# steveschwarcz/Cuda-Path-Tracer-SS

Measured on AMD Instinct MI355X. Metric: Mrays/sec at 1920x1080, 8 bounces, 2072 spp run (BASELINE configs[2] asks 2000 spp; a rate metric); ray = one live ray processed in one bounce, higher is better.
Workload: dtype f32; 1 GPU; configs[2]: 1920x1080 'mixed' preset (22 spheres, 16 triangles, Lambert/Phong/Cook-Torrance/glass/mirror), 8 bounces, 2072 spp = 74 steps x 1 pass(es) x 28 sample lanes per pixel; samples_per_pass=28, frame_lanes=1, lanes_free_run=True, seed=24301

## Files before the change

### cuda-path-tracer-ss_amd/csrc/pthit.h

```cpp
#pragma once
#include "ptaccel.h"

namespace ptss {
namespace {

template <bool kPrimary, bool kAccel, bool kBounded, bool kMesh = false>
__device__ __forceinline__ Hit closestHit(const float4* sc, const float4* cold, const SceneLayout& L, vec3 o, vec3 d, bool live, uint32_t* ws) {
    Hit h;
    h.distance = ptm::inf();
    h.kind = 0;
    h.idx = 0;
    h.w0 = h.w1 = h.w2 = 0;
    if constexpr (kAccel) closestSpheresRegrouped<kPrimary>(sc, cold, L, o, d, live, h, ws);
    for (int base = 0; base < (kAccel ? 0 : L.numSpheres); base += 32) {
        const int cnt = (L.numSpheres - base < 32) ? (L.numSpheres - base) : 32;
        uint32_t mask = sphereCandidates<kPrimary, kBounded>(sc, (kPrimary ? L.offPrimSphere : L.offSphere) + base, cnt, o, d);
        mask &= live ? lowBits(cnt) : 0u;
        PTSS_DIAG_CANDIDATES(mask, live, 0);
        while (mask != 0) {
            const int j = __builtin_ctz(mask);
            mask &= mask - 1;
            float t;
            const bool acc = kPrimary ? sphereTestPrimary(sc[L.offPrimSphere + base + j], d, h.distance, t)
                                      : sphereTest(sc[L.offSphere + base + j], o, d, h.distance, t);
            if (acc) {
                h.distance = t;
                h.kind = 1;
                h.idx = base + j;
            }
        }
    }
    const unsigned long long liveMask = maskOf(live);
    if constexpr (kMesh) {
        if (meshQueryOk(o, d, live)) {
            TriBest best{h.distance, kNoTriangle, 0.0f, 0.0f};
            closestTrianglesMesh<kPrimary>(sc, cold, L, o, d, live, best);
            if (best.key != kNoTriangle) {
                h.distance = best.dist;
                h.kind = 2;
                h.idx = reinterpret_cast<const int*>(cold + L.offTriPos)[0xfffffffeu - best.key];
                h.w1 = best.w1;
                h.w2 = best.w2;
                h.w0 = 1.0f - (best.w1 + best.w2);
            }
            return h;
        }
    } else if (L.triClassed) {
        if (classedQueryOk(o, d)) {
            TriBest best{h.distance, kNoTriangle, 0.0f, 0.0f};
            uint32_t triAt = vectorRow(sc, L.offTri), primAt = vectorRow(sc, L.offPrimTri);
#define PTSS_CLOSEST_BODY(c1, c2, t) \
    triangleClassed<kPrimary, c1, c2, true>(rowAt(sc, triAt), rowAt(sc, primAt), 0u, o, d, liveMask, best);
            PTSS_FOR_TRIANGLES_BY_CLASS(L, PTSS_CLOSEST_BODY, (triAt += 3 * kRowBytes, primAt += 2 * kRowBytes));
#undef PTSS_CLOSEST_BODY
            if (waveAny(best.key != kNoTriangle)) {
                const int* posOf = reinterpret_cast<const int*>(sc + L.offTriPos);
                int pos = 0;
                if (best.key != kNoTriangle) pos = posOf[0xfffffffeu - best.key];
                const bool zeroWeight = best.key != kNoTriangle && (best.w1 == 0.0f || best.w2 == 0.0f);
                if (waveAny(zeroWeight)) {
                    if (zeroWeight) {
                        const float4* rows = sc + L.offTri + 3 * pos;
                        const float4* prim = sc + L.offPrimTri + 2 * pos;
                        const pttri::Head g = pttri::head<0, 0, kPrimary>(xyz(rows[0]), xyz(rows[1]), xyz(rows[2]), xyz(prim[0]), xyz(prim[1]), prim[0].w, o, d);
                        float b0;
                        pttri::weights<0, 0>(g, d, b0, best.w1, best.w2);
                    }
                }
                if (best.key != kNoTriangle) {
                    h.distance = best.dist;
                    h.kind = 2;
                    h.idx = pos;
                    h.w1 = best.w1;
                    h.w2 = best.w2;
                    h.w0 = 1.0f - (best.w1 + best.w2);
                }
            }
            return h;
        }
    } else if (L.triDetBounded && waveAll(dot(d, d) < 0x1p30f)) {
        TriBest best{h.distance, kNoTriangle, 0.0f, 0.0f};
        uint32_t triAt = vectorRow(sc, L.offTri), primAt = vectorRow(sc, L.offPrimTri);
        for (int i = 0; i < L.numTriangles; ++i, triAt += 3 * kRowBytes, primAt += 2 * kRowBytes)
            triangleClassed<kPrimary, 0, 0, false>(rowAt(sc, triAt), rowAt(sc, primAt), (uint32_t)i, o, d, liveMask, best);
        if (best.key != kNoTriangle) {
            h.distance = best.dist;
            h.kind = 2;
            h.idx = (int)best.key;
            h.w1 = best.w1;
            h.w2 = best.w2;
            h.w0 = 1.0f - (best.w1 + best.w2);
        }
        return h;
    }
    const float4* td = kMesh ? cold : sc;
    const int* posOfOriginal = reinterpret_cast<const int*>(td + L.offTriPos);
    for (int k = 0; k < L.numTriangles; ++k) {
        const int i = (kMesh || L.triClassed) ? posOfOriginal[k] : k;
        const TriRows tcur = kPrimary ? loadTriEdges(td + L.offTri + 3 * i) : loadTri(td + L.offTri + 3 * i);
        const TriHit th = kPrimary ? triangleTestPrimary(tcur, td[L.offPrimTri + 2 * i], loadRow16(td + L.offPrimTri + 2 * i + 1), d,
                                                         h.distance, liveMask)
                                   : triangleTest(tcur, o, d, h.distance, liveMask);
        if (th.hit) {
            h.distance = th.dist;
            h.kind = 2;
            h.idx = i;
            h.w0 = th.w0;
            h.w1 = th.w1;
            h.w2 = th.w2;
        }
    }
    return h;
}

__device__ __forceinline__ void anyTriangleLoop(const float4* sc, const SceneLayout& L, vec3 lo, vec3 w_i, float distance, unsigned long long& need,
                                                unsigned long long& blocked) {
    if (L.triClassed && classedQueryOk(lo, w_i)) {
        uint32_t triAt = vectorRow(sc, L.offTri);
#define PTSS_ANY_BODY(c1, c2, t)   \
    if (need == 0ull) break;      \
    triangleClassedAny<c1, c2>(rowAt(sc, triAt), lo, w_i, distance, need, blocked);
        PTSS_FOR_TRIANGLES_BY_CLASS(L, PTSS_ANY_BODY, triAt += 3 * kRowBytes);
#undef PTSS_ANY_BODY
        return;
    }
    for (int i = 0; i < L.numTriangles; ++i) {
        if (need == 0ull) break;
        const TriRows tcur = loadTri(sc + L.offTri + 3 * i);
        const TriHit th = triangleTest(tcur, lo, w_i, distance, need);
        blocked |= th.hitMask;
        need &= ~th.hitMask;
    }
}

__device__ __forceinline__ bool anyTriangles(const float4* sc, const SceneLayout& L, vec3 lo, vec3 w_i, float distance, bool live) {
    unsigned long long need = maskOf(live), blocked = 0ull;
    anyTriangleLoop(sc, L, lo, w_i, distance, need, blocked);
    return __builtin_amdgcn_inverse_ballot_w64(blocked);
}

template <bool kAccel, bool kBounded, bool kMesh = false>
__device__ __forceinline__ bool anyHit(const float4* sc, const SceneLayout& L, vec3 lo, vec3 w_i, float distance,
                                       bool live, const float4* cold = nullptr) {
    bool occluded = false;
    if constexpr (kAccel) occluded = anySphereChunked(sc, L, lo, w_i, distance, live);
    for (int base = 0; base < (kAccel ? 0 : L.numSpheres); base += 32) {
        const int cnt = (L.numSpheres - base < 32) ? (L.numSpheres - base) : 32;
        uint32_t mask = sphereCandidatesPairs<kBounded>(sc, L.offSphere + base, cnt, lo, w_i);
        mask &= (live && !occluded) ? lowBits(cnt) : 0u;
        PTSS_DIAG_CANDIDATES(mask, live, 4);
        while (mask != 0) {
            const int j = __builtin_ctz(mask);
            mask &= mask - 1;
            float t;
            if (sphereTest(sc[L.offSphere + base + j], lo, w_i, distance, t)) {
                occluded = true;
                mask = 0;
            }
        }
    }
    if constexpr (kMesh) return anyTrianglesMesh(sc, cold, L, lo, w_i, distance, live && !occluded) || occluded;
    unsigned long long need = maskOf(live) & ~maskOf(occluded);
    unsigned long long blocked = 0ull;
    anyTriangleLoop(sc, L, lo, w_i, distance, need, blocked);
    return occluded || __builtin_amdgcn_inverse_ballot_w64(blocked);
}

template <bool kBounded>
__device__ __forceinline__ bool anyHitSplit(const float4* sc, const SceneLayout& L, vec3 lo, vec3 w_i, float distance,
                                            bool live, int shift, int sub) {
    bool occluded = false;
    const int g = 1 << shift;
    const int sphereSteps = (L.numSpheres + g - 1) >> shift;
    for (int base = 0; base < sphereSteps; base += 32) {
        const int cnt = (sphereSteps - base < 32) ? (sphereSteps - base) : 32;
        uint32_t mask = sphereCandidatesStridedPairs<kBounded>(sc + L.offSphere + (base << shift) + sub, g, cnt, lo, w_i);
        mask &= (live && !occluded) ? lowBitsClamped(((L.numSpheres - sub + g - 1) >> shift) - base) : 0u;
        while (mask != 0) {
            const int j = __builtin_ctz(mask);
            mask &= mask - 1;
            float t;
            if (sphereTest(sc[L.offSphere + ((base + j) << shift) + sub], lo, w_i, distance, t)) {
                occluded = true;
                mask = 0;
            }
        }
    }
    const int triSteps = (L.numTriangles + g - 1) >> shift;
    unsigned long long need = maskOf(live) & ~maskOf(occluded);
    unsigned long long blocked = 0ull;
    for (int k = 0; k < triSteps; ++k) {
        if (need == 0ull) break;
        const int idx = (k << shift) + sub;
        const bool in = idx < L.numTriangles;
        const TriRows tcur = loadTri(sc + L.offTri + 3 * (in ? idx : 0));
        const TriHit th = triangleTest(tcur, lo, w_i, distance, need & maskOf(in));
        blocked |= th.hitMask;
        need &= ~th.hitMask;
    }
    return occluded || __builtin_amdgcn_inverse_ballot_w64(blocked);
}

template <bool kBounded, bool kSplit>
__device__ __forceinline__ void pairAnyHit(const float4* sc, const SceneLayout& L, vec3 lo, vec3 wA, float dA, bool liveA, vec3 wB, float dB,
                                           bool liveB, int shift, int sub, bool& occA, bool& occB) {
// ... 196 lines not shown
```

### cuda-path-tracer-ss_amd/csrc/ptprim.h

```cpp
#pragma once
#include "ptscene.h"
#include "pttri.h"
#include "ptwave.h"

namespace ptss {
namespace {

__device__ __forceinline__ bool sphereTest(float4 sp, vec3 o, vec3 d, float limit, float& t) {
    const vec3 v = o - xyz(sp);
    const float b = dot(d, v) * 2;
    const float c = dot(v, v) - sp.w;
    float disc = (b * b) - 4 * c;
    if (disc < 0) return false;
    disc = ptm::sqrt(disc);
    float t0 = (-b + disc) * 0.5f;
    float t1 = (-b - disc) * 0.5f;
    if (t0 < 0 && t1 < 0) return false;
    if (t0 > t1) {
        const float tmp = t0;
        t0 = t1;
        t1 = tmp;
    }
    const float cand = (t0 < 0) ? t1 : t0;
    if (cand > limit) return false;
// ... 80 lines not shown
        const bool hit = __builtin_amdgcn_inverse_ballot_w64(hitMask);
        best.dist = hit ? h.dist : best.dist;
        best.key = hit ? key : best.key;
        best.w1 = hit ? b1 : best.w1;
        best.w2 = hit ? b2 : best.w2;
    }
}
struct ClassBounds {
    uint32_t w[5];
};
__device__ __forceinline__ ClassBounds classBounds(const SceneLayout& L) {
    return ClassBounds{{L.triClassPack[0], L.triClassPack[1], L.triClassPack[2], L.triClassPack[3], L.triClassPack[4]}};
}
template <int kCode>
__device__ __forceinline__ int classBegin(ClassBounds& b) {
    asm volatile("" : "+s"(b.w[kCode / 4]));
    return (int)((b.w[kCode / 4] >> (8 * (kCode % 4))) & 255u);
}
#define PTSS_FOR_TRIANGLES_BY_CLASS(L, BODY, STEP)                                                                  \
    do {                                                                                                            \
        ClassBounds _cb = classBounds(L);                                                                           \
        PTSS_TRI_CLASS_LOOP(_cb, 0, 0, BODY, STEP) PTSS_TRI_CLASS_LOOP(_cb, 0, 1, BODY, STEP) PTSS_TRI_CLASS_LOOP(_cb, 0, 2, BODY, STEP) PTSS_TRI_CLASS_LOOP(_cb, 0, 3, BODY, STEP) \
        PTSS_TRI_CLASS_LOOP(_cb, 1, 0, BODY, STEP) PTSS_TRI_CLASS_LOOP(_cb, 1, 2, BODY, STEP) PTSS_TRI_CLASS_LOOP(_cb, 1, 3, BODY, STEP)      \
        PTSS_TRI_CLASS_LOOP(_cb, 2, 0, BODY, STEP) PTSS_TRI_CLASS_LOOP(_cb, 2, 1, BODY, STEP) PTSS_TRI_CLASS_LOOP(_cb, 2, 3, BODY, STEP)      \
        PTSS_TRI_CLASS_LOOP(_cb, 3, 0, BODY, STEP) PTSS_TRI_CLASS_LOOP(_cb, 3, 1, BODY, STEP) PTSS_TRI_CLASS_LOOP(_cb, 3, 2, BODY, STEP)      \
    } while (0)
#define PTSS_TRI_CLASS_LOOP(cb, c1, c2, BODY, STEP) \
    for (int t = classBegin<(c1) * 4 + (c2)>(cb), tEnd = classBegin<(c1) * 4 + (c2) + 1>(cb); t < tEnd; ++t, STEP) { BODY(c1, c2, t) }

template <int kC1, int kC2>
__device__ __forceinline__ void triangleClassedAny(const float4* rows, vec3 o, vec3 d, float limit, unsigned long long& need, unsigned long long& blocked) {
    const pttri::Head h = pttri::head<kC1, kC2, false>(xyz(loadRow16(rows)), xyz(loadRow16(rows + 1)), xyz(loadRow16(rows + 2)), v3(0, 0, 0), v3(0, 0, 0), 0.0f, o, d);
    const unsigned long long passMask = need & maskOf(!(ptm::abs(h.det) <= 1e-7f)) & maskOf(!(h.dist <= 0.0f)) & maskOf(!(h.dist > limit));
    if (passMask != 0ull) {
        float b0, b1, b2;
        pttri::weights<kC1, kC2>(h, d, b0, b1, b2);
        const unsigned long long hitMask = passMask & maskOf(!(__builtin_fminf(__builtin_fminf(b0, b1), b2) < 0));
        blocked |= hitMask;
        need &= ~hitMask;
    }
}
template <int kC1, int kC2>
__device__ __forceinline__ void triangleClassedPair(const float4* rows, vec3 o, vec3 dA, float limitA, vec3 dB, float limitB, unsigned long long& needA,
                                                    unsigned long long& needB, unsigned long long& blockedA, unsigned long long& blockedB) {
    const vec3 e1 = xyz(loadRow16(rows + 1)), e2 = xyz(loadRow16(rows + 2));
    const pttri::OriginPart p = pttri::originPart<kC1, kC2>(xyz(loadRow16(rows)), e1, e2, o);
    if (needA != 0ull) {
        const pttri::Head h = pttri::headFrom<kC1, kC2>(p, e1, e2, dA);
        const unsigned long long pass = needA & maskOf(!(ptm::abs(h.det) <= 1e-7f)) & maskOf(!(h.dist <= 0.0f)) & maskOf(!(h.dist > limitA));
        if (pass != 0ull) {
            float b0, b1, b2;
            pttri::weights<kC1, kC2>(h, dA, b0, b1, b2);
            const unsigned long long hit = pass & maskOf(!(__builtin_fminf(__builtin_fminf(b0, b1), b2) < 0));
            blockedA |= hit;
            needA &= ~hit;
        }
    }
    if (needB != 0ull) {
        const pttri::Head h = pttri::headFrom<kC1, kC2>(p, e1, e2, dB);
        const unsigned long long pass = needB & maskOf(!(ptm::abs(h.det) <= 1e-7f)) & maskOf(!(h.dist <= 0.0f)) & maskOf(!(h.dist > limitB));
        if (pass != 0ull) {
            float b0, b1, b2;
            pttri::weights<kC1, kC2>(h, dB, b0, b1, b2);
            const unsigned long long hit = pass & maskOf(!(__builtin_fminf(__builtin_fminf(b0, b1), b2) < 0));
            blockedB |= hit;
            needB &= ~hit;
        }
    }
}
__device__ __forceinline__ bool classedQueryOk(vec3 o, vec3 d) { return waveAll(dot(d, d) < 0x1p30f) && waveAll(dot(o, o) < 0x1p100f); }

__device__ __forceinline__ bool sphereTestPrimary(float4 pv, vec3 d, float limit, float& t) {
    const float b = dot(d, xyz(pv)) * 2;
    float disc = (b * b) - 4 * pv.w;
    if (disc < 0) return false;
    disc = ptm::sqrt(disc);
    float t0 = (-b + disc) * 0.5f;
    float t1 = (-b - disc) * 0.5f;
    if (t0 < 0 && t1 < 0) return false;
    if (t0 > t1) {
        const float tmp = t0;
        t0 = t1;
        t1 = tmp;
    }
    const float cand = (t0 < 0) ? t1 : t0;
    if (cand > limit) return false;
    t = cand;
    return true;
}

__device__ __forceinline__ TriHit triangleTestPrimary(const TriRows& tr, float4 ps , float4 pr ,
                                                      vec3 d, float limit, unsigned long long liveMask) {
    const vec3 e1 = xyz(tr.b), e2 = xyz(tr.c);
    const vec3 q = cross(d, e2);
    const float det = dot(e1, q);
    const float inverseDet = triRcp(det);
    const float dist = ps.w * inverseDet;
    const unsigned long long passMask = liveMask & maskOf(!(ptm::abs(det) <= 1e-7f)) & maskOf(!(dist <= 0.0f)) & maskOf(!(dist > limit));
    TriHit h;
    h.hit = false;
    h.hitMask = 0ull;
    h.dist = dist;
    h.w0 = h.w1 = h.w2 = 0;
    if (passMask != 0ull) {
        const float b1 = dot(xyz(ps), q) * inverseDet;
        const float b2 = dot(d, xyz(pr)) * inverseDet;
        const float b0 = 1.0f - (b1 + b2);
        h.hitMask = passMask & maskOf(!(b0 < 0)) & maskOf(!(b1 < 0)) & maskOf(!(b2 < 0));
        h.hit = __builtin_amdgcn_inverse_ballot_w64(h.hitMask);
        h.w0 = b0;
        h.w1 = b1;
        h.w2 = b2;
    }
    return h;
}

__device__ __forceinline__ void shiftInMayHit(uint32_t& rev, float bb, float c4) {
    asm("v_cmp_nlt_f32 vcc, %1, %2\n\tv_addc_co_u32 %0, vcc, %0, %0, vcc" : "+v"(rev) : "v"(bb), "v"(c4) : "vcc");
}
template <bool kCull>
__device__ __forceinline__ float aheadFactor(float h) {
    if constexpr (kCull) {
        const float hk = h * 0x1p-18f;
        float m;
        asm("v_min_f32 %0, %1, %2" : "=v"(m) : "v"(hk), "v"(h));
        return m;
    } else {
        return h;
    }
}
template <bool kBounded, bool kCull = false>
__device__ __forceinline__ void shiftInSphere(uint32_t& rev, float4 sp, vec3 o, vec3 d) {
    const vec3 v = o - xyz(sp);
    if constexpr (kBounded) {
        const float h = dot(d, v);
        const float c = dot(v, v) - sp.w;
        shiftInMayHit(rev, h * aheadFactor<kCull>(h), c);
    } else {
        const float b = dot(d, v) * 2;
        const float c = dot(v, v) - sp.w;
        shiftInMayHit(rev, b * b, 4 * c);
    }
}
template <bool kBounded>
__device__ __forceinline__ void shiftInSpherePrimary(uint32_t& rev, float4 pv, vec3 d) {
    if constexpr (kBounded) {
        const float h = dot(d, xyz(pv));
        shiftInMayHit(rev, h * h, pv.w);
    } else {
        const float b = dot(d, xyz(pv)) * 2;
        shiftInMayHit(rev, b * b, 4 * pv.w);
    }
}
template <bool kPrimary, bool kBounded>
__device__ __forceinline__ uint32_t sphereCandidates(const float4* image, int firstRow, int cnt, vec3 o, vec3 d) {
    const int trips = (cnt + 3) >> 2;
    uint32_t rev = 0;
    uint32_t at = vectorRow(image, firstRow);
    for (int g = 0; g < trips; ++g, at += 4 * kRowBytes) {
        const float4* p = rowAt(image, at);
        const float4 r0 = p[0], r1 = p[1], r2 = p[2], r3 = p[3];
        if constexpr (kPrimary) {
            shiftInSpherePrimary<kBounded>(rev, r0, d);
            shiftInSpherePrimary<kBounded>(rev, r1, d);
            shiftInSpherePrimary<kBounded>(rev, r2, d);
            shiftInSpherePrimary<kBounded>(rev, r3, d);
        } else {
            shiftInSphere<kBounded, true>(rev, r0, o, d);
            shiftInSphere<kBounded, true>(rev, r1, o, d);
            shiftInSphere<kBounded, true>(rev, r2, o, d);
            shiftInSphere<kBounded, true>(rev, r3, o, d);
        }
    }
    return __builtin_bitreverse32(rev) >> (32 - 4 * trips);
}
template <bool kBounded>
__device__ __forceinline__ uint32_t sphereCandidatesPairs(const float4* image, int firstRow, int cnt, vec3 o, vec3 d) {
    const int trips = (cnt + 1) >> 1;
    uint32_t rev = 0;
    uint32_t at = vectorRow(image, firstRow);
    for (int g = 0; g < trips; ++g, at += 2 * kRowBytes) {
        const float4* p = rowAt(image, at);
        const float4 r0 = p[0], r1 = p[1];
        shiftInSphere<kBounded>(rev, r0, o, d);
        shiftInSphere<kBounded>(rev, r1, o, d);
    }
    return __builtin_bitreverse32(rev) >> (32 - 2 * trips);
}
template <bool kBounded>
__device__ __forceinline__ uint32_t sphereCandidatesStridedPairs(const float4* first, int stride, int cnt, vec3 o, vec3 d) {
    const int trips = (cnt + 1) >> 1;
    uint32_t rev = 0;
    for (int g = 0; g < trips; ++g) {
        const float4* p = first + 2 * g * stride;
        const float4 r0 = p[0], r1 = p[stride];
        shiftInSphere<kBounded>(rev, r0, o, d);
        shiftInSphere<kBounded>(rev, r1, o, d);
    }
    return __builtin_bitreverse32(rev) >> (32 - 2 * trips);
}

}
}
```

### cuda-path-tracer-ss_amd/csrc/ptss_api.hip

```cpp
#include <stdio.h>
#include <stdlib.h>
#include <string.h>

#include <new>
#include <string>
#include <vector>

#include "ptss.h"
#include "ptss_device.h"
#include <algorithm>
#include "ptdenoise.h"
#include "ptupsample.h"
#include "ptreproject.h"
#include "ptspecular.h"
#include "ptpack.h"

using namespace ptv;
using ptpack::cameraInRange;
static_assert(sizeof(ptpack::Row) == sizeof(float4) && alignof(ptpack::Row) == alignof(float4), "a packed row is uploaded as a float4");

#if PTSS_DIAG
namespace ptss { hipError_t readDiagCounters(unsigned long long* out8); }
#endif
namespace {

thread_local std::string g_detail;

int fail(int code, const char* what, hipError_t e = hipSuccess) {
    char buf[512];
    if (e != hipSuccess)
        snprintf(buf, sizeof(buf), "%s: %s (%s)", what, hipGetErrorString(e), hipGetErrorName(e));
    else
        snprintf(buf, sizeof(buf), "%s", what);
    g_detail = buf;
    return code;
}

#define HIP_TRY(expr)                                        \
    do {                                                     \
        hipError_t _e = (expr);                              \
        if (_e != hipSuccess) return fail(PTSS_EHIP, #expr, _e); \
    } while (0)

#define RC_TRY(expr) do { if (int _rc = (expr)) return _rc; } while (0)

struct EventPair {
    hipEvent_t a, b;
};

}

struct Lane {
    hipStream_t stream = nullptr;
    float* dPool[2] = {nullptr, nullptr};
    uint32_t* dCounts[2] = {nullptr, nullptr};
    uint32_t* dShardCount0 = nullptr;
    uint32_t* dLastCounts = nullptr;
    uint32_t* dDone = nullptr;
    uint32_t doneTarget[ptss::kMaxBounces + 1] = {};
    hipEvent_t evDone[2] = {nullptr, nullptr};
    uint32_t regionCap = 0;
    int maxBlocks = 0;
    uint32_t hint[ptss::kMaxBounces + 1] = {0};
    bool haveHint = false;
    uint32_t* hCounts = nullptr;
    hipEvent_t hintEvent[4] = {nullptr, nullptr, nullptr, nullptr};
    bool hintPending[4] = {false, false, false, false};
};

struct SceneImage {
    float4* dBlob = nullptr;
    ptss::SceneLayout layout{};
    bool inLds = true;
    bool oneLaunch = false;
    uint32_t guardFlags = 0;
};

struct ptss_context {
    ptss_render_config cfg{};
    hipStream_t stream = nullptr;
    ptss::TileMap tile{};
    SceneImage images[2];
    int active = 0;
    const SceneImage& image() const { return images[active]; }
    std::vector<Lane> lanes;
    hipEvent_t evFork = nullptr;
    int countParity = 0;
    uint32_t* dRngHome = nullptr;
    unsigned long long* dTotal = nullptr;
    uint32_t* dAccumOwned = nullptr;
    uint32_t* dAccum = nullptr;
    float* dFsum = nullptr;
    uint32_t* dStaged = nullptr;
    bool stagedTwice = false;
    hipEvent_t evDisplay[2] = {nullptr, nullptr};
    uint32_t capacity = 0, numPixels = 0;
    uint32_t samples = 1;
    bool cameraDirty = true;
    float defaultColor[3] = {0, 0, 0};
    ptss_camera camera{};
    int lastResetTick = 0;
    int lastTicks = 0;
    unsigned maxIterations = 15;
    bool resetTicksThisFrame = true;
    bool usePathTracer = true;
    hipEvent_t evStart = nullptr, evStop = nullptr;
    float lastMs = 0.0f;
    int gridCap = 0;
    unsigned frameIndex = 0;
    std::vector<EventPair> evFree, evBusy;
    std::vector<std::pair<double, double>> kernelSpans;
    hipEvent_t evEpoch = nullptr;
    unsigned int timeoutsSeen = 0;
    unsigned long long launchedKernels = 0;
    unsigned long long specularFeatureLaunches[2] = {0, 0};
    unsigned long long upsampleLaunches = 0;
    unsigned long long pathLaunches[2] = {0, 0};
    uint32_t* dPathJumpTable = nullptr;
    float4* dDenoise[2] = {nullptr, nullptr};
    int denoiseLastPlane = -1;
    int denoiseLastLevel = -1;
    hipStream_t denoiseStream = nullptr;
    int numCUs = 0;
    hipStream_t updateStream = nullptr;
    bool updated = false;
    ptss::ResortScratch resortScratch;
    unsigned long long resortLaunches = 0;
};
constexpr int kTotalWords = ptss::kMaxLanes + 8 + 1;
constexpr int kRejectedWord = ptss::kMaxLanes;

namespace {

int validateScene(const ptss_scene_desc& s) {
    const char* what = ptpack::validateScene(s);
    return what ? fail(PTSS_EINVAL, what) : PTSS_OK;
}

int localRows(const ptss_render_config& cfg) {
    int rows = 0;
    for (int y = 0; y < cfg.height; ++y)
        if ((y / cfg.bandRows) % cfg.tileWorld == cfg.tileRank) ++rows;
    return rows;
}

int createCheck(hipError_t e, const char* what) { return e == hipSuccess ? PTSS_OK : fail(e == hipErrorOutOfMemory ? PTSS_ENOMEM : PTSS_EHIP, what, e); }
#define ALLOC_TRY(expr) RC_TRY(createCheck((expr), #expr))
template <class T>
hipError_t mallocZeroed(T** p, size_t bytes) {
    const hipError_t e = hipMalloc(p, bytes);
    return e == hipSuccess ? hipMemset(*p, 0, bytes) : e;
}

struct SceneState {
    SceneImage images[2];
    int gridCap = 0;
    float defaultColor[3] = {0, 0, 0};
};
void releaseSceneState(SceneState& st) {
    for (SceneImage& im : st.images) {
        (void)hipFree(im.dBlob);
        im = SceneImage{};
    }
}
int buildSceneState(const ptss_scene_desc& scene, const ptss_render_config& cfg, int numLanes, int maxBlocks0, int numCUs, SceneState& st) {
    std::vector<ptpack::PackedImage> packed;
    try {
        packed = ptpack::packImages(scene, cfg.everySphereLoop != 0);
    } catch (const std::bad_alloc&) {
        return fail(PTSS_ENOMEM, "scene image (host)");
    }
    const int numImages = (int)packed.size();
    for (int i = 0; i < numImages; ++i) {
        SceneImage& im = st.images[i];
        im.layout = packed[(size_t)i].layout;
        im.inLds = packed[(size_t)i].inLds;
        im.guardFlags = ptpack::sceneGuardFlags(scene);
        const std::vector<ptpack::Row>& blob = packed[(size_t)i].blob;
        hipError_t e = hipMalloc(&im.dBlob, blob.size() * sizeof(float4));
        if (e == hipSuccess) e = hipMemcpy(im.dBlob, blob.data(), blob.size() * sizeof(float4), hipMemcpyHostToDevice);
        if (e != hipSuccess) {
            releaseSceneState(st);
            return createCheck(e, "scene image (device)");
        }
    }
    st.defaultColor[0] = scene.defaultColor.x;
    st.defaultColor[1] = scene.defaultColor.y;
    st.defaultColor[2] = scene.defaultColor.z;
    const SceneImage& primary = st.images[0];
    const int perCU = ptss::bounceOccupancyBlocksPerCU(primary.layout, primary.inLds, primary.layout.sphereBounded != 0);
    st.gridCap = numCUs * (perCU > 0 ? perCU : 4) * 16 / ptss::kShards;
    auto qualifies = [&](const SceneImage& im) {
        if (cfg.oneLaunchFrames <= 0 || numLanes != 1 || !im.inLds) return false;
        if (ptss::meshImage(im.layout)) return false;
        int perCU = ptss::frameOccupancyBlocksPerCU(im.layout, false);
        if (im.layout.sphereBounded) perCU = std::min(perCU, ptss::frameOccupancyBlocksPerCU(im.layout, true));
        const int resident = perCU - 1;
        return resident >= 1 && maxBlocks0 <= numCUs * resident;
    };
    for (int i = 0; i < numImages; ++i) st.images[i].oneLaunch = qualifies(st.images[i]);
#ifdef PTSS_TUNING_KNOBS
    if (const char* e = getenv("PTSS_SCENE_PATH")) {
        if (!strcmp(e, "scalar"))
            for (int i = 0; i < numImages; ++i) st.images[i].inLds = false;
    }
    if (const char* e = getenv("PTSS_GRID_CAP")) st.gridCap = atoi(e);
#endif
    return PTSS_OK;
}
void adoptSceneState(ptss_context* c, const SceneState& st) {
    for (int i = 0; i < 2; ++i) c->images[i] = st.images[i];
    c->gridCap = st.gridCap;
    for (int k = 0; k < 3; ++k) c->defaultColor[k] = st.defaultColor[k];
    c->active = 0;
}

int allocLane(Lane& ln, const uint32_t (&shardCount0)[ptss::kShards], bool ownStream) {
    const size_t poolBytes = (size_t)ptss::kRayPlanes * ln.regionCap * ptss::kShards * sizeof(float);
    for (float*& pool : ln.dPool) ALLOC_TRY(hipMalloc(&pool, poolBytes));
    for (uint32_t*& counts : ln.dCounts) ALLOC_TRY(mallocZeroed(&counts, ptss::kCountWords * sizeof(uint32_t)));
    ALLOC_TRY(mallocZeroed(&ln.dLastCounts, ptss::kCountWords * sizeof(uint32_t)));
    for (int s = 0; s < ptss::kShards; ++s)
        ALLOC_TRY(hipMemcpy(ln.dCounts[0] + ptss::countIndex(0, s), &shardCount0[s], sizeof(uint32_t), hipMemcpyHostToDevice));
    ALLOC_TRY(hipMalloc(&ln.dShardCount0, sizeof(shardCount0)));
    ALLOC_TRY(hipMemcpy(ln.dShardCount0, shardCount0, sizeof(shardCount0), hipMemcpyHostToDevice));
    ALLOC_TRY(mallocZeroed(&ln.dDone, (ptss::kCountWords + ptss::kCountStride) * sizeof(uint32_t)));
    if (ownStream) {
        ALLOC_TRY(hipStreamCreateWithFlags(&ln.stream, hipStreamNonBlocking));
        for (hipEvent_t& ev : ln.evDone) ALLOC_TRY(hipEventCreateWithFlags(&ev, hipEventDisableTiming));
    }
    ALLOC_TRY(hipHostMalloc(&ln.hCounts, 4 * ptss::kCountWords * sizeof(uint32_t), hipHostMallocDefault));
    for (hipEvent_t& ev : ln.hintEvent) ALLOC_TRY(hipEventCreateWithFlags(&ev, hipEventDisableTiming));
    return PTSS_OK;
}
#undef ALLOC_TRY

hipError_t seedStreams(ptss_context* c, unsigned long long seed, hipStream_t st) {
    std::vector<uint32_t> table(ptrng::kJumpTableWords);
    ptrng::build_subsequence_table(table.data());
    uint32_t* dTable = nullptr;
    hipError_t e = hipMalloc(&dTable, table.size() * sizeof(uint32_t));
    if (e != hipSuccess) return e;
    e = hipMemcpy(dTable, table.data(), table.size() * sizeof(uint32_t), hipMemcpyHostToDevice);
    if (e == hipSuccess && c->numPixels > 0) e = ptss::launchRngInit(st, c->dRngHome, c->capacity, c->samples, c->tile, seed, dTable);
    if (e == hipSuccess) e = hipStreamSynchronize(st);
    (void)hipFree(dTable);
    return e;
}

int quiesce(ptss_context* c) {
    HIP_TRY(hipStreamSynchronize(c->stream));
    for (const Lane& ln : c->lanes)
        if (ln.stream) HIP_TRY(hipStreamSynchronize(ln.stream));
    return PTSS_OK;
}

void releaseLane(Lane& ln) {
    for (hipEvent_t ev : ln.hintEvent)
        if (ev) (void)hipEventDestroy(ev);
    if (ln.hCounts) (void)hipHostFree(ln.hCounts);
    (void)hipFree(ln.dDone);
    for (hipEvent_t ev : ln.evDone)
        if (ev) (void)hipEventDestroy(ev);
    if (ln.stream) (void)hipStreamDestroy(ln.stream);
    for (float* pool : ln.dPool) (void)hipFree(pool);
    for (uint32_t* counts : ln.dCounts) (void)hipFree(counts);
    (void)hipFree(ln.dShardCount0);
    (void)hipFree(ln.dLastCounts);
}

ptss::FrameBuffers frameBuffers(const ptss_context* c, int laneIdx, ptss_uchar4* pixels, int sample) {
    const Lane& ln = c->lanes[(size_t)laneIdx];
    ptss::FrameBuffers fb{};
    fb.pool[0] = ln.dPool[0];
    fb.pool[1] = ln.dPool[1];
    fb.rngHome = c->dRngHome;
    fb.counts = ln.dCounts[c->countParity];
    fb.countsNext = ln.dCounts[1 - c->countParity];
    fb.shardCount0 = ln.dShardCount0;
    fb.lastCounts = ln.dLastCounts;
    fb.totalRayBounces = c->dTotal + laneIdx;
    fb.guardTimeouts = reinterpret_cast<uint32_t*>(c->dTotal + ptss::kMaxLanes + 8);
    fb.accum = c->dAccum;
    fb.fsum = c->dFsum;
    fb.staged = c->dStaged ? c->dStaged + (c->stagedTwice ? (size_t)(c->frameIndex & 1u) * c->capacity * c->samples : 0) : nullptr;
    fb.quantTable = reinterpret_cast<const float*>(c->image().dBlob + c->image().layout.offQuant);
    fb.pixels = pixels;
    fb.regionCap = ln.regionCap;
    fb.numPixels = c->numPixels;
    fb.plane = c->capacity;
    fb.samples = c->samples;
    fb.firstTiles = c->samples * (c->capacity / ptss::kBlock);
    fb.minLive = c->tile.world > 1 ? 0u : ptss::kMinLiveRays;
    fb.inverseTicks = 1.f / (float)((int)c->samples * (sample + 1));
    fb.defaultColor[0] = c->defaultColor[0];
    fb.defaultColor[1] = c->defaultColor[1];
    fb.defaultColor[2] = c->defaultColor[2];
    fb.guardFlags = c->image().guardFlags;
    fb.laneIndex = (uint32_t)laneIdx;
    fb.laneCount = (uint32_t)c->lanes.size();
    fb.frameRays = c->numPixels * c->samples;
    fb.numPeers = fb.laneCount - 1;
    fb.myDone = ln.dDone;
    fb.myFrameDone = ln.dDone + ptss::kCountWords;
    fb.frameSeq = c->frameIndex;
    fb.joinsFrame = (laneIdx + 1 == (int)c->lanes.size()) ? 1u : 0u;
    uint32_t p = 0;
    for (size_t k = 0; k < c->lanes.size(); ++k) {
        if ((int)k == laneIdx) continue;
        fb.peerCounts[p] = c->lanes[k].dCounts[c->countParity];
        fb.peerDone[p] = c->lanes[k].dDone;
        fb.peerFrameDone[p] = c->lanes[k].dDone + ptss::kCountWords;
        ++p;
    }
    return fb;
}

void drainKernelEvents(ptss_context* c, bool wait) {
    size_t k = 0;
    for (size_t i = 0; i < c->evBusy.size(); ++i) {
        EventPair p = c->evBusy[i];
        hipError_t q = wait ? hipEventSynchronize(p.b) : hipEventQuery(p.b);
        if (q == hipSuccess) {
            float start = 0, ms = 0;
            if (hipEventElapsedTime(&start, c->evEpoch, p.a) == hipSuccess && hipEventElapsedTime(&ms, p.a, p.b) == hipSuccess)
            {
                if (c->kernelSpans.size() >= (1u << 20)) c->kernelSpans.clear();
                c->kernelSpans.emplace_back((double)start, (double)start + (double)ms);
            }
            c->evFree.push_back(p);
        } else {
            c->evBusy[k++] = p;
        }
    }
    c->evBusy.resize(k);
    (void)hipGetLastError();
}

int checkLaneTimeouts(ptss_context* c) {
    if (c->lanes.size() < 2 && !c->images[0].oneLaunch && !c->images[1].oneLaunch) return PTSS_OK;
    uint32_t v = 0;
    HIP_TRY(hipMemcpy(&v, c->dTotal + ptss::kMaxLanes + 8, sizeof(v), hipMemcpyDeviceToHost));
    if (v != c->timeoutsSeen) {
        c->timeoutsSeen = v;
        return fail(PTSS_ETIMEOUT, "a bounded wait on the device expired (a frame lane for a peer lane, or a workgroup of the one-launch "
                                   "frame kernel for its shard): the frame was not traced as specified");
    }
    return PTSS_OK;
}

void selectImage(ptss_context* c) {
    if (!c->images[1].dBlob) return;
    const int want = cameraInRange(c->camera) ? 0 : 1;
    if (want != c->active) {
        c->active = want;
        c->cameraDirty = true;
    }
}

ptss::EyeParams eyeParams(const ptss_context* c) {
    return {c->camera, -2 * ptm::tan(c->camera.fieldOfView * 0.5f), (float)c->tile.height / (float)c->tile.width, 1.0f / c->tile.width,
            1.0f / c->tile.height};
}

void harvestHints(ptss_context* c) {
    for (Lane& ln : c->lanes)
        for (int q = 0; q < 4; ++q) {
            if (!ln.hintPending[q] || hipEventQuery(ln.hintEvent[q]) != hipSuccess) continue;
            const uint32_t* src = ln.hCounts + (size_t)q * ptss::kCountWords;
            for (int b = 0; b <= ptss::kMaxBounces; ++b) {
                uint32_t mx = 0;
                for (int s = 0; s < ptss::kShards; ++s) mx = std::max(mx, src[ptss::countIndex(b, s)]);
                ln.hint[b] = mx;
            }
            ln.haveHint = true;
            ln.hintPending[q] = false;
        }
    (void)hipGetLastError();
}

int forkLanes(ptss_context* c, bool forkNeeded) {
    if (c->lanes.size() > 1 && (forkNeeded || c->frameIndex == 0 || !c->cfg.lanesFreeRun)) {
        HIP_TRY(hipEventRecord(c->evFork, c->stream));
        for (Lane& ln : c->lanes) HIP_TRY(hipStreamWaitEvent(ln.stream, c->evFork, 0));
    }
    if (c->stagedTwice && c->frameIndex >= 2)
        for (Lane& ln : c->lanes) HIP_TRY(hipStreamWaitEvent(ln.stream, c->evDisplay[c->frameIndex & 1u], 0));
    return PTSS_OK;
}

template <class Launch>
int timedLaunch(ptss_context* c, hipStream_t s, Launch launch) {
    if (!c->cfg.timeKernels) return launch();
    EventPair ev{nullptr, nullptr};
    if (c->evFree.empty() && c->evBusy.size() >= 4096) drainKernelEvents(c, true);
    if (c->evFree.empty()) {
        HIP_TRY(hipEventCreate(&ev.a));
        HIP_TRY(hipEventCreate(&ev.b));
    } else {
        ev = c->evFree.back();
        c->evFree.pop_back();
    }
    HIP_TRY(hipEventRecord(ev.a, s));
    RC_TRY(launch());
    HIP_TRY(hipEventRecord(ev.b, s));
    c->evBusy.push_back(ev);
    return PTSS_OK;
}

int traceOneLaunch(ptss_context* c, const ptss::FrameBuffers& fb, int numIterations, bool bounded, const ptss::EyeParams& eye) {
    const SceneImage& im = c->image();
    return timedLaunch(c, c->stream, [&] {
        HIP_TRY(ptss::launchFrame(c->stream, fb, im.dBlob, im.layout, numIterations, bounded, c->lanes[0].maxBlocks, c->tile, eye,
                                          &c->launchedKernels));
        return PTSS_OK;
    });
}

int traceBounces(ptss_context* c, ptss::FrameBuffers* fbs, int numIterations, bool bounded, const ptss::EyeParams& eye) {
    const SceneImage& im = c->image();
    const int K = (int)c->lanes.size();
    for (int i = 0; i < numIterations; ++i)
        for (int k = 0; k < K; ++k) {
            Lane& ln = c->lanes[(size_t)k];
            const hipStream_t ls = K > 1 ? ln.stream : c->stream;
            int blocks = ln.maxBlocks;
            if (i > 0 && ln.haveHint) {
                const unsigned long long tilesPerShard = ((unsigned long long)ln.hint[i] * 65 / 64 + ptss::kBlock) / ptss::kBlock + 1;
                const unsigned long long want = tilesPerShard * ptss::kShards;
                if (want < (unsigned long long)blocks) blocks = (int)want;
            }
            if (c->gridCap > 0 && c->gridCap * ptss::kShards < blocks) blocks = c->gridCap * ptss::kShards;
            if (i > 0)
                for (int j = 0, p = 0; j < K; ++j)
                    if (j != k) fbs[k].peerTarget[p++] = c->lanes[(size_t)j].doneTarget[i - 1];
            RC_TRY(timedLaunch(c, ls, [&] {
                HIP_TRY(ptss::launchBounce(ls, fbs[k], im.dBlob, im.layout, i, i == numIterations - 1, im.inLds, bounded, blocks, c->tile, eye,
                                               &c->launchedKernels));
                return PTSS_OK;
            }));
            ln.doneTarget[i] += (uint32_t)blocks;
        }
    return PTSS_OK;
}

int flushAndJoin(ptss_context* c, const ptss::FrameBuffers* fbs, int numIterations) {
    const int K = (int)c->lanes.size();
    for (int k = 0; k < K; ++k) {
        Lane& ln = c->lanes[(size_t)k];
        const hipStream_t ls = K > 1 ? ln.stream : c->stream;
        ptss::FlushTargets targets{};
        for (int j = 0, p = 0; j < K; ++j)
            if (j != k) {
                for (int b = 0; b <= ptss::kMaxBounces; ++b) targets.target[p][b] = c->lanes[(size_t)j].doneTarget[b];
                ++p;
            }
        HIP_TRY(ptss::launchFlush(ls, fbs[k], numIterations, targets));
        if (!ln.haveHint || (c->frameIndex & 7u) == 0) {
            const int q = (int)((c->frameIndex >> 3) & 3u);
            if (!ln.hintPending[q]) {
                HIP_TRY(hipMemcpyAsync(ln.hCounts + (size_t)q * ptss::kCountWords, ln.dLastCounts, ptss::kCountWords * sizeof(uint32_t),
                                       hipMemcpyDeviceToHost, ls));
                HIP_TRY(hipEventRecord(ln.hintEvent[q], ls));
                ln.hintPending[q] = true;
            }
        }
        if (K > 1 && k == K - 1) {
            HIP_TRY(hipEventRecord(ln.evDone[c->frameIndex & 1u], ls));
            HIP_TRY(hipStreamWaitEvent(c->stream, ln.evDone[c->frameIndex & 1u], 0));
        }
    }
    return PTSS_OK;
}

}

extern "C" {

int ptss_version(void) { return PTSS_VERSION; }

const char* ptss_error_string(int code) {
    switch (code) {
        case PTSS_OK: return "ok";
        case PTSS_EINVAL: return "invalid argument";
        case PTSS_EHIP: return "HIP runtime error";
        case PTSS_ENODEVICE: return "no usable HIP device";
        case PTSS_ENOMEM: return "out of memory";
        case PTSS_ERANGE: return "buffer too small or index out of range";
        case PTSS_ETIMEOUT: return "a frame lane timed out waiting for a peer lane";
        default: return "unknown error";
    }
}

const char* ptss_last_error_detail(void) { return g_detail.c_str(); }

int ptss_default_config(ptss_render_config* cfg) {
    if (!cfg) return fail(PTSS_EINVAL, "cfg is null");
    memset(cfg, 0, sizeof(*cfg));
    cfg->structSize = (unsigned int)sizeof(*cfg);
    cfg->width = 512;
    cfg->height = 512;
    cfg->seed = 0x5EEDull;
    cfg->maxIterations = 15;
    cfg->device = 0;
    cfg->tileRank = 0;
    cfg->tileWorld = 1;
    cfg->bandRows = 8;
    cfg->syncEachFrame = 1;
    cfg->floatAccumulator = 0;
    cfg->timeKernels = 0;
    cfg->samplesPerPass = 1;
    cfg->everySphereLoop = 0;
    cfg->frameLanes = 0;
    cfg->lanesFreeRun = 0;
    cfg->oneLaunchFrames = 0;
    return PTSS_OK;
}

int ptss_create(const ptss_scene_desc* scene, const ptss_render_config* cfg, ptss_context** out) {
    if (!scene || !cfg || !out) return fail(PTSS_EINVAL, "null argument");
    if (cfg->structSize != (unsigned int)sizeof(ptss_render_config))
        return fail(PTSS_EINVAL, "cfg->structSize is not this library's sizeof(ptss_render_config): the caller was built against another "
                                 "ptss.h (compare ptss_version() with PTSS_VERSION) or did not start from ptss_default_config");
    if (cfg->width <= 0 || cfg->height <= 0 || (long long)cfg->width * cfg->height > (1ll << 31) - 256)
        return fail(PTSS_EINVAL, "bad frame size");
    if (cfg->maxIterations == 0 || cfg->maxIterations > (unsigned)ptss::kMaxBounces)
        return fail(PTSS_EINVAL, "maxIterations must be in [1, 64]");
    if (cfg->tileWorld <= 0 || cfg->tileRank < 0 || cfg->tileRank >= cfg->tileWorld || cfg->bandRows <= 0)
        return fail(PTSS_EINVAL, "bad tile spec");
    const int spp = cfg->samplesPerPass == 0 ? 1 : cfg->samplesPerPass;
    if (spp < 1 || spp > 64) return fail(PTSS_EINVAL, "samplesPerPass must be in [1, 64]");
    if ((long long)cfg->width * cfg->height >= (1ll << 26)) return fail(PTSS_EINVAL, "frame too large (>= 2^26 pixels)");
    {
        const long long rows = localRows(*cfg);
        const unsigned long long rays = ((unsigned long long)cfg->width * rows + 255ull) / 256ull * 256ull * (unsigned long long)spp;
        if ((rays + (unsigned long long)ptss::kShards * ptss::kBlock) * ptss::kRayPlanes >= (1ull << 32))
            return fail(PTSS_EINVAL, "too many rays per pass: width x local rows x samplesPerPass must stay below ~226 million");
    }
    int rc = validateScene(*scene);
    if (rc != PTSS_OK) return rc;

    int ndev = 0;
    hipError_t e = hipGetDeviceCount(&ndev);
    if (e != hipSuccess || ndev <= 0) {
        (void)hipGetLastError();
        return fail(PTSS_ENODEVICE, "hipGetDeviceCount found no device (libptss has no CPU path)", e);
    }
    if (cfg->device < 0 || cfg->device >= ndev) return fail(PTSS_ENODEVICE, "device ordinal out of range");
    HIP_TRY(hipSetDevice(cfg->device));

    ptss_context* c = new (std::nothrow) ptss_context();
    if (!c) return fail(PTSS_ENOMEM, "context");
    c->cfg = *cfg;
    c->maxIterations = cfg->maxIterations;
    c->samples = (uint32_t)spp;
    c->camera.rotation = q4(1, 0, 0, 0);
    c->camera.position = v3(0, 0, 0);
    c->camera.zNear = -0.1f;
    c->camera.zFar = -100.0f;
    c->camera.fieldOfView = ptm::kPi / 2.0f;

    c->tile = ptss::TileMap{cfg->width, cfg->height, localRows(*cfg), cfg->tileRank, cfg->tileWorld, cfg->bandRows};
    c->numPixels = (uint32_t)cfg->width * (uint32_t)c->tile.localRows;
    const uint32_t gran = ptss::kBlock > 256 ? (uint32_t)ptss::kBlock : 256u;
    c->capacity = ((c->numPixels + gran - 1) / gran) * gran;
    if (c->capacity == 0) c->capacity = gran;
    int numLanes = cfg->frameLanes;
    if (numLanes < 0 || numLanes > ptss::kMaxLanes) return (delete c, fail(PTSS_EINVAL, "frameLanes must be in [0, 4]"));
    {
        const unsigned long long rays = (unsigned long long)c->numPixels * c->samples;
        if (numLanes == 0) numLanes = (cfg->lanesFreeRun && rays >= (3ull << 17) && rays <= (1ull << 24)) ? 2 : 1;
    }
    c->lanes.resize((size_t)numLanes);
    uint32_t shardCount0[ptss::kMaxLanes][ptss::kShards] = {{0}};
    {
        const uint32_t tilesPerPlane = c->capacity / ptss::kBlock;
        const uint32_t tiles = tilesPerPlane * c->samples;
        const uint32_t rounds = (tiles + ptss::kShards - 1) / ptss::kShards;
        for (int k = 0; k < numLanes; ++k) {
            const uint32_t laneRounds = (rounds + (uint32_t)numLanes - 1 - (uint32_t)k) / (uint32_t)numLanes;
            c->lanes[(size_t)k].regionCap = (laneRounds ? laneRounds : 1) * ptss::kBlock;
            c->lanes[(size_t)k].maxBlocks = (int)(c->lanes[(size_t)k].regionCap / ptss::kBlock) * ptss::kShards;
        }
        for (uint32_t t = 0; t < tiles; ++t) {
            const uint32_t first = (t % tilesPerPlane) * ptss::kBlock;
            uint32_t cnt = 0;
            if (first < c->numPixels) cnt = c->numPixels - first < (uint32_t)ptss::kBlock ? c->numPixels - first : (uint32_t)ptss::kBlock;
            shardCount0[(t / ptss::kShards) % (uint32_t)numLanes][t % ptss::kShards] += cnt;
        }
    }

#define CREATE_TRY(expr) do { if (int _rc = createCheck((expr), #expr)) return (ptss_destroy(c), _rc); } while (0)

    {
        hipDeviceProp_t prop;
        CREATE_TRY(hipGetDeviceProperties(&prop, cfg->device));
        c->numCUs = prop.multiProcessorCount;
        SceneState st;
        if (int sceneRc = buildSceneState(*scene, *cfg, numLanes, c->lanes[0].maxBlocks, c->numCUs, st)) return (ptss_destroy(c), sceneRc);
        adoptSceneState(c, st);
    }
    CREATE_TRY(hipMalloc(&c->dRngHome, (size_t)ptss::kHomeWords * c->capacity * c->samples * sizeof(uint32_t)));
    for (int k = 0; k < numLanes; ++k)
        if (int laneRc = allocLane(c->lanes[(size_t)k], shardCount0[k], numLanes > 1)) return (ptss_destroy(c), laneRc);
    if (numLanes > 1) CREATE_TRY(hipEventCreateWithFlags(&c->evFork, hipEventDisableTiming));
    CREATE_TRY(mallocZeroed(&c->dTotal, kTotalWords * sizeof(unsigned long long)));
    CREATE_TRY(mallocZeroed(&c->dAccumOwned, (size_t)3 * c->capacity * sizeof(uint32_t)));
    c->dAccum = c->dAccumOwned;
    if (cfg->floatAccumulator) CREATE_TRY(mallocZeroed(&c->dFsum, (size_t)3 * c->capacity * c->samples * sizeof(float)));
    if (c->samples > 1) {
        c->stagedTwice = numLanes > 1 && cfg->lanesFreeRun != 0;
        const size_t words = (size_t)c->capacity * c->samples * (c->stagedTwice ? 2 : 1);
        CREATE_TRY(mallocZeroed(&c->dStaged, words * sizeof(uint32_t)));
        if (c->stagedTwice)
            for (int q = 0; q < 2; ++q) CREATE_TRY(hipEventCreateWithFlags(&c->evDisplay[q], hipEventDisableTiming));
    }
    CREATE_TRY(hipEventCreate(&c->evStart));
    CREATE_TRY(hipEventCreate(&c->evStop));
    CREATE_TRY(hipEventCreate(&c->evEpoch));

    CREATE_TRY(seedStreams(c, cfg->seed, nullptr));
    CREATE_TRY(hipEventRecord(c->evEpoch, nullptr));
    CREATE_TRY(hipDeviceSynchronize());

#undef CREATE_TRY

    *out = c;
    return PTSS_OK;
}

int ptss_destroy(ptss_context* c) {
    if (!c) return PTSS_OK;
    (void)hipSetDevice(c->cfg.device);
    (void)hipDeviceSynchronize();
    drainKernelEvents(c, true);
    for (EventPair& p : c->evFree) {
        (void)hipEventDestroy(p.a);
        (void)hipEventDestroy(p.b);
    }
    for (Lane& ln : c->lanes) releaseLane(ln);
    for (hipEvent_t ev : {c->evFork, c->evDisplay[0], c->evDisplay[1], c->evStart, c->evStop, c->evEpoch})
        if (ev) (void)hipEventDestroy(ev);
    for (SceneImage& im : c->images) (void)hipFree(im.dBlob);
    (void)hipFree(c->dRngHome);
    (void)hipFree(c->dTotal);
    (void)hipFree(c->dAccumOwned);
    (void)hipFree(c->dFsum);
    (void)hipFree(c->dStaged);
    for (float4* plane : c->dDenoise) (void)hipFree(plane);
    ptss::releaseResortScratch(c->resortScratch);
    (void)hipFree(c->dPathJumpTable);
    delete c;
    return PTSS_OK;
}

int ptss_generate_frame(ptss_context* c, ptss_uchar4* pixels, int ticks) {
    if (!c) return fail(PTSS_EINVAL, "ctx is null");
    hipStream_t st = c->stream;
    HIP_TRY(hipSetDevice(c->cfg.device));
    c->lastTicks = ticks;
    if (c->numPixels == 0) {
        if (c->resetTicksThisFrame) c->lastResetTick = ticks;
        c->resetTicksThisFrame = false;
        c->lastMs = 0.0f;
        return PTSS_OK;
    }

    selectImage(c);
    bool forkNeeded = false;
    if (c->resetTicksThisFrame) {
        forkNeeded = true;
        c->lastResetTick = ticks;
        HIP_TRY(ptss::launchClear(st, frameBuffers(c, 0, pixels, 0)));
        c->resetTicksThisFrame = false;
    }
    const int sample = ticks - c->lastResetTick;
    const int K = (int)c->lanes.size();
    ptss::FrameBuffers fbs[ptss::kMaxLanes];
    for (int k = 0; k < K; ++k) fbs[k] = frameBuffers(c, k, pixels, sample);

    if (c->cfg.syncEachFrame) HIP_TRY(hipEventRecord(c->evStart, st));

    const int numIterations = c->usePathTracer ? (int)c->maxIterations : 1;
    const ptss::EyeParams eye = eyeParams(c);
    if (c->cameraDirty) {
        forkNeeded = true;
        HIP_TRY(ptss::launchPrimaryPrep(st, c->image().dBlob, c->image().layout, c->camera.position));
        c->cameraDirty = false;
    }
    harvestHints(c);
    RC_TRY(forkLanes(c, forkNeeded));
    if (c->cfg.timeKernels) drainKernelEvents(c, false);
    const bool bounded = c->image().layout.sphereBounded != 0 && cameraInRange(c->camera);
    RC_TRY(c->image().oneLaunch && K == 1 ? traceOneLaunch(c, fbs[0], numIterations, bounded, eye) : traceBounces(c, fbs, numIterations, bounded, eye));
    RC_TRY(flushAndJoin(c, fbs, numIterations));
    if (c->samples > 1) {
        HIP_TRY(ptss::launchDisplay(st, fbs[0]));
        if (c->stagedTwice) HIP_TRY(hipEventRecord(c->evDisplay[c->frameIndex & 1u], st));
    }
    c->countParity ^= 1;
    c->frameIndex++;

    if (c->cfg.syncEachFrame) {
        HIP_TRY(hipEventRecord(c->evStop, st));
        HIP_TRY(hipEventSynchronize(c->evStop));
        HIP_TRY(hipEventElapsedTime(&c->lastMs, c->evStart, c->evStop));
        return c->lanes.size() > 1 ? checkLaneTimeouts(c) : PTSS_OK;
    }
    return PTSS_OK;
}

int ptss_set_camera(ptss_context* c, const ptss_camera* camera) {
    if (!c || !camera) return fail(PTSS_EINVAL, "null argument");
    c->camera = *camera;
    c->cameraDirty = true;
    c->resetTicksThisFrame = true;
    return PTSS_OK;
}

int ptss_get_camera(const ptss_context* c, ptss_camera* out) {
    if (!c || !out) return fail(PTSS_EINVAL, "null argument");
    *out = c->camera;
    return PTSS_OK;
}

int ptss_request_reset(ptss_context* c) {
    if (!c) return fail(PTSS_EINVAL, "ctx is null");
    c->resetTicksThisFrame = true;
    return PTSS_OK;
}

int ptss_set_mode(ptss_context* c, int usePathTracer) {
    if (!c) return fail(PTSS_EINVAL, "ctx is null");
    c->usePathTracer = usePathTracer != 0;
    c->resetTicksThisFrame = true;
    return PTSS_OK;
}

int ptss_set_max_iterations(ptss_context* c, unsigned int maxIterations) {
    if (!c || maxIterations == 0 || maxIterations > (unsigned)ptss::kMaxBounces)
        return fail(PTSS_EINVAL, "maxIterations must be in [1, 64]");
    c->maxIterations = maxIterations;
    return PTSS_OK;
}

int ptss_set_stream(ptss_context* c, void* hipStream) {
    if (!c) return fail(PTSS_EINVAL, "ctx is null");
    c->stream = (hipStream_t)hipStream;
    return PTSS_OK;
}

int ptss_bind_accumulator(ptss_context* c, uint32_t* dev) {
    if (!c) return fail(PTSS_EINVAL, "ctx is null");
    c->dAccum = dev ? dev : c->dAccumOwned;
    return PTSS_OK;
}

int ptss_accumulator_devptr(ptss_context* c, uint32_t** out) {
    if (!c || !out) return fail(PTSS_EINVAL, "null argument");
    *out = c->dAccum;
    return PTSS_OK;
}

int ptss_float_accumulator_devptr(ptss_context* c, float** out) {
    if (!c || !out) return fail(PTSS_EINVAL, "null argument");
    *out = c->dFsum;
    return PTSS_OK;
}

int ptss_alloc_pixels(ptss_context* c, ptss_uchar4** out) {
    if (!c || !out) return fail(PTSS_EINVAL, "null argument");
    HIP_TRY(hipSetDevice(c->cfg.device));
    HIP_TRY(hipMalloc(out, (size_t)c->capacity * sizeof(ptss_uchar4)));
    HIP_TRY(hipMemset(*out, 0, (size_t)c->capacity * sizeof(ptss_uchar4)));
    return PTSS_OK;
}

int ptss_free_pixels(ptss_context* c, ptss_uchar4* dev) {
    if (!c) return fail(PTSS_EINVAL, "ctx is null");
    HIP_TRY(hipFree(dev));
    return PTSS_OK;
}

int ptss_local_pixels(const ptss_context* c, size_t* out) {
    if (!c || !out) return fail(PTSS_EINVAL, "null argument");
    *out = c->numPixels;
    return PTSS_OK;
}

int ptss_local_rows(const ptss_context* c, int* rows, int cap, int* count) {
    if (!c || !count) return fail(PTSS_EINVAL, "null argument");
    int n = 0;
    for (int y = 0; y < c->tile.height; ++y) {
        if ((y / c->tile.bandRows) % c->tile.world != c->tile.rank) continue;
        if (rows) {
            if (n >= cap) return fail(PTSS_ERANGE, "rows[] too small");
            rows[n] = y;
        }
        ++n;
    }
    *count = n;
    return PTSS_OK;
}

int ptss_synchronize(ptss_context* c) {
    if (!c) return fail(PTSS_EINVAL, "ctx is null");
    HIP_TRY(hipStreamSynchronize(c->stream));
    return checkLaneTimeouts(c);
}

int ptss_read_accumulator(ptss_context* c, uint32_t* host, size_t count) {
    if (!c || !host) return fail(PTSS_EINVAL, "null argument");
    if (count != (size_t)3 * c->numPixels) return fail(PTSS_ERANGE, "count must be 3 * local pixels");
    HIP_TRY(hipStreamSynchronize(c->stream));
    HIP_TRY(hipMemcpy(host, c->dAccum, count * sizeof(uint32_t), hipMemcpyDeviceToHost));
    return checkLaneTimeouts(c);
}

int ptss_read_float_accumulator(ptss_context* c, float* host, size_t count) {
    if (!c || !host) return fail(PTSS_EINVAL, "null argument");
    if (!c->dFsum) return fail(PTSS_EINVAL, "context was created without floatAccumulator");
    if (count != (size_t)3 * c->numPixels) return fail(PTSS_ERANGE, "count must be 3 * local pixels");
    HIP_TRY(hipStreamSynchronize(c->stream));
    if (c->samples == 1) {
        HIP_TRY(hipMemcpy(host, c->dFsum, count * sizeof(float), hipMemcpyDeviceToHost));
    } else {
        std::vector<float> lane(count);
        for (size_t k = 0; k < count; ++k) host[k] = 0.0f;
        for (uint32_t l = 0; l < c->samples; ++l) {
            HIP_TRY(hipMemcpy(lane.data(), c->dFsum + (size_t)3 * l * c->capacity, count * sizeof(float), hipMemcpyDeviceToHost));
            for (size_t k = 0; k < count; ++k) host[k] = host[k] + lane[k];
        }
    }
    return checkLaneTimeouts(c);
}

int ptss_read_pixels(ptss_context* c, const ptss_uchar4* dev, ptss_uchar4* host, size_t count) {
    if (!c || !dev || !host) return fail(PTSS_EINVAL, "null argument");
    if (count > c->numPixels) return fail(PTSS_ERANGE, "count exceeds local pixels");
    HIP_TRY(hipStreamSynchronize(c->stream));
    HIP_TRY(hipMemcpy(host, dev, count * sizeof(ptss_uchar4), hipMemcpyDeviceToHost));
    return checkLaneTimeouts(c);
}

int ptss_read_rng_state(ptss_context* c, size_t local_pixel, uint32_t* out6) { return ptss_read_rng_state_lane(c, local_pixel, 0, out6); }

int ptss_read_rng_state_lane(ptss_context* c, size_t local_pixel, unsigned int lane, uint32_t* out6) {
    if (!c || !out6) return fail(PTSS_EINVAL, "null argument");
    if (local_pixel >= c->numPixels || lane >= c->samples) return fail(PTSS_ERANGE, "pixel or lane out of range");
    HIP_TRY(hipStreamSynchronize(c->stream));
    HIP_TRY(hipMemcpy(out6, c->dRngHome + (size_t)ptss::kHomeWords * ((size_t)lane * c->capacity + local_pixel), 6 * sizeof(uint32_t),
                      hipMemcpyDeviceToHost));
    return PTSS_OK;
}

int ptss_last_pass_ms(ptss_context* c, float* out) {
    if (!c || !out) return fail(PTSS_EINVAL, "null argument");
    *out = c->lastMs;
    return PTSS_OK;
}

int ptss_samples_since_reset(const ptss_context* c, int* out) {
    if (!c || !out) return fail(PTSS_EINVAL, "null argument");
    *out = c->resetTicksThisFrame ? 0 : (c->lastTicks - c->lastResetTick + 1) * (int)c->samples;
    return PTSS_OK;
}

int ptss_live_counts(ptss_context* c, uint32_t* out, int cap, int* n) {
    if (!c || !out || !n) return fail(PTSS_EINVAL, "null argument");
// ... 557 lines not shown
```

### cuda-path-tracer-ss_amd/csrc/ptss_device.h

```cpp
#pragma once
#include <hip/hip_runtime.h>
#include <stdint.h>

#include "ptmath.h"
#include "ptscene.h"
#include "ptss_types.h"
#include "xorwow.h"

namespace ptdn { struct Level; }
namespace ptrp { struct View; struct Params; }

namespace ptss {

enum RayPlane : int {
    kOx = 0, kOy, kOz,
    kDx, kDy, kDz,
    kL0x, kL0y, kL0z,
    kTx, kTy, kTz,
    kPix,
    kR0, kR1, kR2, kR3, kR4,
    kRd,
    kRayPlanes
};
constexpr int kHomeWords = 8;
constexpr int kMaxBounces = 64;
#ifndef PTSS_SHARDS
#define PTSS_SHARDS 16
#endif
#ifndef PTSS_MINWAVES
#define PTSS_MINWAVES 7
#endif
#ifndef PTSS_MINWAVES_BOUNDED
#define PTSS_MINWAVES_BOUNDED 6
#endif
#ifndef PTSS_MINWAVES_FIRST
#define PTSS_MINWAVES_FIRST 6
#endif
#ifndef PTSS_ABLATE
#define PTSS_ABLATE 0
#endif
#ifndef PTSS_DIAG
#define PTSS_DIAG 0
#endif
constexpr int kShards = PTSS_SHARDS;
constexpr int kCountStride = 32;
constexpr int kCountWords = (kMaxBounces + 1) * kShards * kCountStride;
__host__ __device__ inline int countIndex(int bounce, int shard) { return (bounce * kShards + shard) * kCountStride; }
constexpr uint32_t kMinLiveRays = 128;

struct TileMap {
    int width, height;
    int localRows;
    int rank, world, bandRows;
};

struct EyeParams {
    ptss_camera camera;
    float s;
    float aspect;
    float invW, invH;
};

constexpr int kMaxLanes = 4;

struct FrameBuffers {
    float* pool[2];
    uint32_t* rngHome;
    uint32_t* counts;
    uint32_t* countsNext;
    const uint32_t* shardCount0;
    uint32_t* lastCounts;
    unsigned long long* totalRayBounces;
    uint32_t* accum;
    float* fsum;
    const float* quantTable;
    uint32_t* staged;
    ptss_uchar4* pixels;
    uint32_t regionCap;
    uint32_t numPixels;
    uint32_t plane;
    uint32_t samples;
    uint32_t firstTiles;
    uint32_t minLive;
    float inverseTicks;
    float defaultColor[3];
    uint32_t guardFlags;
    uint32_t laneIndex, laneCount;
    uint32_t frameRays;
    uint32_t numPeers;
    const uint32_t* peerCounts[kMaxLanes - 1];
    const uint32_t* peerDone[kMaxLanes - 1];
    uint32_t peerTarget[kMaxLanes - 1];
    uint32_t* myDone;
    uint32_t* myFrameDone;
    const uint32_t* peerFrameDone[kMaxLanes - 1];
    uint32_t frameSeq;
    uint32_t joinsFrame;
    uint32_t* guardTimeouts;
};

inline void markLaunched(unsigned long long* launched, int base, int index = 0) { *launched |= 1ull << (base + index); }
hipError_t launchRngInit(hipStream_t st, uint32_t* rngHome, uint32_t plane, uint32_t samples, TileMap tile, uint64_t seed,
                         const uint32_t* jumpTable);
hipError_t launchDisplay(hipStream_t st, const FrameBuffers& fb);
hipError_t launchClear(hipStream_t st, const FrameBuffers& fb);
hipError_t launchPrimaryPrep(hipStream_t st, float4* sceneBlob, const SceneLayout& layout, ptss_vec3 origin);
hipError_t launchBounce(hipStream_t st, const FrameBuffers& fb, const float4* sceneBlob, SceneLayout layout, int bounce,
                        bool isLast, bool sceneInLds, bool bounded, int gridBlocks, TileMap tile, EyeParams eye, unsigned long long* launched);
hipError_t launchFrame(hipStream_t st, const FrameBuffers& fb, const float4* sceneBlob, SceneLayout layout, int numBounces, bool bounded, int gridBlocks,
                       TileMap tile, EyeParams eye, unsigned long long* launched);
int frameOccupancyBlocksPerCU(const SceneLayout& layout, bool bounded);
struct FlushTargets {
    uint32_t target[kMaxLanes - 1][kMaxBounces + 1];
};
hipError_t launchFlush(hipStream_t st, const FrameBuffers& fb, int numBounces, const FlushTargets& targets);
int bounceOccupancyBlocksPerCU(const SceneLayout& layout, bool sceneInLds, bool bounded);
hipError_t launchQuery(hipStream_t st, bool any, const float4* sceneBlob, SceneLayout layout, bool sceneInLds, const void* rays, void* out,
                       uint32_t n, int maxBlocks, unsigned long long* launched);
hipError_t launchFeatures(hipStream_t st, const float4* sceneBlob, SceneLayout layout, bool sceneInLds, TileMap tile, EyeParams eye,
                          ptss_vec3 defaultColor, void* out, uint32_t n, int maxBlocks, unsigned long long* launched);
hipError_t launchFeaturesMotion(hipStream_t st, const float4* sceneBlob, SceneLayout layout, bool sceneInLds, TileMap tile, EyeParams eye,
                                ptss_vec3 defaultColor, void* out, uint32_t n, int maxBlocks, const void* prevRecords, uint32_t first,
                                uint32_t count, void* motionOut, unsigned long long* launched);
hipError_t launchFeaturesSpecular(hipStream_t st, const float4* sceneBlob, SceneLayout layout, bool sceneInLds, TileMap tile, EyeParams eye,
                                  ptss_vec3 defaultColor, void* out, void* steps, uint32_t n, int maxSteps, int maxBlocks,
                                  unsigned long long* launches);
hipError_t launchPathRngSeed(hipStream_t st, void* rng, uint32_t n, uint64_t seed, uint32_t firstSequence, uint32_t skip, const uint32_t* jumpTable);
hipError_t launchPathQuery(hipStream_t st, const float4* sceneBlob, SceneLayout layout, bool sceneInLds, const void* rays, void* rng, void* out,
                           uint32_t n, int maxIterations, ptss_vec3 defaultColor, uint32_t guardFlags, int maxBlocks, unsigned long long* launches);
hipError_t launchDenoise(hipStream_t st, bool first, bool last, const void* src, void* dst, const void* features, int width, int height,
                         const ptdn::Level& level, float inverseTicks, unsigned long long* launched);
hipError_t launchSceneUpdate(hipStream_t st, float4* sceneBlob, const SceneLayout& layout, const void* records, uint32_t first, uint32_t count,
                             unsigned long long* rejected, unsigned long long* launched);
hipError_t launchMeshRefit(hipStream_t st, float4* sceneBlob, const SceneLayout& layout, unsigned long long* launched);
struct ResortScratch {
    char* base = nullptr;
    int capacity = 0;
    float4* rows = nullptr;
    unsigned long long* keysIn = nullptr, *keysOut = nullptr;
    int2* seg = nullptr;
    uint32_t* codes = nullptr;
    int* iota = nullptr, *order = nullptr, *newPos = nullptr;
    uint32_t* extent = nullptr;
    size_t extentBytes = 0;
    void* temp = nullptr;
    size_t tempBytes = 0;
};
hipError_t reserveResortScratch(ResortScratch& scratch, int numTriangles);
void releaseResortScratch(ResortScratch& scratch);
hipError_t launchResort(hipStream_t st, float4* sceneBlob, const SceneLayout& layout, const ResortScratch& scratch);
hipError_t launchReproject(hipStream_t st, const uint32_t* accum, const void* featuresNow, const void* featuresPrev, const void* historyPrev,
                           void* historyOut, int width, int height, const ptrp::View& now, const ptrp::View& prev, const ptrp::Params& params,
                           float inverseTicks, float n, unsigned long long* launched);
hipError_t launchReprojectMotion(hipStream_t st, const uint32_t* accum, const void* featuresNow, const void* motionNow, const void* featuresPrev,
                                 const void* historyPrev, void* historyOut, int width, int height, const ptrp::View& now, const ptrp::View& prev,
                                 const ptrp::Params& params, float inverseTicks, float n, unsigned long long* launched);
hipError_t launchUpsample(hipStream_t st, const void* lo, const void* featuresLo, const void* featuresHi, void* outHi, void* outFloat, int width,
                          int height, int factor, const ptdn::Level& level, unsigned long long* launches);

}
```

### cuda-path-tracer-ss_amd/csrc/ptss_kernels.hip

```cpp
#include "ptss_device.h"
#include "ptmotion.h"
#include "ptspecular.h"
#include "pthit.h"
#include "ptshade.h"

#include <array>
#include <utility>

namespace ptss {

__global__ void rngInitKernel(uint32_t* __restrict__ rngHome, uint32_t plane, uint32_t samples, TileMap tile, uint64_t seed,
                              const uint32_t* __restrict__ jumpTable) {
    const uint32_t i = blockIdx.x * blockDim.x + threadIdx.x;
    const uint32_t n = (uint32_t)tile.width * (uint32_t)tile.localRows;
    const uint32_t lane = i / plane, p = i - lane * plane;
    if (lane >= samples || p >= n) return;
    const PixelCoord pc = locate(tile, p);
    ptrng::State s = ptrng::seeded(seed);
    ptrng::skip_subsequences(s, pc.globalIndex * samples + lane, jumpTable);
    storeHome(rngHome, i, s);
}

__global__ void clearKernel(FrameBuffers fb) {
    const uint32_t i = blockIdx.x * blockDim.x + threadIdx.x;
    if (i >= fb.numPixels) return;
    fb.accum[3 * i] = 0;
    fb.accum[3 * i + 1] = 0;
    fb.accum[3 * i + 2] = 0;
    if (fb.fsum)
        for (uint32_t l = 0; l < fb.samples; ++l) {
            float* fs = fb.fsum + 3u * (l * fb.plane + i);
            fs[0] = 0;
            fs[1] = 0;
            fs[2] = 0;
        }
    if (fb.pixels) fb.pixels[i] = ptss_uchar4{0, 0, 0, 0};
}

__global__ void displayKernel(FrameBuffers fb) {
    const uint32_t p = blockIdx.x * blockDim.x + threadIdx.x;
    if (p >= fb.numPixels) return;
    U3 t = reinterpret_cast<const U3*>(fb.accum)[p];
    uint32_t l = 0;
    for (; l + 8 <= fb.samples; l += 8) {
        uint32_t q[8];
#pragma unroll
        for (int k = 0; k < 8; ++k) q[k] = fb.staged[(l + k) * fb.plane + p];
#pragma unroll
        for (int k = 0; k < 8; ++k) {
            t.x += q[k] & 255u;
            t.y += (q[k] >> 8) & 255u;
            t.z += (q[k] >> 16) & 255u;
        }
    }
    for (; l < fb.samples; ++l) {
        const uint32_t q = fb.staged[l * fb.plane + p];
        t.x += q & 255u;
        t.y += (q >> 8) & 255u;
        t.z += (q >> 16) & 255u;
    }
    reinterpret_cast<U3*>(fb.accum)[p] = t;
    if (fb.pixels) {
        const uint32_t px = (uint32_t)(unsigned char)(t.x * fb.inverseTicks + 0.5f) |
                            ((uint32_t)(unsigned char)(t.y * fb.inverseTicks + 0.5f) << 8) |
                            ((uint32_t)(unsigned char)(t.z * fb.inverseTicks + 0.5f) << 16) | (255u << 24);
        reinterpret_cast<uint32_t*>(fb.pixels)[p] = px;
    }
}

__global__ void primaryPrepKernel(float4* __restrict__ blob, SceneLayout L, vec3 origin) {
    const int i = blockIdx.x * blockDim.x + threadIdx.x;
    if (i < L.numSpheres && !L.accelSpheres) {
        const float4 sp = blob[L.offSphere + i];
        const vec3 v = origin - xyz(sp);
        blob[L.offPrimSphere + i] = float4{v.x, v.y, v.z, dot(v, v) - sp.w};
    }
    if (L.accelSpheres && i < L.numChunks) {
        const float4 b = blob[L.offChunk + i];
        const vec3 v = origin - xyz(b);
        const float x = dot(v, v) - b.w;
        blob[L.offPrimChunk + i] = float4{v.x, v.y, v.z, x - ptm::abs(x) * 2.4e-7f};
    }
    if (i < L.numTriangles) {
        const vec3 v0 = xyz(blob[L.offTri + 3 * i]), e1 = xyz(blob[L.offTri + 3 * i + 1]), e2 = xyz(blob[L.offTri + 3 * i + 2]);
        const vec3 s = origin - v0;
        const vec3 r = cross(s, e1);
        blob[L.offPrimTri + 2 * i] = float4{s.x, s.y, s.z, dot(e2, r)};
        blob[L.offPrimTri + 2 * i + 1] = float4{r.x, r.y, r.z, 0.0f};
    }
}

struct TileEnv {
    const float4* sc;
    const float4* sceneBlob;
    const float* quantT;
    const float* in;
    float* out;
    float* wq;
    uint32_t* wqOwner;
    unsigned char* wqAnswer;
    uint32_t shard, lane, n;
    int numLights, bounce;
};

template <bool kLast, bool kFirst, bool kAccel, bool kBounded, bool kPairs, bool kCoherentIo, bool kMesh = false>
__device__ __forceinline__ void bounceTile(const FrameBuffers& fb, const SceneLayout& L, const TileMap& tile, const EyeParams& eye, const TileEnv& env,
                                           uint32_t base) {
    const float4* sc = env.sc;
    const float4* sceneBlob = env.sceneBlob;
    const float* quantT = env.quantT;
    const float* __restrict__ in = env.in;
    float* __restrict__ out = env.out;
    float* wq = env.wq;
    uint32_t* wqOwner = env.wqOwner;
    unsigned char* wqAnswer = env.wqAnswer;
    const uint32_t shard = env.shard, lane = env.lane, n = env.n;
    const int numLights = env.numLights, bounce = env.bounce;
    {
        const uint32_t i = base + threadIdx.x;
        uint32_t firstPixel = 0, firstLane = 0;
        bool valid = i < n;
        if constexpr (kFirst) {
            const uint32_t start = (((base / kBlock) * fb.laneCount + fb.laneIndex) * kShards + shard) * kBlock;
            firstLane = start / fb.plane;
            firstPixel = start - firstLane * fb.plane + threadIdx.x;
            valid = firstPixel < fb.numPixels;
        }

        RayRegs ray;
        ray.o = ray.d = ray.L0 = ray.T = v3(0, 0, 0);
        ray.pix = 0;
        ray.active = false;
        if constexpr (kFirst) {
            if (valid) {
                const uint32_t pixel = firstPixel;
                const uint32_t waveFirst = __builtin_amdgcn_readfirstlane(firstPixel - lane);
                const PixelCoord pc = locateLane(tile, locateWave(tile, waveFirst), waveFirst, lane);
                loadHome(fb.rngHome, firstLane * fb.plane + pixel, ray.rng);
                const float jitteredX = pc.x + ptrng::uniform(ray.rng);
                const float jitteredY = pc.gy + ptrng::uniform(ray.rng);
                const vec3 start = v3(((jitteredX * eye.invW) - 0.5f) * eye.s,
                                      1 * ((jitteredY * eye.invH) - 0.5f) * eye.s * eye.aspect, 1.0f) *
                                   eye.camera.zNear;
                ray.o = eye.camera.position;
                ray.d = normalize(rotate(eye.camera.rotation, start));
                ray.L0 = v3(0, 0, 0);
                ray.T = v3(1, 1, 1);
                ray.pix = pixel | (firstLane << kLaneShift);
                ray.active = true;
            }
        } else {
            if (valid) loadRayGeometry<kCoherentIo>(tileBlock(in, base), threadIdx.x, ray);
        }
#if PTSS_ABLATE & 2
        Hit h;
        h.kind = 2; h.idx = (int)(pixOf(ray.pix) % (uint32_t)L.numTriangles); h.distance = 1.0f + ray.d.x;
        h.w0 = 0.3f; h.w1 = 0.3f; h.w2 = 0.4f;
#else
        const Hit h = closestHit<kFirst, kAccel, kBounded, kMesh>(sc, sceneBlob, L, ray.o, ray.d, valid, reinterpret_cast<uint32_t*>(wq));
#endif
        const bool hit = valid && h.kind != 0;
        if constexpr (!kFirst) {
            if (valid) loadRayRng<kCoherentIo>(tileBlock(in, base), threadIdx.x, ray);
        }
        const float4* td = kMesh ? sceneBlob : sc;
        vec3 point = v3(0, 0, 0), normal = v3(0, 0, 0);
        float cosI = 0;
        int materialIdx = 0;
        if (hit) {
            point = ray.o + ray.d * h.distance;
            if (h.kind == 1) {
                normal = normalize(point - xyz(loadRow16(sc + L.offSphere + h.idx)));
                materialIdx = reinterpret_cast<const int*>((kAccel ? sceneBlob : sc) + L.offSphereMat)[h.idx];
            } else {
                const float4* nn = td + L.offTriNormal + 3 * h.idx;
                normal = (xyz(loadRow16(nn)) * h.w0 + xyz(loadRow16(nn + 1)) * h.w1) + xyz(loadRow16(nn + 2)) * h.w2;
                materialIdx = (int)asU(td[L.offTri + 3 * h.idx].w);
            }
            cosI = dot(-ray.d, normal);
        }
        const bool inside = cosI <= 0.0f;
        const bool lit = hit && !inside && !(PTSS_ABLATE & 1);
        const float4* mat = sc + L.offMaterial + 5 * materialIdx;

        vec3 radiance = v3(0, 0, 0);
        for (int l0 = 0; l0 < numLights; l0 += kNeeLights) {
            uint32_t queued = 0;
            bool need[kNeeLights];
            float cosL[kNeeLights], distance2[kNeeLights];
            [[maybe_unused]] vec3 pairW[kNeeLights];
            [[maybe_unused]] float pairReach[kNeeLights];
#pragma unroll
            for (int k = 0; k < kNeeLights; ++k) {
                need[k] = false;
                cosL[k] = 0;
                distance2[k] = 0;
                pairW[k] = v3(0, 0, 0);
                pairReach[k] = 0;
                const int li = l0 + k;
                if (li >= numLights) continue;
                vec3 lo = v3(0, 0, 0), w_i = v3(0, 0, 0);
                float distance = 0;
                if (lit) {
                    vec3 lightPoint;
                    if (li < L.numPointLights) {
                        lightPoint = xyz(loadRow16(sc + L.offPointLight + 2 * li));
                    } else {
                        const float4 light = sc[L.offAreaLight + 2 * (li - L.numPointLights)];
                        const float u1 = ptrng::uniform(ray.rng);
                        const float u2 = ptrng::uniform(ray.rng);
                        const float u3 = ptrng::uniform(ray.rng);
                        const float inverseTotal = ptm::rcp_in_range(u1 + u2 + u3);
                        const float weight0 = u1 * inverseTotal, weight1 = u2 * inverseTotal, weight2 = u3 * inverseTotal;
                        const int tri = (ptrng::uniform(ray.rng) > .5f) ? (int)asU(light.w) : (int)asU(sc[L.offAreaLight + 2 * (li - L.numPointLights) + 1].x);
                        const vec3 a = xyz(loadRow16(td + L.offTri + 3 * tri));
                        const vec3 b = xyz(loadRow16(td + L.offTriVert + 2 * tri));
                        const vec3 c = xyz(loadRow16(td + L.offTriVert + 2 * tri + 1));
                        lightPoint = (a * weight0 + b * weight1) + c * weight2;
                    }
                    const vec3 offset = lightPoint - point;
                    lightSample(offset, distance2[k], distance, w_i);
                    cosL[k] = ptm::max(0.0f, dot(normal, w_i));
                    const bool zeroTerm = L.neeSkipSafe && (distance2[k] > 0.0f) && (distance2[k] < ptm::inf()) &&
                                          (cosL[k] == 0.0f || mat[0].w == 0.0f);
                    need[k] = !zeroTerm;
                    lo = point + (ptm::kRayBump * normal);
                    distance -= 2 * ptm::kRayBump;
                }
                if constexpr (kPairs) {
                    pairW[k] = w_i;
                    pairReach[k] = distance;
                    continue;
                }
                const unsigned long long m = __ballot(need[k]);
                if (need[k]) {
                    const uint32_t slot = queued + __popcll(m & ((1ull << lane) - 1ull));
                    wq[0 * kQueueCap + slot] = lo.x;
                    wq[1 * kQueueCap + slot] = lo.y;
                    wq[2 * kQueueCap + slot] = lo.z;
                    wq[3 * kQueueCap + slot] = w_i.x;
                    wq[4 * kQueueCap + slot] = w_i.y;
                    wq[5 * kQueueCap + slot] = w_i.z;
                    wq[6 * kQueueCap + slot] = distance;
                    wqOwner[slot] = lane | ((uint32_t)k << 8);
                    wqAnswer[k * 64 + lane] = 0;
                }
                queued += (uint32_t)__popcll(m);
            }
            PTSS_DIAG_PAIRS(need[0], need[1], lit);
            waveLdsFence();
            PTSS_DIAG_QUEUE(queued);
            if constexpr (kPairs) {
                constexpr int kPairCap = 64;
                const bool needAny = need[0] || need[1];
                const unsigned long long m = __ballot(needAny);
                const uint32_t pairs = (uint32_t)__popcll(m);
                uint32_t* pairOwner = reinterpret_cast<uint32_t*>(wq + 11 * kPairCap);
                if (needAny) {
                    const uint32_t slot = __popcll(m & ((1ull << lane) - 1ull));
                    const vec3 lo = point + (ptm::kRayBump * normal);
                    wq[0 * kPairCap + slot] = lo.x;
                    wq[1 * kPairCap + slot] = lo.y;
                    wq[2 * kPairCap + slot] = lo.z;
                    wq[3 * kPairCap + slot] = pairW[0].x;
                    wq[4 * kPairCap + slot] = pairW[0].y;
                    wq[5 * kPairCap + slot] = pairW[0].z;
                    wq[6 * kPairCap + slot] = pairReach[0];
                    wq[7 * kPairCap + slot] = pairW[1].x;
                    wq[8 * kPairCap + slot] = pairW[1].y;
                    wq[9 * kPairCap + slot] = pairW[1].z;
                    wq[10 * kPairCap + slot] = pairReach[1];
                    pairOwner[slot] = lane | ((need[0] ? 1u : 0u) << 8) | ((need[1] ? 1u : 0u) << 9);
                    wqAnswer[0 * 64 + lane] = 0;
                    wqAnswer[1 * 64 + lane] = 0;
                }
                waveLdsFence();
                for (uint32_t e0 = 0; e0 < pairs;) {
                    const uint32_t rem = pairs - e0;
                    const uint32_t units = (rem + 7u) >> 3;
                    const int chunkLog = (units >= 7u) ? 6 : (units >= 4u ? 5 : (units >= 2u ? 4 : 3));
                    const int shift = 6 - chunkLog;
                    const uint32_t mine = lane >> shift;
                    const uint32_t sub = lane & ((1u << shift) - 1u);
                    const bool have = mine < rem;
                    const uint32_t es = have ? e0 + mine : 0u;
                    const vec3 lo = v3(wq[0 * kPairCap + es], wq[1 * kPairCap + es], wq[2 * kPairCap + es]);
                    const vec3 wA = v3(wq[3 * kPairCap + es], wq[4 * kPairCap + es], wq[5 * kPairCap + es]);
                    const float dA = wq[6 * kPairCap + es];
                    const vec3 wB = v3(wq[7 * kPairCap + es], wq[8 * kPairCap + es], wq[9 * kPairCap + es]);
                    const float dB = wq[10 * kPairCap + es];
                    const uint32_t ow = pairOwner[es];
                    const bool liveA = have && ((ow >> 8) & 1u) != 0u, liveB = have && ((ow >> 9) & 1u) != 0u;
                    bool occA, occB;
                    if (shift == 0) pairAnyHit<kBounded, false>(sc, L, lo, wA, dA, liveA, wB, dB, liveB, 0, 0, occA, occB);
                    else pairAnyHit<kBounded, true>(sc, L, lo, wA, dA, liveA, wB, dB, liveB, shift, (int)sub, occA, occB);
                    const unsigned long long verdictsA = __ballot(occA), verdictsB = __ballot(occB);
                    const unsigned long long group = ((1ull << (1u << shift)) - 1ull) << (mine << shift);
                    if (have && sub == 0u) {
                        if ((verdictsA & group) != 0ull) wqAnswer[0 * 64 + (ow & 63u)] = 1;
                        if ((verdictsB & group) != 0ull) wqAnswer[1 * 64 + (ow & 63u)] = 1;
                    }
                    e0 += 1u << chunkLog;
                }
            } else {
            for (uint32_t e0 = 0; e0 < queued;) {
                const uint32_t rem = queued - e0;
                const uint32_t units = (rem + 7u) >> 3;
                const int chunkLog = (units >= 7u || kAccel || kMesh) ? 6 : (units >= 4u ? 5 : (units >= 2u ? 4 : 3));
                const int shift = 6 - chunkLog;
                const uint32_t mine = lane >> shift;
                const uint32_t sub = lane & ((1u << shift) - 1u);
                const bool have = mine < rem;
// ... 385 lines not shown
            }
        }
    }
}

template <bool kMotion>
struct FeatureMotion {};
template <>
struct FeatureMotion<true> {
    const float* prevRecords;
    uint32_t first, count;
    float4* out;
};

template <bool kSceneInLds, bool kMotion = false>
__global__ __launch_bounds__(kBlock) void featureKernel(const float4* __restrict__ sceneBlob, SceneLayout L, TileMap tile, EyeParams eye,
                                                         vec3 defaultColor, float4* __restrict__ out, uint32_t n, FeatureMotion<kMotion> motion) {
    extern __shared__ __attribute__((aligned(256))) float4 lds[];
    const float4* sc;
    if constexpr (kSceneInLds) {
        for (int k = threadIdx.x; k < L.ldsVec4; k += kBlock) lds[k] = sceneBlob[k];
        __syncthreads();
        sc = lds;
    } else {
        sc = sceneBlob;
    }
    for (uint32_t base = blockIdx.x * kBlock; base < n; base += gridDim.x * kBlock) {
        const uint32_t i = base + threadIdx.x;
        const bool live = i < n;
        vec3 d = v3(0, 0, 0);
        if (live) {
            const PixelCoord pc = locate(tile, i);
            const float jitteredX = pc.x + 0.5f;
            const float jitteredY = pc.gy + 0.5f;
            const vec3 start = v3(((jitteredX * eye.invW) - 0.5f) * eye.s,
                                  1 * ((jitteredY * eye.invH) - 0.5f) * eye.s * eye.aspect, 1.0f) *
                               eye.camera.zNear;
            d = normalize(rotate(eye.camera.rotation, start));
        }
        const QueryHit q = closestQuery(sc, sceneBlob, L, eye.camera.position, d, ptm::inf(), live);
        if (live) {
            vec3 albedo = defaultColor;
            if (q.kind != 0) albedo = xyz(loadRow16(sc + L.offMaterial + 5 * q.materialIdx));
            float4* f = out + 2 * (size_t)i;
            f[0] = float4{q.normal.x, q.normal.y, q.normal.z, q.dist};
            f[1] = float4{albedo.x, albedo.y, albedo.z, asF((uint32_t)q.materialIdx)};
            if constexpr (kMotion) {
                const ptmo::Motion m = ptmo::pixelMotion(d, eye.camera.position, q.kind, q.prim, q.dist, q.w1, q.w2, motion.prevRecords,
                                                         motion.first, motion.count);
                motion.out[i] = float4{m.prevPoint.x, m.prevPoint.y, m.prevPoint.z, asF((uint32_t)m.surface)};
            }
        }
    }
}

template <bool kSceneInLds>
__global__ __launch_bounds__(kBlock) void specularFeatureKernel(const float4* __restrict__ sceneBlob, SceneLayout L, TileMap tile, EyeParams eye,
                                                                 vec3 defaultColor, float4* __restrict__ out, uint32_t* __restrict__ steps, uint32_t n,
                                                                 int maxSteps) {
    extern __shared__ __attribute__((aligned(256))) float4 lds[];
    const float4* sc;
    if constexpr (kSceneInLds) {
        for (int k = threadIdx.x; k < L.ldsVec4; k += kBlock) lds[k] = sceneBlob[k];
        __syncthreads();
        sc = lds;
    } else {
        sc = sceneBlob;
    }
    for (uint32_t base = blockIdx.x * kBlock; base < n; base += gridDim.x * kBlock) {
        const uint32_t i = base + threadIdx.x;
        const bool inFrame = i < n;
        vec3 o = eye.camera.position, d = v3(0, 0, 0);
        if (inFrame) {
            const PixelCoord pc = locate(tile, i);
            const float jitteredX = pc.x + 0.5f;
            const float jitteredY = pc.gy + 0.5f;
            const vec3 start = v3(((jitteredX * eye.invW) - 0.5f) * eye.s,
                                  1 * ((jitteredY * eye.invH) - 0.5f) * eye.s * eye.aspect, 1.0f) *
                               eye.camera.zNear;
            d = normalize(rotate(eye.camera.rotation, start));
        }
        bool live = inFrame;
        vec3 normal = v3(0, 0, 0);
        float depth = ptm::inf();
        int materialIdx = -1;
        bool hit = false;
        uint32_t taken = 0;
        for (int k = 0; k <= maxSteps; ++k) {
            if (!waveAny(live)) break;
            const QueryHit q = closestQuery(sc, sceneBlob, L, o, d, ptm::inf(), live);
            if (live) {
                live = false;
                hit = q.kind != 0;
                if (!hit) {
                    normal = v3(0, 0, 0);
                    depth = ptm::inf();
                    materialIdx = -1;
                } else {
                    normal = q.normal;
                    depth = (k == 0) ? q.dist : depth + q.dist;
                    materialIdx = q.materialIdx;
                    if (k < maxSteps) {
                        const float4* mat = sc + L.offMaterial + 5 * q.materialIdx;
                        const float4 misc = loadRow16(mat + 4);
                        const ptsp::Material m{loadRow16(mat).w, loadRow16(mat + 1).w, loadRow16(mat + 2).w, misc.x, misc.y, (int)asU(misc.z)};
                        const ptsp::Step s = ptsp::step(m, d, q.point, q.normal);
                        if (s.follows) {
                            o = s.o;
                            d = s.d;
                            ++taken;
                            live = true;
                        }
                    }
                }
            }
        }
        if (inFrame) {
            vec3 albedo = defaultColor;
            if (hit) albedo = xyz(loadRow16(sc + L.offMaterial + 5 * materialIdx));
            float4* f = out + 2 * (size_t)i;
            f[0] = float4{normal.x, normal.y, normal.z, depth};
            f[1] = float4{albedo.x, albedo.y, albedo.z, asF((uint32_t)materialIdx)};
            if (steps) steps[i] = taken;
        }
    }
}

static inline unsigned blocksFor(uint32_t n, unsigned block) { return (n + block - 1) / block; }

hipError_t launchRngInit(hipStream_t st, uint32_t* rngHome, uint32_t plane, uint32_t samples, TileMap tile, uint64_t seed,
                         const uint32_t* jumpTable) {
    hipLaunchKernelGGL(rngInitKernel, dim3(blocksFor(plane * samples, 256)), dim3(256), 0, st, rngHome, plane, samples, tile, seed,
                       jumpTable);
    return hipGetLastError();
}

hipError_t launchDisplay(hipStream_t st, const FrameBuffers& fb) {
    hipLaunchKernelGGL(displayKernel, dim3(blocksFor(fb.numPixels, 256)), dim3(256), 0, st, fb);
    return hipGetLastError();
}

hipError_t launchClear(hipStream_t st, const FrameBuffers& fb) {
    hipLaunchKernelGGL(clearKernel, dim3(blocksFor(fb.numPixels, 256)), dim3(256), 0, st, fb);
    return hipGetLastError();
}

hipError_t launchPrimaryPrep(hipStream_t st, float4* sceneBlob, const SceneLayout& layout, ptss_vec3 origin) {
    const int n = layout.numSpheres > layout.numTriangles ? layout.numSpheres : layout.numTriangles;
    if (n <= 0) return hipSuccess;
    hipLaunchKernelGGL(primaryPrepKernel, dim3(blocksFor((uint32_t)n, 64)), dim3(64), 0, st, sceneBlob, layout, origin);
    return hipGetLastError();
}

#if PTSS_DIAG
hipError_t readDiagCounters(unsigned long long* out8) { return hipMemcpyFromSymbol(out8, HIP_SYMBOL(g_diag), 64); }
#endif
static_assert(sizeof(float4) == kVec4Bytes, "bounceLdsBytes counts rows of float4");

enum SceneVariant : int { kVariantAccel, kVariantBoundedPairs, kVariantBounded, kVariantPlain, kVariantMesh, kNumVariants };
constexpr int kNumFrameVariants = kVariantMesh;
constexpr bool kVariantArgs[kNumVariants][4] = {{true, false, false, false}, {false, true, true, false}, {false, true, false, false},
                                                {false, false, false, false}, {false, false, false, true}};

static SceneVariant sceneVariant(const SceneLayout& layout, bool bounded) {
    if (meshImage(layout)) return kVariantMesh;
    if (layout.accelSpheres) return kVariantAccel;
    if (bounded && layout.neePairs) return kVariantBoundedPairs;
    return bounded ? kVariantBounded : kVariantPlain;
}

using KernelFn = void (*)(FrameBuffers, const float4*, SceneLayout, int, TileMap, EyeParams);

template <size_t... I>
constexpr std::array<KernelFn, sizeof...(I)> bounceTable(std::index_sequence<I...>) {
    return {{bounceKernel<(I & 4) != 0, (I & 2) != 0, (I & 1) != 0, kVariantArgs[I / 8][0], kVariantArgs[I / 8][1], kVariantArgs[I / 8][2],
                          kVariantArgs[I / 8][3]>...}};
}
template <size_t... V>
constexpr std::array<KernelFn, sizeof...(V)> frameTable(std::index_sequence<V...>) {
    return {{frameKernel<kVariantArgs[V][0], kVariantArgs[V][1], kVariantArgs[V][2]>...}};
}
static int bounceIndex(SceneVariant v, bool last, bool sceneInLds, bool first) { return v * 8 + last * 4 + sceneInLds * 2 + first; }
static KernelFn bounceKernelFor(int index) {
    static constexpr auto table = bounceTable(std::make_index_sequence<kNumVariants * 8>{});
    return table[index];
}
static KernelFn frameKernelFor(SceneVariant v) {
    static constexpr auto table = frameTable(std::make_index_sequence<kNumFrameVariants>{});
    return v < kNumFrameVariants ? table[v] : nullptr;
}
static int blocksPerCU(KernelFn k, size_t lds) {
    int a = 0;
    return hipOccupancyMaxActiveBlocksPerMultiprocessor(&a, k, kBlock, lds) == hipSuccess ? a : 0;
}

constexpr int kKernelBitRanges[][2] = {
    {PTSS_KERNEL_BOUNCE, PTSS_KERNEL_WIDTH_BOUNCE},       {PTSS_KERNEL_FRAME, PTSS_KERNEL_WIDTH_FRAME},
    {PTSS_KERNEL_BOUNCE_MESH, PTSS_KERNEL_WIDTH_BOUNCE_MESH}, {PTSS_KERNEL_QUERY, PTSS_KERNEL_WIDTH_QUERY},
    {PTSS_KERNEL_FEATURES, PTSS_KERNEL_WIDTH_FEATURES},   {PTSS_KERNEL_DENOISE, PTSS_KERNEL_WIDTH_DENOISE},
    {PTSS_KERNEL_UPDATE, PTSS_KERNEL_WIDTH_UPDATE},       {PTSS_KERNEL_REFIT, PTSS_KERNEL_WIDTH_REFIT},
    {PTSS_KERNEL_REPROJECT, PTSS_KERNEL_WIDTH_REPROJECT}, {PTSS_KERNEL_FEATURES_MOTION, PTSS_KERNEL_WIDTH_FEATURES_MOTION},
    {PTSS_KERNEL_REPROJECT_MOTION, PTSS_KERNEL_WIDTH_REPROJECT_MOTION}};
constexpr bool kernelBitRangesDisjoint() {
    unsigned long long taken = 0;
    for (const auto& r : kKernelBitRanges) {
        if (r[0] < 0 || r[1] < 1 || r[0] + r[1] > 64) return false;
        const unsigned long long bits = (r[1] == 64 ? ~0ull : (1ull << r[1]) - 1ull) << r[0];
        if (taken & bits) return false;
        taken |= bits;
    }
    return true;
}
static_assert(kernelBitRangesDisjoint(), "two kernels share a bit of ptss_launched_kernels, or a range leaves the 64-bit word");
static_assert(kNumFrameVariants * 8 == PTSS_KERNEL_WIDTH_BOUNCE && kNumFrameVariants == PTSS_KERNEL_WIDTH_FRAME &&
                  (kNumVariants - kNumFrameVariants) * 8 == PTSS_KERNEL_WIDTH_BOUNCE_MESH,
              "the bounce and frame tables fill their bit ranges");

hipError_t launchBounce(hipStream_t st, const FrameBuffers& fb, const float4* sceneBlob, SceneLayout layout, int bounce,
                        bool isLast, bool sceneInLds, bool bounded, int gridBlocks, TileMap tile, EyeParams eye, unsigned long long* launched) {
    const int index = bounceIndex(sceneVariant(layout, bounded), isLast, sceneInLds, bounce == 0);
    hipLaunchKernelGGL(bounceKernelFor(index), dim3(gridBlocks), dim3(kBlock), bounceLdsBytes(layout, sceneInLds), st, fb, sceneBlob, layout, bounce,
                       tile, eye);
    const hipError_t e = hipGetLastError();
    const bool mesh = index >= kVariantMesh * 8;
    if (e == hipSuccess) markLaunched(launched, mesh ? PTSS_KERNEL_BOUNCE_MESH : PTSS_KERNEL_BOUNCE, mesh ? index - kVariantMesh * 8 : index);
    return e;
}

hipError_t launchFrame(hipStream_t st, const FrameBuffers& fb, const float4* sceneBlob, SceneLayout layout, int numBounces, bool bounded, int gridBlocks,
                       TileMap tile, EyeParams eye, unsigned long long* launched) {
    const SceneVariant v = sceneVariant(layout, bounded);
    if (!frameKernelFor(v)) return hipErrorInvalidValue;
    hipLaunchKernelGGL(frameKernelFor(v), dim3(gridBlocks), dim3(kBlock), bounceLdsBytes(layout, true), st, fb, sceneBlob, layout, numBounces, tile, eye);
    const hipError_t e = hipGetLastError();
    if (e == hipSuccess) markLaunched(launched, PTSS_KERNEL_FRAME, v);
    return e;
}
int frameOccupancyBlocksPerCU(const SceneLayout& layout, bool bounded) {
    const KernelFn k = frameKernelFor(sceneVariant(layout, bounded));
    return k ? blocksPerCU(k, bounceLdsBytes(layout, true)) : 0;
}

hipError_t launchQuery(hipStream_t st, bool any, const float4* sceneBlob, SceneLayout layout, bool sceneInLds, const void* rays, void* out,
                       uint32_t n, int maxBlocks, unsigned long long* launched) {
    using QueryFn = void (*)(const float4*, SceneLayout, const float4*, float4*, uint32_t);
    static constexpr QueryFn table[4] = {queryKernel<false, false>, queryKernel<false, true>, queryKernel<true, false>, queryKernel<true, true>};
    const int index = (any ? 2 : 0) + (sceneInLds ? 1 : 0);
    unsigned blocks = blocksFor(n, kBlock);
    if (maxBlocks > 0 && blocks > (unsigned)maxBlocks) blocks = (unsigned)maxBlocks;
    const size_t lds = sceneInLds ? (size_t)layout.ldsVec4 * sizeof(float4) : 0;
    hipLaunchKernelGGL(table[index], dim3(blocks), dim3(kBlock), lds, st, sceneBlob, layout, static_cast<const float4*>(rays),
                       static_cast<float4*>(out), n);
    const hipError_t e = hipGetLastError();
    if (e == hipSuccess) markLaunched(launched, PTSS_KERNEL_QUERY, index);
    return e;
}

template <bool kMotion>
static hipError_t launchFeatureKernel(hipStream_t st, const float4* sceneBlob, SceneLayout layout, bool sceneInLds, TileMap tile, EyeParams eye,
                                      ptss_vec3 defaultColor, void* out, uint32_t n, int maxBlocks, FeatureMotion<kMotion> motion,
                                      unsigned long long* launched) {
    unsigned blocks = blocksFor(n, kBlock);
    if (maxBlocks > 0 && blocks > (unsigned)maxBlocks) blocks = (unsigned)maxBlocks;
    const size_t lds = sceneInLds ? (size_t)layout.ldsVec4 * sizeof(float4) : 0;
    const auto kernel = sceneInLds ? featureKernel<true, kMotion> : featureKernel<false, kMotion>;
    hipLaunchKernelGGL(kernel, dim3(blocks), dim3(kBlock), lds, st, sceneBlob, layout, tile, eye, defaultColor, static_cast<float4*>(out), n, motion);
    const hipError_t e = hipGetLastError();
    if (e == hipSuccess) markLaunched(launched, kMotion ? PTSS_KERNEL_FEATURES_MOTION : PTSS_KERNEL_FEATURES, sceneInLds ? 1 : 0);
    return e;
}

hipError_t launchFeatures(hipStream_t st, const float4* sceneBlob, SceneLayout layout, bool sceneInLds, TileMap tile, EyeParams eye,
                          ptss_vec3 defaultColor, void* out, uint32_t n, int maxBlocks, unsigned long long* launched) {
    return launchFeatureKernel<false>(st, sceneBlob, layout, sceneInLds, tile, eye, defaultColor, out, n, maxBlocks, {}, launched);
}

hipError_t launchFeaturesMotion(hipStream_t st, const float4* sceneBlob, SceneLayout layout, bool sceneInLds, TileMap tile, EyeParams eye,
                                ptss_vec3 defaultColor, void* out, uint32_t n, int maxBlocks, const void* prevRecords, uint32_t first,
                                uint32_t count, void* motionOut, unsigned long long* launched) {
    return launchFeatureKernel<true>(st, sceneBlob, layout, sceneInLds, tile, eye, defaultColor, out, n, maxBlocks,
                                     {static_cast<const float*>(prevRecords), first, count, static_cast<float4*>(motionOut)}, launched);
}

hipError_t launchFeaturesSpecular(hipStream_t st, const float4* sceneBlob, SceneLayout layout, bool sceneInLds, TileMap tile, EyeParams eye,
                                  ptss_vec3 defaultColor, void* out, void* steps, uint32_t n, int maxSteps, int maxBlocks,
                                  unsigned long long* launches) {
    unsigned blocks = blocksFor(n, kBlock);
    if (maxBlocks > 0 && blocks > (unsigned)maxBlocks) blocks = (unsigned)maxBlocks;
    const size_t lds = sceneInLds ? (size_t)layout.ldsVec4 * sizeof(float4) : 0;
    const auto kernel = sceneInLds ? specularFeatureKernel<true> : specularFeatureKernel<false>;
    hipLaunchKernelGGL(kernel, dim3(blocks), dim3(kBlock), lds, st, sceneBlob, layout, tile, eye, defaultColor, static_cast<float4*>(out),
                       static_cast<uint32_t*>(steps), n, maxSteps);
    const hipError_t e = hipGetLastError();
    if (e == hipSuccess) ++launches[sceneInLds ? 1 : 0];
    return e;
}

hipError_t launchFlush(hipStream_t st, const FrameBuffers& fb, int numBounces, const FlushTargets& targets) {
    hipLaunchKernelGGL(flushKernel, dim3(1), dim3(kMinLiveRays), 0, st, fb, numBounces, targets);
    return hipGetLastError();
}

int bounceOccupancyBlocksPerCU(const SceneLayout& layout, bool sceneInLds, bool bounded) {
    return blocksPerCU(bounceKernelFor(bounceIndex(sceneVariant(layout, bounded), false, sceneInLds, false)), bounceLdsBytes(layout, sceneInLds));
}

// ... 2 lines not shown
```

### cuda-path-tracer-ss_amd/host/host_capi.cpp

```cpp
#include "ptss_host.h"

#include <cstdio>
#include <cstring>
#include <new>
#include <vector>

#include "HostOps.h"
#include "Scene.h"
#include "ptdenoise.h"
#include "ptreproject.h"
#include "ptupsample.h"
#include "ptmotion.h"
#include "ptspecular.h"
#include "ptquant.h"
#include "ptlocate.h"
#include "ptmesh.h"
#include "ptorder.h"
#include "ptpack.h"
#include "pttri.h"
#include "xorwow.h"

struct ptss_scene {
    Scene scene;
};

namespace {
using namespace ptv;
template <int kC1, int kC2>
void triangleForm(const float* t, const float* o3, const float* d3, float limit, bool primary, float* out) {
    const vec3 v0 = v3(t[0], t[1], t[2]), e1 = v3(t[3], t[4], t[5]), e2 = v3(t[6], t[7], t[8]);
    const vec3 o = v3(o3[0], o3[1], o3[2]), d = v3(d3[0], d3[1], d3[2]);
    pttri::Head h;
    if (primary) {
        const vec3 s = o - v0, r = cross(s, e1);
        h = pttri::head<kC1, kC2, true>(v0, e1, e2, s, r, dot(e2, r), o, d);
    } else {
        h = pttri::head<kC1, kC2, false>(v0, e1, e2, v3(0, 0, 0), v3(0, 0, 0), 0.0f, o, d);
    }
    float b0 = 0, b1 = 0, b2 = 0;
    const bool pass = pttri::passesHead(h, limit);
    if (pass) pttri::weights<kC1, kC2>(h, d, b0, b1, b2);
    out[0] = (pass && pttri::passesWeights(b0, b1, b2)) ? 1.0f : 0.0f;
    out[1] = h.dist;
    out[2] = b0;
    out[3] = b1;
    out[4] = b2;
    out[5] = h.det;
}
}

extern "C" {

int ptss_scene_create(const char* preset, ptss_scene** out) {
    if (!preset || !out) return PTSS_HOST_EINVAL;
    ptss_scene* s = new (std::nothrow) ptss_scene();
    if (!s) return PTSS_HOST_EINVAL;
    if (!s->scene.buildPreset(preset)) {
        delete s;
        return PTSS_HOST_EINVAL;
    }
    *out = s;
    return PTSS_HOST_OK;
}

void ptss_scene_destroy(ptss_scene* s) { delete s; }

int ptss_scene_describe(const ptss_scene* s, ptss_scene_desc* out) {
    if (!s || !out) return PTSS_HOST_EINVAL;
    *out = s->scene.desc();
    return PTSS_HOST_OK;
}

int ptss_scene_add_obj(ptss_scene* s, const char* path, const float* m, int materialIdx, size_t* added) {
    if (!s || !path || materialIdx < 0 || (size_t)materialIdx >= s->scene.materialsVec.size()) return PTSS_HOST_EINVAL;
    mat4 t = mat4::identity();
    if (m)
        for (int r = 0; r < 4; ++r)
            for (int c = 0; c < 4; ++c) t.c[c][r] = m[4 * r + c];
    const long n = s->scene.addObjModel(path, t, materialIdx);
    if (n < 0) return n == -2 ? PTSS_HOST_EIO : PTSS_HOST_EINVAL;
    if (added) *added = (size_t)n;
    return PTSS_HOST_OK;
}

int ptss_camera_default(ptss_camera* out) {
    if (!out) return PTSS_HOST_EINVAL;
    *out = Camera();
    return PTSS_HOST_OK;
}

int ptss_camera_ray(const ptss_camera* cam, int width, int height, int x, int y, float jx, float jy, ptss_ray_query* out) {
    if (!cam || !out || width <= 0 || height <= 0) return PTSS_HOST_EINVAL;
    *out = cameraRay(*cam, width, height, x, y, jx, jy);
    return PTSS_HOST_OK;
}

int ptss_camera_move(ptss_camera* cam, unsigned char key, int* moved) {
    if (!cam) return PTSS_HOST_EINVAL;
    Camera c;
    static_cast<ptss_camera&>(c) = *cam;
    const bool m = moveCamera(c, key);
    *cam = c;
    if (moved) *moved = m ? 1 : 0;
    return PTSS_HOST_OK;
}

int ptss_write_tga(const char* filename, const ptss_uchar4* rgba, int width, int height) {
    if (!filename || !rgba || width <= 0 || height <= 0) return PTSS_HOST_EINVAL;
    return writeTga(filename, rgba, width, height) ? PTSS_HOST_OK : PTSS_HOST_EIO;
}

int ptss_tile_rows(int height, int band_rows, int rank, int world, int* rows, int cap) {
    if (height < 0 || band_rows <= 0 || world <= 0 || rank < 0 || rank >= world) return PTSS_HOST_EINVAL;
    int n = 0;
    for (int y = 0; y < height; ++y) {
        if ((y / band_rows) % world != rank) continue;
        if (rows && n < cap) rows[n] = y;
        ++n;
    }
    return n;
}

int ptss_probe_guard(int op, const float* x, unsigned int* out, size_t n) {
    if (!x || !out || op < 0 || op > 3) return PTSS_HOST_EINVAL;
    for (size_t i = 0; i < n; ++i) {
        switch (op) {
            case 0: out[i] = ptm::fast_numerator(x[i]) ? 1u : 0u; break;
            case 1: out[i] = ptm::fast_divisor(x[i]) ? 1u : 0u; break;
            case 2: out[i] = ptm::fast_rcp_operand(x[i]) ? 1u : 0u; break;
            default: out[i] = ptm::in_light_window(x[i]) ? 1u : 0u; break;
        }
    }
    return PTSS_HOST_OK;
}

int ptss_probe_guard_constants(float* out9) {
    if (!out9) return PTSS_HOST_EINVAL;
    const float k[9] = {ptm::kSqrtLo, ptm::kSqrtHi, ptm::kRcpLo, ptm::kRcpHi, ptm::kDivLo, ptm::kDivHi, ptm::kLightD2Lo, ptm::kLightD2Hi,
                        ptm::kFourPi};
    for (int i = 0; i < 9; ++i) out9[i] = k[i];
    return PTSS_HOST_OK;
}

int ptss_probe_scene_guard_flags(const ptss_scene_desc* scene, unsigned int* out) {
    if (!scene || !out) return PTSS_HOST_EINVAL;
    *out = ptpack::sceneGuardFlags(*scene);
    return PTSS_HOST_OK;
}

int ptss_probe_math(int op, const float* x, const float* y, float* out, size_t n) {
    if (!x || !out) return PTSS_HOST_EINVAL;
    for (size_t i = 0; i < n; ++i) {
        float s, c;
        switch (op) {
            case 0: ptm::sincos(x[i], s, c); out[i] = s; break;
            case 1: ptm::sincos(x[i], s, c); out[i] = c; break;
            case 2: out[i] = ptm::tan(x[i]); break;
            case 3: out[i] = ptm::atan(x[i]); break;
            case 4: out[i] = ptm::log(x[i]); break;
            case 5: out[i] = ptm::exp(x[i]); break;
            case 6: if (!y) return PTSS_HOST_EINVAL; out[i] = ptm::pow(x[i], y[i]); break;
            case 7: out[i] = ptm::sqrt(x[i]); break;
            default: return PTSS_HOST_EINVAL;
        }
    }
    return PTSS_HOST_OK;
}

int ptss_probe_triangle_forms(const float* tri9, const float* o3, const float* d3, const float* limit, int primary, size_t n, int* cls,
                              float* general6, float* classed6) {
    if (!tri9 || !o3 || !d3 || !limit || !cls || !general6 || !classed6) return PTSS_HOST_EINVAL;
    for (size_t i = 0; i < n; ++i) {
        const float* t = tri9 + 9 * i;
        const int c = pttri::triangleClass(v3(t[3], t[4], t[5]), v3(t[6], t[7], t[8]));
        cls[i] = c;
        triangleForm<0, 0>(t, o3 + 3 * i, d3 + 3 * i, limit[i], primary != 0, general6 + 6 * i);
        float* out = classed6 + 6 * i;
        switch (c) {
#define PTSS_TRI_CASE(c1, c2) \
    case (c1) * 4 + (c2): triangleForm<c1, c2>(t, o3 + 3 * i, d3 + 3 * i, limit[i], primary != 0, out); break;
            PTSS_TRI_CASE(0, 1) PTSS_TRI_CASE(0, 2) PTSS_TRI_CASE(0, 3)
            PTSS_TRI_CASE(1, 0) PTSS_TRI_CASE(1, 2) PTSS_TRI_CASE(1, 3)
            PTSS_TRI_CASE(2, 0) PTSS_TRI_CASE(2, 1) PTSS_TRI_CASE(2, 3)
            PTSS_TRI_CASE(3, 0) PTSS_TRI_CASE(3, 1) PTSS_TRI_CASE(3, 2)
#undef PTSS_TRI_CASE
            default: triangleForm<0, 0>(t, o3 + 3 * i, d3 + 3 * i, limit[i], primary != 0, out); break;
        }
    }
    return PTSS_HOST_OK;
}

int ptss_probe_wave_locate(int width, int rank, int world, int bandRows, unsigned int firstBegin, size_t n, int* wave3, int* lane3, int* fast) {
    if (!wave3 || !lane3 || !fast || width <= 0 || bandRows <= 0 || world <= 0 || rank < 0 || rank >= world) return PTSS_HOST_EINVAL;
    for (size_t i = 0; i < n; ++i) {
        const uint32_t first = firstBegin + (uint32_t)i;
        const ptloc::WaveOrigin w = ptloc::waveOrigin(width, rank, world, bandRows, first);
        fast[i] = w.oneWrap ? 1 : 0;
        for (uint32_t k = 0; k < ptloc::kStrip; ++k) {
            const ptloc::Coord ref = ptloc::locate(width, rank, world, bandRows, first + k);
            const ptloc::Coord got = w.oneWrap ? ptloc::laneCoord(w, width, k) : ref;
            int* a = wave3 + 3 * (i * ptloc::kStrip + k);
            int* b = lane3 + 3 * (i * ptloc::kStrip + k);
            a[0] = got.x; a[1] = got.gy; a[2] = (int)got.globalIndex;
            b[0] = ref.x; b[1] = ref.gy; b[2] = (int)ref.globalIndex;
        }
    }
    return PTSS_HOST_OK;
}

int ptss_probe_quantize(const float* x, unsigned int* out, size_t n) {
    if (!x || !out) return PTSS_HOST_EINVAL;
    for (size_t i = 0; i < n; ++i) out[i] = ptq::quantize_literal(x[i]);
    return PTSS_HOST_OK;
}

int ptss_probe_quant_table(float* out257) {
    if (!out257) return PTSS_HOST_EINVAL;
    float T[ptq::kTableFloats];
    if (!ptq::build_thresholds(T)) return PTSS_HOST_EINVAL;
    for (int k = 0; k <= 256; ++k) out257[k] = T[k];
    return PTSS_HOST_OK;
}

static const uint32_t* jumpTable() {
    static std::vector<uint32_t> table;
    if (table.empty()) {
        table.resize(ptrng::kJumpTableWords);
        ptrng::build_subsequence_table(table.data());
    }
    return table.data();
}

int ptss_probe_mesh_bound(const float* tri9, size_t ntri, const float* o3, const float* d3, size_t n, float margin, int* out, float* bound12) {
    if (!tri9 || ntri == 0 || ntri > (1u << 20) || (n && (!o3 || !d3 || !out))) return PTSS_HOST_EINVAL;
    float b[12];
    ptmesh::buildBound(tri9, (int)ntri, b);
    if (bound12)
        for (int k = 0; k < 12; ++k) bound12[k] = b[k];
    for (size_t i = 0; i < n; ++i) {
        const vec3 o = v3(o3[3 * i], o3[3 * i + 1], o3[3 * i + 2]), d = v3(d3[3 * i], d3[3 * i + 1], d3[3 * i + 2]);
        out[i] = ptmesh::mayTouch(v3(b[0], b[1], b[2]), b[3], v3(b[4], b[5], b[6]), b[7], b[8], b[9], b[10], b[11], o, d, margin) ? 1 : 0;
    }
    return PTSS_HOST_OK;
}

int ptss_probe_mesh_refit(const float* tri9, size_t ntri, float* bounds12) {
    if (!tri9 || !bounds12 || ntri == 0 || ntri > (1u << 20)) return PTSS_HOST_EINVAL;
    const size_t leaves = (ntri + 15) / 16, groups = (leaves + 15) / 16;
    for (size_t k = 0; k < leaves; ++k)
        ptmesh::refitBound(tri9 + 9 * 16 * k, (int)(ntri - 16 * k < 16 ? ntri - 16 * k : 16), 16, bounds12 + 12 * k);
    for (size_t g = 0; g < groups; ++g)
        ptmesh::refitBound(tri9 + 9 * 256 * g, (int)(ntri - 256 * g < 256 ? ntri - 256 * g : 256), ptmesh::kRefitSlots, bounds12 + 12 * (leaves + g));
    return PTSS_HOST_OK;
}

static int probeKdOrder(const ptss_triangle* triangles, size_t n, int* position, bool canonicalZero) {
    if (!triangles || !position || n == 0 || n > (1u << 20)) return PTSS_HOST_EINVAL;
    std::vector<float> v(9 * n);
    for (size_t i = 0; i < n; ++i) {
        const ptss_vec3* p[3] = {&triangles[i].vertex0, &triangles[i].vertex1, &triangles[i].vertex2};
        for (int k = 0; k < 3; ++k) { v[9 * i + 3 * k] = p[k]->x; v[9 * i + 3 * k + 1] = p[k]->y; v[9 * i + 3 * k + 2] = p[k]->z; }
    }
    ptorder::kdPositions(v.data(), (int)n, position, canonicalZero);
    return PTSS_HOST_OK;
}
int ptss_probe_kd_order(const ptss_triangle* triangles, size_t n, int* position) { return probeKdOrder(triangles, n, position, true); }
int ptss_probe_kd_order_signed_zero(const ptss_triangle* triangles, size_t n, int* position) { return probeKdOrder(triangles, n, position, false); }

int ptss_probe_mesh_touch(const float* b, const float* o3, const float* d3, size_t n, float margin, int* out) {
    if (!b || (n && (!o3 || !d3 || !out))) return PTSS_HOST_EINVAL;
    for (size_t i = 0; i < n; ++i) {
        const vec3 o = v3(o3[3 * i], o3[3 * i + 1], o3[3 * i + 2]), d = v3(d3[3 * i], d3[3 * i + 1], d3[3 * i + 2]);
        out[i] = ptmesh::mayTouch(v3(b[0], b[1], b[2]), b[3], v3(b[4], b[5], b[6]), b[7], b[8], b[9], b[10], b[11], o, d, margin) ? 1 : 0;
    }
    return PTSS_HOST_OK;
}

int ptss_probe_pack_scene(const ptss_scene_desc* scene, int everySphereLoop, int image, int* numImages, int* inLds, void* layout,
                          size_t layoutBytes, float* blob, size_t blobCapacity, size_t* blobWords) {
    if (!scene || ptpack::validateScene(*scene) || (everySphereLoop != 0 && everySphereLoop != 1)) return PTSS_HOST_EINVAL;
    const int n = ptpack::planImages(*scene, everySphereLoop != 0).numImages;
    if (numImages) *numImages = n;
    if (image < 0 || image >= n || (layout && layoutBytes != sizeof(ptss::SceneLayout))) return PTSS_HOST_EINVAL;
    if (!layout && !blob && !inLds && !blobWords) return PTSS_HOST_OK;
    std::vector<ptpack::PackedImage> images;
    try {
        images = ptpack::packImages(*scene, everySphereLoop != 0);
    } catch (const std::bad_alloc&) {
        return PTSS_HOST_EINVAL;
    }
    const ptpack::PackedImage& im = images[(size_t)image];
    const size_t words = im.blob.size() * 4;
    if (inLds) *inLds = im.inLds ? 1 : 0;
    if (layout) std::memcpy(layout, &im.layout, sizeof(im.layout));
    if (blobWords) *blobWords = words;
    if (blob) {
        if (blobCapacity < words) return PTSS_HOST_EINVAL;
        std::memcpy(blob, im.blob.data(), words * sizeof(float));
    }
    return PTSS_HOST_OK;
}

static int denoiseColours(std::vector<vec3> (&plane)[2], const ptss_pixel_feature* features, int width, int height, const ptss_denoise_params* params,
                          unsigned char* out_rgba, float* out_float) {
    const size_t n = (size_t)width * (size_t)height;
    auto featureAt = [&](int q) { return ptdn::Feature{features[q].normal, features[q].depth, features[q].materialIdx}; };
    auto depthAt = [&](int q) { return features[q].depth; };
    int cur = 0;
    for (int i = 0; i < params->levels; ++i) {
        const ptdn::Level lv = ptdn::levelOf(*params, i);
        const std::vector<vec3>& src = plane[cur];
        std::vector<vec3>& dst = plane[1 - cur];
        dst.resize(n);
        auto colourAt = [&](int q) { return src[(size_t)q]; };
        for (int y = 0; y < height; ++y)
            for (int x = 0; x < width; ++x) dst[(size_t)y * width + x] = ptdn::filterPixel(x, y, width, height, lv, colourAt, featureAt, depthAt);
        cur = 1 - cur;
    }
    for (size_t p = 0; p < n; ++p) {
        const vec3 v = plane[cur][p];
        if (out_float) { out_float[3 * p] = v.x; out_float[3 * p + 1] = v.y; out_float[3 * p + 2] = v.z; }
        if (out_rgba) { out_rgba[4 * p] = ptdn::toByte(v.x); out_rgba[4 * p + 1] = ptdn::toByte(v.y); out_rgba[4 * p + 2] = ptdn::toByte(v.z); out_rgba[4 * p + 3] = 255; }
    }
    return PTSS_HOST_OK;
}

static bool denoiseArgumentsOk(const void* input, const ptss_pixel_feature* features, int width, int height, const ptss_denoise_params* params) {
    if (!input || !features || !params || width <= 0 || height <= 0) return false;
    if (params->structSize != (unsigned int)sizeof(ptss_denoise_params) || params->levels < 0 || params->levels > PTSS_DENOISE_MAX_LEVELS)
        return false;
    return params->sigmaColor > 0.0f && params->sigmaNormal > 0.0f && params->sigmaDepth >= 0.0f;
}

int ptss_probe_denoise(const uint32_t* accum, float inverseTicks, const ptss_pixel_feature* features, int width, int height,
                       const ptss_denoise_params* params, unsigned char* out_rgba, float* out_float) {
    if (!denoiseArgumentsOk(accum, features, width, height, params)) return PTSS_HOST_EINVAL;
    const size_t n = (size_t)width * (size_t)height;
    std::vector<vec3> plane[2];
    plane[0].resize(n);
    for (size_t p = 0; p < n; ++p) plane[0][p] = ptdn::displayValue(accum[3 * p], accum[3 * p + 1], accum[3 * p + 2], inverseTicks);
    return denoiseColours(plane, features, width, height, params, out_rgba, out_float);
}

int ptss_probe_denoise_history(const ptss_history_entry* history, const ptss_pixel_feature* features, int width, int height,
                               const ptss_denoise_params* params, unsigned char* out_rgba, float* out_float) {
    if (!denoiseArgumentsOk(history, features, width, height, params)) return PTSS_HOST_EINVAL;
    const size_t n = (size_t)width * (size_t)height;
    std::vector<vec3> plane[2];
    plane[0].resize(n);
    for (size_t p = 0; p < n; ++p) plane[0][p] = v3(history[p].r, history[p].g, history[p].b);
    return denoiseColours(plane, features, width, height, params, out_rgba, out_float);
}

int ptss_probe_upsample(const unsigned char* lo_rgba, const ptss_pixel_feature* features_lo, int width, int height,
                        const ptss_pixel_feature* features_hi, const ptss_upsample_params* params, unsigned char* out_rgba, float* out_float4) {
    if (!lo_rgba || !features_lo || !features_hi || !out_rgba || width <= 0 || height <= 0) return PTSS_HOST_EINVAL;
    if (ptup::paramsError(params) || out_rgba == lo_rgba) return PTSS_HOST_EINVAL;
    const int f = params->factor;
    if ((unsigned long long)width * (unsigned long long)height * (unsigned long long)(f * f) >= (1ull << 31)) return PTSS_HOST_EINVAL;
// ... 152 lines not shown
```

### cuda-path-tracer-ss_amd/ptss.py

```python
import ctypes as C
import os

import numpy as np

from ptss_types import (KERNEL_BITS, PATH_RESULT_DTYPE, PATH_RNG_DTYPE, SCENE_LAYOUT_FIELDS, SCENE_LAYOUT_MESH_FIELDS, AreaLight, Camera, DenoiseParams,
                        HistoryEntry, Material, PixelFeature, PixelMotion, PointLight, RayHit, RayQuery, ReprojectParams, SceneDesc, Sphere, Triangle,
                        UChar4, UpsampleParams, Vec3, struct_to_dict)

_HERE = os.path.dirname(os.path.abspath(__file__))
LIBDIR = os.path.join(_HERE, "lib")
HOST_LIB = os.path.join(LIBDIR, "libptss_host.so")
DEVICE_LIB = os.path.join(LIBDIR, os.environ.get("PTSS_LIBNAME", "libptss.so"))

_u32p = C.POINTER(C.c_uint32)
_f32p = C.POINTER(C.c_float)


class PtssError(RuntimeError):
    pass


class RenderConfig(C.Structure):
    _fields_ = [("structSize", C.c_uint), ("width", C.c_int), ("height", C.c_int), ("seed", C.c_ulonglong), ("maxIterations", C.c_uint),
                ("device", C.c_int), ("tileRank", C.c_int), ("tileWorld", C.c_int), ("bandRows", C.c_int),
                ("syncEachFrame", C.c_int), ("floatAccumulator", C.c_int), ("timeKernels", C.c_int),
                ("samplesPerPass", C.c_int), ("everySphereLoop", C.c_int), ("frameLanes", C.c_int),
                ("lanesFreeRun", C.c_int), ("oneLaunchFrames", C.c_int)]


KERNEL_VARIANTS = ("accel", "bounded+pairs", "bounded", "plain")


def _bounce(variant, j):
    return ("bounce", variant, bool(j & 4), bool(j & 2), bool(j & 1))


_KERNEL_NAMES = {
    "BOUNCE": lambda j: _bounce(KERNEL_VARIANTS[j // 8], j % 8),
    "FRAME": lambda j: ("frame", KERNEL_VARIANTS[j]),
    "BOUNCE_MESH": lambda j: _bounce("mesh", j),
    "QUERY": lambda j: ("query", "any" if j & 2 else "closest", bool(j & 1)),
    "FEATURES": lambda j: ("features", bool(j)),
    "DENOISE": lambda j: ("denoise",),
    "UPDATE": lambda j: ("update",),
    "REFIT": lambda j: ("refit",),
    "REPROJECT": lambda j: ("reproject",),
    "FEATURES_MOTION": lambda j: ("features_motion", bool(j)),
    "REPROJECT_MOTION": lambda j: ("reproject_motion",),
}
KERNEL_OF_BIT = {base + j: _KERNEL_NAMES[rng](j) for rng, (base, width) in KERNEL_BITS.items() for j in range(width)}


def _kernels_of(*ranges):
    return {KERNEL_OF_BIT[KERNEL_BITS[r][0] + j] for r in ranges for j in range(KERNEL_BITS[r][1])}


def decode_launched_kernels(mask):
    return {name for bit, name in KERNEL_OF_BIT.items() if mask >> bit & 1}


def all_kernels():
    return _kernels_of("BOUNCE", "FRAME")


def mesh_kernels():
    return _kernels_of("BOUNCE_MESH")


def query_kernels():
    return _kernels_of("QUERY")


def feature_kernels():
    return _kernels_of("FEATURES")


def reproject_kernels():
    return _kernels_of("REPROJECT")


def motion_kernels():
    return _kernels_of("FEATURES_MOTION", "REPROJECT_MOTION")


_host = None
_dev = None
_hip = None


def _hip_lib():
    global _hip
    if _hip is None:
        device_lib()
        L = C.CDLL("libamdhip64.so.7", mode=C.RTLD_GLOBAL)
        L.hipMalloc.argtypes = [C.POINTER(C.c_void_p), C.c_size_t]
        L.hipFree.argtypes = [C.c_void_p]
        L.hipMemcpy.argtypes = [C.c_void_p, C.c_void_p, C.c_size_t, C.c_int]
        L.hipSetDevice.argtypes = [C.c_int]
        L.hipDeviceSynchronize.argtypes = []
        _hip = L
    return _hip


def _hip_check(rc, what):
    if rc != 0:
        raise PtssError(f"{what} failed (hipError {rc})")


def host_lib():
    global _host
    if _host is None:
        if not os.path.exists(HOST_LIB):
            raise PtssError(f"{HOST_LIB} missing: run `python __graft_entry__.py build` first")
        L = C.CDLL(HOST_LIB)
        L.ptss_scene_create.argtypes = [C.c_char_p, C.POINTER(C.c_void_p)]
        L.ptss_scene_destroy.argtypes = [C.c_void_p]
        L.ptss_scene_destroy.restype = None
        L.ptss_scene_describe.argtypes = [C.c_void_p, C.POINTER(SceneDesc)]
        L.ptss_camera_default.argtypes = [C.POINTER(Camera)]
        L.ptss_camera_move.argtypes = [C.POINTER(Camera), C.c_ubyte, C.POINTER(C.c_int)]
        L.ptss_write_tga.argtypes = [C.c_char_p, C.c_void_p, C.c_int, C.c_int]
        L.ptss_tile_rows.argtypes = [C.c_int, C.c_int, C.c_int, C.c_int, C.POINTER(C.c_int), C.c_int]
        L.ptss_probe_math.argtypes = [C.c_int, _f32p, _f32p, _f32p, C.c_size_t]
        L.ptss_probe_quantize.argtypes = [_f32p, C.POINTER(C.c_uint), C.c_size_t]
        L.ptss_probe_guard.argtypes = [C.c_int, _f32p, C.POINTER(C.c_uint), C.c_size_t]
        L.ptss_probe_guard_constants.argtypes = [_f32p]
        L.ptss_probe_scene_guard_flags.argtypes = [C.POINTER(SceneDesc), C.POINTER(C.c_uint)]
        L.ptss_probe_triangle_forms.argtypes = [_f32p, _f32p, _f32p, _f32p, C.c_int, C.c_size_t, C.POINTER(C.c_int), _f32p, _f32p]
        L.ptss_probe_quant_table.argtypes = [_f32p]
        L.ptss_probe_wave_locate.argtypes = [C.c_int, C.c_int, C.c_int, C.c_int, C.c_uint, C.c_size_t, C.POINTER(C.c_int), C.POINTER(C.c_int),
                                             C.POINTER(C.c_int)]
        L.ptss_probe_rng_init.argtypes = [C.c_ulonglong, C.c_uint, _u32p]
        L.ptss_scene_add_obj.argtypes = [C.c_void_p, C.c_char_p, _f32p, C.c_int, C.POINTER(C.c_size_t)]
        L.ptss_probe_mesh_bound.argtypes = [_f32p, C.c_size_t, _f32p, _f32p, C.c_size_t, C.c_float, C.POINTER(C.c_int), _f32p]
        L.ptss_probe_rng_draw.argtypes = [_u32p, _u32p, _f32p, C.c_size_t]
        L.ptss_probe_rng_jump_table.argtypes = [_u32p, C.c_size_t]
        L.ptss_camera_ray.argtypes = [C.POINTER(Camera), C.c_int, C.c_int, C.c_int, C.c_int, C.c_float, C.c_float, C.POINTER(RayQuery)]
        L.ptss_probe_mesh_refit.argtypes = [_f32p, C.c_size_t, _f32p]
        L.ptss_probe_mesh_touch.argtypes = [_f32p, _f32p, _f32p, C.c_size_t, C.c_float, C.POINTER(C.c_int)]
        L.ptss_probe_kd_order.argtypes = [C.c_void_p, C.c_size_t, C.POINTER(C.c_int)]
        L.ptss_probe_kd_order_signed_zero.argtypes = [C.c_void_p, C.c_size_t, C.POINTER(C.c_int)]
        L.ptss_probe_pack_scene.argtypes = [C.POINTER(SceneDesc), C.c_int, C.c_int, C.POINTER(C.c_int), C.POINTER(C.c_int), C.c_void_p,
                                            C.c_size_t, _f32p, C.c_size_t, C.POINTER(C.c_size_t)]
        L.ptss_probe_denoise.argtypes = [_u32p, C.c_float, C.c_void_p, C.c_int, C.c_int, C.POINTER(DenoiseParams), C.c_void_p, _f32p]
        L.ptss_probe_denoise_history.argtypes = [C.c_void_p, C.c_void_p, C.c_int, C.c_int, C.POINTER(DenoiseParams), C.c_void_p, _f32p]
        L.ptss_probe_reproject.argtypes = [_u32p, C.c_float, C.c_int, C.POINTER(Camera), C.POINTER(Camera), C.c_int, C.c_int, C.c_void_p,
                                           C.c_void_p, C.c_void_p, C.POINTER(ReprojectParams), C.c_void_p]
        L.ptss_probe_reproject_motion.argtypes = [_u32p, C.c_float, C.c_int, C.POINTER(Camera), C.POINTER(Camera), C.c_int, C.c_int, C.c_void_p,
                                                  C.c_void_p, C.c_void_p, C.c_void_p, C.POINTER(ReprojectParams), C.c_void_p]
        L.ptss_probe_upsample.argtypes = [C.c_void_p, C.c_void_p, C.c_int, C.c_int, C.c_void_p, C.POINTER(UpsampleParams), C.c_void_p, _f32p]
        L.ptss_probe_upsample_axis.argtypes = [C.c_int, C.c_int, C.POINTER(C.c_int), C.POINTER(C.c_int), _f32p]
        L.ptss_probe_motion.argtypes = [C.c_void_p, C.c_void_p, C.c_size_t, C.c_void_p, C.c_size_t, C.c_size_t, C.c_size_t, C.c_void_p]
        L.ptss_probe_specular_step.argtypes = [C.c_void_p, C.c_void_p, C.c_size_t, C.c_void_p, C.c_size_t, C.c_void_p, C.POINTER(C.c_int)]
        L.ptss_probe_specular_class.argtypes = [C.c_void_p]
        _host = L
    return _host


def _torch_first():
    import sys
    torch = sys.modules.get("torch")
    if torch is None:
        return
    try:
        if torch.cuda.is_available() and not torch.cuda.is_initialized():
            torch.cuda.init()
    except Exception as e:
        raise PtssError("torch is imported but torch.cuda could not be initialised before libptss.so's HIP runtime "
                        f"(INTEGRATION.md §5, two HIP runtimes in one process): {e}")


def device_lib():
    global _dev
    _torch_first()
    if _dev is None:
        if not os.path.exists(DEVICE_LIB):
            raise PtssError(f"{DEVICE_LIB} missing: the HIP extension was not built (no CPU fallback exists)")
        L = C.CDLL(DEVICE_LIB)
        vp = C.c_void_p
        L.ptss_default_config.argtypes = [C.POINTER(RenderConfig)]
        L.ptss_create.argtypes = [C.POINTER(SceneDesc), C.POINTER(RenderConfig), C.POINTER(vp)]
        L.ptss_destroy.argtypes = [vp]
        L.ptss_generate_frame.argtypes = [vp, vp, C.c_int]
        L.ptss_set_camera.argtypes = [vp, C.POINTER(Camera)]
        L.ptss_get_camera.argtypes = [vp, C.POINTER(Camera)]
        L.ptss_request_reset.argtypes = [vp]
        L.ptss_set_mode.argtypes = [vp, C.c_int]
        L.ptss_set_max_iterations.argtypes = [vp, C.c_uint]
        L.ptss_set_stream.argtypes = [vp, vp]
        L.ptss_bind_accumulator.argtypes = [vp, vp]
        L.ptss_accumulator_devptr.argtypes = [vp, C.POINTER(vp)]
        L.ptss_float_accumulator_devptr.argtypes = [vp, C.POINTER(vp)]
        L.ptss_alloc_pixels.argtypes = [vp, C.POINTER(vp)]
        L.ptss_free_pixels.argtypes = [vp, vp]
        L.ptss_local_pixels.argtypes = [vp, C.POINTER(C.c_size_t)]
        L.ptss_local_rows.argtypes = [vp, C.POINTER(C.c_int), C.c_int, C.POINTER(C.c_int)]
        L.ptss_read_accumulator.argtypes = [vp, _u32p, C.c_size_t]
        L.ptss_read_float_accumulator.argtypes = [vp, _f32p, C.c_size_t]
        L.ptss_read_pixels.argtypes = [vp, vp, vp, C.c_size_t]
        L.ptss_read_rng_state.argtypes = [vp, C.c_size_t, _u32p]
        L.ptss_read_rng_state_lane.argtypes = [vp, C.c_size_t, C.c_uint, _u32p]
        L.ptss_synchronize.argtypes = [vp]
        L.ptss_last_pass_ms.argtypes = [vp, _f32p]
        L.ptss_samples_since_reset.argtypes = [vp, C.POINTER(C.c_int)]
        L.ptss_live_counts.argtypes = [vp, _u32p, C.c_int, C.POINTER(C.c_int)]
        L.ptss_total_ray_bounces.argtypes = [vp, C.POINTER(C.c_ulonglong)]
        L.ptss_frame_lanes.argtypes = [vp, C.POINTER(C.c_int)]
        L.ptss_one_launch_frames.argtypes = [vp, C.POINTER(C.c_int)]
        L.ptss_guard_timeouts.argtypes = [vp, C.POINTER(C.c_uint)]
        L.ptss_bounce_kernel_time.argtypes = [vp, C.POINTER(C.c_double), C.POINTER(C.c_ulonglong)]
        L.ptss_launched_kernels.argtypes = [vp, C.POINTER(C.c_ulonglong)]
        L.ptss_guard_flags.argtypes = [vp, C.POINTER(C.c_uint)]
        L.ptss_debug_counters.argtypes = [vp, C.POINTER(C.c_ulonglong)]
        L.ptss_triangle_leaves.argtypes = [vp, C.POINTER(C.c_int)]
        L.ptss_intersect.argtypes = [vp, vp, vp, C.c_size_t, vp]
        L.ptss_occluded.argtypes = [vp, vp, vp, C.c_size_t, vp]
        L.ptss_render_features.argtypes = [vp, vp, vp]
        L.ptss_default_denoise_params.argtypes = [C.POINTER(DenoiseParams)]
        L.ptss_denoise.argtypes = [vp, vp, C.POINTER(DenoiseParams), vp, vp]
        L.ptss_read_denoise_plane.argtypes = [vp, _f32p, C.c_size_t, C.POINTER(C.c_int)]
        L.ptss_default_reproject_params.argtypes = [C.POINTER(ReprojectParams)]
        L.ptss_reproject.argtypes = [vp, vp, C.POINTER(Camera), vp, vp, C.POINTER(ReprojectParams), vp, vp]
        L.ptss_denoise_history.argtypes = [vp, vp, vp, C.POINTER(DenoiseParams), vp, vp]
        L.ptss_render_features_motion.argtypes = [vp, vp, C.c_size_t, C.c_size_t, vp, vp, vp]
        L.ptss_reproject_motion.argtypes = [vp, vp, vp, C.POINTER(Camera), vp, vp, C.POINTER(ReprojectParams), vp, vp]
        L.ptss_render_features_specular.argtypes = [vp, C.c_int, vp, vp, vp]
        L.ptss_specular_feature_launches.argtypes = [vp, C.POINTER(C.c_ulonglong)]
        L.ptss_seed_path_rng.argtypes = [vp, vp, C.c_size_t, C.c_ulonglong, C.c_ulonglong, C.c_uint, vp]
        L.ptss_trace_paths.argtypes = [vp, vp, vp, vp, C.c_size_t, C.c_uint, vp]
        L.ptss_path_launches.argtypes = [vp, C.POINTER(C.c_ulonglong)]
        L.ptss_render_features_scaled.argtypes = [vp, C.c_int, vp, vp]
        L.ptss_default_upsample_params.argtypes = [C.POINTER(UpsampleParams)]
        L.ptss_upsample.argtypes = [vp, vp, vp, vp, C.POINTER(UpsampleParams), vp, vp, vp]
        L.ptss_upsample_launches.argtypes = [vp, C.POINTER(C.c_ulonglong)]
        L.ptss_set_scene.argtypes = [vp, C.POINTER(SceneDesc)]
        L.ptss_update_triangles.argtypes = [vp, vp, C.c_size_t, C.c_size_t, vp]
        L.ptss_update_rejected.argtypes = [vp, C.POINTER(C.c_ulonglong)]
        L.ptss_resort_triangles.argtypes = [vp, vp]
        L.ptss_resort_launches.argtypes = [vp, C.POINTER(C.c_ulonglong)]
        L.ptss_reseed.argtypes = [vp, C.c_ulonglong]
        L.ptss_read_triangle_bounds.argtypes = [vp, _f32p, C.c_size_t]
        L.ptss_read_triangle_positions.argtypes = [vp, C.POINTER(C.c_int), C.c_size_t]
        L.ptss_error_string.argtypes = [C.c_int]
        L.ptss_error_string.restype = C.c_char_p
        L.ptss_last_error_detail.restype = C.c_char_p
        _dev = L
    return _dev


def _check(rc):
    if rc != 0:
        L = device_lib()
        raise PtssError(f"ptss error {rc} ({L.ptss_error_string(rc).decode()}): {L.ptss_last_error_detail().decode()}")


class Scene:

    def __init__(self, preset="default"):
        self._h = C.c_void_p()
        rc = host_lib().ptss_scene_create(preset.encode(), C.byref(self._h))
        if rc != 0:
            raise PtssError(f"unknown scene preset {preset!r}")
        self.preset = preset
        self.desc = SceneDesc()
        host_lib().ptss_scene_describe(self._h, C.byref(self.desc))
        self.desc._owner = self

    def add_obj(self, path, transform=None, material=0):
        m = None
        if transform is not None:
            t = np.ascontiguousarray(np.asarray(transform, dtype=np.float32).reshape(4, 4))
            m = t.ctypes.data_as(_f32p)
        added = C.c_size_t()
        rc = host_lib().ptss_scene_add_obj(self._h, os.fsencode(path), m, int(material), C.byref(added))
        if rc != 0:
            raise PtssError(f"add_obj({path!r}) failed: {'cannot read the file' if rc == -2 else 'malformed OBJ or bad argument'} ({rc})")
        owner = self
        self.desc = SceneDesc()
        host_lib().ptss_scene_describe(self._h, C.byref(self.desc))
        self.desc._owner = owner
        return added.value

    def __del__(self):
        if getattr(self, "_h", None) and self._h.value and host_lib is not None:
            host_lib().ptss_scene_destroy(self._h)
            self._h = C.c_void_p()

    def _arr(self, ptr, n):
        return [ptr[i] for i in range(n)]

    @property
    def spheres(self):
        return self._arr(self.desc.spheres, self.desc.numSpheres)

    @property
    def triangles(self):
        return self._arr(self.desc.triangles, self.desc.numTriangles)

    @property
    def materials(self):
        return self._arr(self.desc.materials, self.desc.numMaterials)

    @property
    def area_lights(self):
        return self._arr(self.desc.areaLights, self.desc.numAreaLights)

    @property
    def point_lights(self):
        return self._arr(self.desc.pointLights, self.desc.numPointLights)

    def table(self):
        return {
            "spheres": [struct_to_dict(s) for s in self.spheres],
            "triangles": [struct_to_dict(s) for s in self.triangles],
            "materials": [struct_to_dict(s) for s in self.materials],
            "pointLights": [struct_to_dict(s) for s in self.point_lights],
            "areaLights": [struct_to_dict(s) for s in self.area_lights],
        }


def probe_mesh_bound(tris, origins, directions, margin=1.0):
    t = np.ascontiguousarray(np.asarray(tris, dtype=np.float32).reshape(-1, 9))
    o = np.ascontiguousarray(np.asarray(origins, dtype=np.float32).reshape(-1, 3))
    d = np.ascontiguousarray(np.asarray(directions, dtype=np.float32).reshape(-1, 3))
    out = np.zeros(len(o), dtype=np.int32)
    bound = np.zeros(12, dtype=np.float32)
    rc = host_lib().ptss_probe_mesh_bound(t.ctypes.data_as(_f32p), len(t), o.ctypes.data_as(_f32p), d.ctypes.data_as(_f32p), len(o),
                                          float(margin), out.ctypes.data_as(C.POINTER(C.c_int)), bound.ctypes.data_as(_f32p))
    if rc != 0:
        raise PtssError(f"ptss_probe_mesh_bound: {rc}")
    return out, bound


def probe_mesh_refit(tris):
    t = np.ascontiguousarray(np.asarray(tris, dtype=np.float32).reshape(-1, 9))
    leaves = (len(t) + 15) // 16
    out = np.zeros((leaves + (leaves + 15) // 16, 12), dtype=np.float32)
    rc = host_lib().ptss_probe_mesh_refit(t.ctypes.data_as(_f32p), len(t), out.ctypes.data_as(_f32p))
    if rc != 0:
        raise PtssError(f"ptss_probe_mesh_refit: {rc}")
    return out


def probe_kd_order(triangles, signed_zero=False):
    a = np.ascontiguousarray(triangles, dtype=TRIANGLE_DTYPE).reshape(-1)
    out = np.empty(len(a), dtype=np.int32)
    L = host_lib()
    fn = L.ptss_probe_kd_order_signed_zero if signed_zero else L.ptss_probe_kd_order
    rc = fn(a.ctypes.data, len(a), out.ctypes.data_as(C.POINTER(C.c_int)))
    if rc != 0:
        raise PtssError(f"ptss_probe_kd_order: {rc}")
    return out


def probe_mesh_touch(bound, origins, directions, margin=1.0):
    b = np.ascontiguousarray(np.asarray(bound, dtype=np.float32).reshape(12))
    o = np.ascontiguousarray(np.asarray(origins, dtype=np.float32).reshape(-1, 3))
    d = np.ascontiguousarray(np.asarray(directions, dtype=np.float32).reshape(-1, 3))
    out = np.zeros(len(o), dtype=np.int32)
    rc = host_lib().ptss_probe_mesh_touch(b.ctypes.data_as(_f32p), o.ctypes.data_as(_f32p), d.ctypes.data_as(_f32p), len(o), float(margin),
                                          out.ctypes.data_as(C.POINTER(C.c_int)))
    if rc != 0:
        raise PtssError(f"ptss_probe_mesh_touch: {rc}")
    return out


def probe_pack_scene_images(scene, every_sphere_loop=False):
    n = C.c_int()
    rc = host_lib().ptss_probe_pack_scene(C.byref(scene.desc), 1 if every_sphere_loop else 0, 0, C.byref(n), None, None, 0, None, 0, None)
    if rc != 0:
        raise PtssError(f"ptss_probe_pack_scene: {rc}")
    return n.value


def probe_pack_scene(scene, every_sphere_loop=False, image=0):
    every = 1 if every_sphere_loop else 0
    raw = np.zeros(len(SCENE_LAYOUT_FIELDS), dtype=np.int32)
    in_lds, words = C.c_int(), C.c_size_t()
    blob = np.empty(1 << 16, dtype=np.float32)
    for _ in range(2):
        rc = host_lib().ptss_probe_pack_scene(C.byref(scene.desc), every, int(image), None, C.byref(in_lds), raw.ctypes.data_as(C.c_void_p),
                                              raw.nbytes, blob.ctypes.data_as(_f32p), blob.size, C.byref(words))
        if rc == 0 or words.value <= blob.size:
            break
        blob = np.empty(words.value, dtype=np.float32)
    if rc != 0:
        raise PtssError(f"ptss_probe_pack_scene: {rc}")
    layout = {name: int(v) for name, v in zip(SCENE_LAYOUT_FIELDS, raw)}
    layout.update({f"triClassPack{k}": layout[f"triClassPack{k}"] & 0xFFFFFFFF for k in range(5)})
    layout.update({name: layout[f"triClassPack{k}"] for k, name in enumerate(SCENE_LAYOUT_MESH_FIELDS)})
    return layout, blob[:words.value].reshape(-1, 4).copy(), bool(in_lds.value)


# ... 90 lines not shown

def probe_upsample(lo_rgba, features_lo, width, height, features_hi, params):
    a = np.ascontiguousarray(lo_rgba, dtype=np.uint8).reshape(-1, 4)
    fl = np.ascontiguousarray(features_lo, dtype=FEATURE_DTYPE).reshape(-1)
    fh = np.ascontiguousarray(features_hi, dtype=FEATURE_DTYPE).reshape(-1)
    n_hi = width * height * params.factor * params.factor
    if len(a) != width * height or len(fl) != width * height or len(fh) != n_hi:
        raise ValueError("lo_rgba and features_lo must hold width * height pixels, features_hi factor^2 times as many")
    rgba = np.empty((n_hi, 4), dtype=np.uint8)
    flt = np.empty(n_hi, dtype=HISTORY_DTYPE)
    rc = host_lib().ptss_probe_upsample(a.ctypes.data_as(C.c_void_p), fl.ctypes.data_as(C.c_void_p), width, height, fh.ctypes.data_as(C.c_void_p),
                                        C.byref(params), rgba.ctypes.data_as(C.c_void_p), flt.ctypes.data_as(_f32p))
    if rc != 0:
        raise PtssError(f"ptss_probe_upsample: {rc}")
    return rgba, flt


def default_reproject_params(**overrides):
    p = ReprojectParams()
    _check(device_lib().ptss_default_reproject_params(C.byref(p)))
    for k, v in overrides.items():
        if v is not None:
            setattr(p, k, v)
    return p


def probe_reproject(accum, inverse_ticks, n, camera_now, camera_prev, width, height, features_now, features_prev, history_prev, params=None):
    a = np.ascontiguousarray(accum, dtype=np.uint32).reshape(-1, 3)
    fn = np.ascontiguousarray(features_now, dtype=FEATURE_DTYPE).reshape(-1)
    if len(a) != width * height or len(fn) != width * height:
        raise ValueError("accum and features_now must hold width * height pixels")
    fp = hp = None
    if history_prev is not None:
        fp = np.ascontiguousarray(features_prev, dtype=FEATURE_DTYPE).reshape(-1)
        hp = np.ascontiguousarray(history_prev, dtype=HISTORY_DTYPE).reshape(-1)
        if len(fp) != width * height or len(hp) != width * height:
            raise ValueError("features_prev and history_prev must hold width * height pixels")
    out = np.empty(len(a), dtype=HISTORY_DTYPE)
    rc = host_lib().ptss_probe_reproject(a.ctypes.data_as(_u32p), float(inverse_ticks), int(n), C.byref(camera_now),
                                         C.byref(camera_prev) if camera_prev is not None else None, width, height,
                                         fn.ctypes.data_as(C.c_void_p), fp.ctypes.data_as(C.c_void_p) if fp is not None else None,
                                         hp.ctypes.data_as(C.c_void_p) if hp is not None else None,
                                         C.byref(params if params is not None else default_reproject_params()), out.ctypes.data_as(C.c_void_p))
    if rc != 0:
        raise PtssError(f"ptss_probe_reproject: {rc}")
    return out


def probe_reproject_motion(accum, inverse_ticks, n, camera_now, camera_prev, width, height, features_now, motion_now, features_prev,
                           history_prev, params=None):
    a = np.ascontiguousarray(accum, dtype=np.uint32).reshape(-1, 3)
    fn = np.ascontiguousarray(features_now, dtype=FEATURE_DTYPE).reshape(-1)
    mn = np.ascontiguousarray(motion_now, dtype=MOTION_DTYPE).reshape(-1)
    if len(a) != width * height or len(fn) != width * height or len(mn) != width * height:
        raise ValueError("accum, features_now and motion_now must hold width * height pixels")
    fp = hp = None
    if history_prev is not None:
        fp = np.ascontiguousarray(features_prev, dtype=FEATURE_DTYPE).reshape(-1)
        hp = np.ascontiguousarray(history_prev, dtype=HISTORY_DTYPE).reshape(-1)
        if len(fp) != width * height or len(hp) != width * height:
            raise ValueError("features_prev and history_prev must hold width * height pixels")
    out = np.empty(len(a), dtype=HISTORY_DTYPE)
    rc = host_lib().ptss_probe_reproject_motion(a.ctypes.data_as(_u32p), float(inverse_ticks), int(n), C.byref(camera_now),
                                                C.byref(camera_prev) if camera_prev is not None else None, width, height,
                                                fn.ctypes.data_as(C.c_void_p), mn.ctypes.data_as(C.c_void_p),
                                                fp.ctypes.data_as(C.c_void_p) if fp is not None else None,
                                                hp.ctypes.data_as(C.c_void_p) if hp is not None else None,
                                                C.byref(params if params is not None else default_reproject_params()),
                                                out.ctypes.data_as(C.c_void_p))
    if rc != 0:
        raise PtssError(f"ptss_probe_reproject_motion: {rc}")
    return out


def probe_motion(rays, hits, prev_triangles=None, first=0, num_triangles=0):
    r = np.ascontiguousarray(rays)
    r = (r.view(np.float32) if r.dtype == RAY_DTYPE else r.astype(np.float32, copy=False)).reshape(-1, 8)
    r = np.ascontiguousarray(r)
    h = np.ascontiguousarray(hits, dtype=HIT_DTYPE).reshape(-1)
    if len(r) != len(h):
        raise ValueError("one hit per ray")
    t = np.ascontiguousarray(prev_triangles, dtype=TRIANGLE_DTYPE).reshape(-1) if prev_triangles is not None else None
    out = np.empty(len(h), dtype=MOTION_DTYPE)
    rc = host_lib().ptss_probe_motion(r.ctypes.data_as(C.c_void_p), h.ctypes.data_as(C.c_void_p), len(h),
                                      t.ctypes.data_as(C.c_void_p) if t is not None and len(t) else None, int(first),
                                      len(t) if t is not None else 0, int(num_triangles), out.ctypes.data_as(C.c_void_p))
    if rc != 0:
        raise PtssError(f"ptss_probe_motion: {rc}")
    return out


SPECULAR_CLASSES = ("terminal", "transmit", "mirror")


def _material_table(materials):
    if hasattr(materials, "numMaterials"):
        return C.cast(materials.materials, C.c_void_p), int(materials.numMaterials), materials
    arr = (Material * max(len(materials), 1))(*materials)
    return C.cast(arr, C.c_void_p), len(materials), arr


def specular_class(material):
    return SPECULAR_CLASSES[host_lib().ptss_probe_specular_class(C.byref(material))]


def probe_specular_step(rays, hits, materials):
    r = np.ascontiguousarray(rays)
    r = (r.view(np.float32) if r.dtype == RAY_DTYPE else r.astype(np.float32, copy=False)).reshape(-1, 8)
    r = np.ascontiguousarray(r)
    h = np.ascontiguousarray(hits, dtype=HIT_DTYPE).reshape(-1)
    if len(r) != len(h):
        raise ValueError("one hit per ray")
    ptr, count, keep = _material_table(materials)
    nxt = r.copy()
    follows = np.zeros(len(h), dtype=np.int32)
    rc = host_lib().ptss_probe_specular_step(r.ctypes.data_as(C.c_void_p), h.ctypes.data_as(C.c_void_p), len(h), ptr, count,
                                             nxt.ctypes.data_as(C.c_void_p), follows.ctypes.data_as(C.POINTER(C.c_int)))
    del keep
    if rc != 0:
        raise PtssError(f"ptss_probe_specular_step: {rc}")
    return nxt, follows != 0


def make_rays(origins, directions, tmax=float("inf")):
    o = np.asarray(origins, dtype=np.float32).reshape(-1, 3)
    d = np.asarray(directions, dtype=np.float32).reshape(-1, 3)
    if o.shape != d.shape:
        raise ValueError("origins and directions differ in shape")
    out = np.zeros((o.shape[0], 8), dtype=np.float32)
    out[:, 0:3], out[:, 4:7] = o, d
    out[:, 3] = np.broadcast_to(np.asarray(tmax, dtype=np.float32), (o.shape[0],))
    return out


def camera_ray(cam, width, height, x, y, jitter=(0.5, 0.5)):
    q = RayQuery()
    rc = host_lib().ptss_camera_ray(C.byref(cam), width, height, x, y, jitter[0], jitter[1], C.byref(q))
    if rc != 0:
        raise PtssError(f"ptss_camera_ray: {rc}")
    return np.frombuffer(bytes(q), dtype=np.float32).copy()


def camera_rays(cam, width, height, jitter=(0.5, 0.5)):
    out = np.empty((width * height, 8), dtype=np.float32)
    q = RayQuery()
    fn, jx, jy, ref_cam, ref_q = host_lib().ptss_camera_ray, C.c_float(jitter[0]), C.c_float(jitter[1]), C.byref(cam), C.byref(q)
    buf = (C.c_float * 8).from_buffer(q)
    for y in range(height):
        for x in range(width):
            if fn(ref_cam, width, height, x, y, jx, jy, ref_q) != 0:
                raise PtssError("ptss_camera_ray failed")
            out[y * width + x] = buf
    return out


def tile_rows(height, band_rows, rank, world):
    n = host_lib().ptss_tile_rows(height, band_rows, rank, world, None, 0)
    if n < 0:
        raise PtssError("bad tile spec")
    rows = (C.c_int * max(n, 1))()
    host_lib().ptss_tile_rows(height, band_rows, rank, world, rows, n)
    return np.array(rows[:n], dtype=np.int64)


def write_tga(path, rgba_hw4):
    a = np.ascontiguousarray(rgba_hw4, dtype=np.uint8)
    h, w = a.shape[:2]
    rc = host_lib().ptss_write_tga(path.encode(), a.ctypes.data_as(C.c_void_p), w, h)
    if rc != 0:
        raise PtssError(f"write_tga failed ({rc})")


class Renderer:

    def __init__(self, scene, width, height, max_iterations=15, seed=0x5EED, device=0, tile_rank=0, tile_world=1,
                 band_rows=8, sync_each_frame=True, float_accumulator=False, time_kernels=False, samples_per_pass=1,
                 every_sphere_loop=False, frame_lanes=0, lanes_free_run=False, one_launch_frames=0):
        L = device_lib()
        cfg = RenderConfig()
        _check(L.ptss_default_config(C.byref(cfg)))
        cfg.width, cfg.height = width, height
        cfg.seed = seed
        cfg.maxIterations = max_iterations
        cfg.device = device
        cfg.tileRank, cfg.tileWorld, cfg.bandRows = tile_rank, tile_world, band_rows
        cfg.syncEachFrame = 1 if sync_each_frame else 0
        cfg.floatAccumulator = 1 if float_accumulator else 0
        cfg.timeKernels = 1 if time_kernels else 0
        cfg.samplesPerPass = samples_per_pass
        cfg.everySphereLoop = 1 if every_sphere_loop else 0
        cfg.frameLanes = frame_lanes
        cfg.lanesFreeRun = 1 if lanes_free_run else 0
        cfg.oneLaunchFrames = one_launch_frames
        self.cfg = cfg
        self._scene = scene
        self._ctx = C.c_void_p()
        _check(L.ptss_create(C.byref(scene.desc), C.byref(cfg), C.byref(self._ctx)))
        n = C.c_size_t()
        _check(L.ptss_local_pixels(self._ctx, C.byref(n)))
        self.local_pixels = n.value
        self.width, self.height = width, height
        self.local_rows = self.local_pixels // width
        self._own_pixels = None
        self._buffers = {}
        self._have_features = False
        self._have_scaled = set()
        self.ticks = 1

    def close(self):
        if self._ctx:
            L = device_lib()
            if self._own_pixels:
                L.ptss_free_pixels(self._ctx, self._own_pixels)
                self._own_pixels = None
            for p in self._buffers.values():
                _hip_lib().hipFree(p)
            self._buffers = {}
            L.ptss_destroy(self._ctx)
            self._ctx = C.c_void_p()

    def __del__(self):
        try:
            self.close()
        except Exception:
            pass

    def pixels_devptr(self):
        if self._own_pixels is None:
            p = C.c_void_p()
            _check(device_lib().ptss_alloc_pixels(self._ctx, C.byref(p)))
            self._own_pixels = p
        return self._own_pixels

    def set_stream(self, raw_stream):
        _check(device_lib().ptss_set_stream(self._ctx, C.c_void_p(raw_stream)))

    def bind_accumulator(self, devptr):
        _check(device_lib().ptss_bind_accumulator(self._ctx, C.c_void_p(devptr)))

    def rows(self):
        cnt = C.c_int()
        rows = (C.c_int * max(self.local_rows, 1))()
        _check(device_lib().ptss_local_rows(self._ctx, rows, self.local_rows, C.byref(cnt)))
        return np.array(rows[:cnt.value], dtype=np.int64)

    def generate_frame(self, dev_pixels=None, ticks=None):
        if ticks is None:
            ticks = self.ticks
            self.ticks += 1
        if dev_pixels is None:
            dev_pixels = self.pixels_devptr()
        elif isinstance(dev_pixels, int):
            dev_pixels = C.c_void_p(dev_pixels)
        _check(device_lib().ptss_generate_frame(self._ctx, dev_pixels, ticks))

    def set_camera(self, cam):
        _check(device_lib().ptss_set_camera(self._ctx, C.byref(cam)))
        self._have_features = False
        self._have_scaled = set()

    def get_camera(self):
        cam = Camera()
        _check(device_lib().ptss_get_camera(self._ctx, C.byref(cam)))
        return cam

    def request_reset(self):
        _check(device_lib().ptss_request_reset(self._ctx))

    def set_mode(self, use_path_tracer):
        _check(device_lib().ptss_set_mode(self._ctx, 1 if use_path_tracer else 0))

    def set_max_iterations(self, n):
        _check(device_lib().ptss_set_max_iterations(self._ctx, n))

    def synchronize(self):
        _check(device_lib().ptss_synchronize(self._ctx))

    def accumulator(self):
        out = np.empty((self.local_pixels, 3), dtype=np.uint32)
        _check(device_lib().ptss_read_accumulator(self._ctx, out.ctypes.data_as(_u32p), out.size))
        return out

    def float_accumulator(self):
        out = np.empty((self.local_pixels, 3), dtype=np.float32)
        _check(device_lib().ptss_read_float_accumulator(self._ctx, out.ctypes.data_as(_f32p), out.size))
        return out

    def pixels(self, dev_pixels=None):
        if dev_pixels is None:
            dev_pixels = self.pixels_devptr()
        elif isinstance(dev_pixels, int):
            dev_pixels = C.c_void_p(dev_pixels)
        out = np.empty((self.local_pixels, 4), dtype=np.uint8)
        _check(device_lib().ptss_read_pixels(self._ctx, dev_pixels, out.ctypes.data_as(C.c_void_p), self.local_pixels))
        return out

    def rng_state(self, local_pixel, lane=0):
        out = np.empty(6, dtype=np.uint32)
        _check(device_lib().ptss_read_rng_state_lane(self._ctx, local_pixel, lane, out.ctypes.data_as(_u32p)))
        return out

    def last_pass_ms(self):
        v = C.c_float()
        _check(device_lib().ptss_last_pass_ms(self._ctx, C.byref(v)))
        return v.value

    def live_counts(self):
        out = (C.c_uint32 * 65)()
        n = C.c_int()
        _check(device_lib().ptss_live_counts(self._ctx, out, 65, C.byref(n)))
        return np.array(out[:n.value], dtype=np.uint32)

    def total_ray_bounces(self):
        v = C.c_ulonglong()
        _check(device_lib().ptss_total_ray_bounces(self._ctx, C.byref(v)))
        return v.value

    @property
    def one_launch_frames(self):
        v = C.c_int()
        _check(device_lib().ptss_one_launch_frames(self._ctx, C.byref(v)))
        return bool(v.value)

    @property
    def frame_lanes(self):
        v = C.c_int()
        _check(device_lib().ptss_frame_lanes(self._ctx, C.byref(v)))
        return v.value

    def guard_timeouts(self):
        v = C.c_uint()
        _check(device_lib().ptss_guard_timeouts(self._ctx, C.byref(v)))
        return v.value

    def launched_kernels(self):
        v = C.c_ulonglong()
        _check(device_lib().ptss_launched_kernels(self._ctx, C.byref(v)))
        return decode_launched_kernels(v.value)

    def guard_flags(self):
        v = C.c_uint()
        _check(device_lib().ptss_guard_flags(self._ctx, C.byref(v)))
        return v.value

    def set_scene(self, scene):
        _check(device_lib().ptss_set_scene(self._ctx, C.byref(scene.desc)))
        self._scene = scene
        self._have_features = False
        self._have_scaled = set()

    def update_triangles(self, triangles, first=0, stream=None):
        L = device_lib()
        if type(triangles).__module__.split(".")[0] == "torch":
            import sys
            torch = sys.modules["torch"]
            if triangles.dtype != torch.float32 or not triangles.is_contiguous() or not triangles.is_cuda or triangles.numel() % 19:
                raise ValueError("triangles: a contiguous float32 device tensor of n x 19 words")
            if stream is None:
                stream = torch.cuda.current_stream(triangles.device).cuda_stream
            _check(L.ptss_update_triangles(self._ctx, C.c_void_p(triangles.data_ptr()), first, triangles.numel() // 19, C.c_void_p(stream)))
        else:
            a = np.ascontiguousarray(triangles, dtype=TRIANGLE_DTYPE).reshape(-1)
            d = self._device_buffer_at_least("triangles_upload", a.nbytes) if len(a) else None
            if len(a):
                _hip_check(_hip_lib().hipMemcpy(d, a.ctypes.data, a.nbytes, 1), "hipMemcpy")
            _check(L.ptss_update_triangles(self._ctx, d, first, len(a), C.c_void_p(stream) if stream else None))
            if len(a):
                if stream:
                    _hip_check(_hip_lib().hipDeviceSynchronize(), "hipDeviceSynchronize")
                self.synchronize()
        self._have_features = False
        self._have_scaled = set()

    def resort_triangles(self, stream=None):
        _check(device_lib().ptss_resort_triangles(self._ctx, C.c_void_p(stream) if stream else None))

    def resort_launches(self):
        v = C.c_ulonglong()
        _check(device_lib().ptss_resort_launches(self._ctx, C.byref(v)))
        return v.value

    def reseed(self, seed):
        _check(device_lib().ptss_reseed(self._ctx, seed))

    def update_rejected(self):
        v = C.c_ulonglong()
        _check(device_lib().ptss_update_rejected(self._ctx, C.byref(v)))
        return v.value

    def triangle_bounds(self):
        leaves = self.triangle_leaves()
        out = np.empty((leaves + (leaves + 15) // 16, 12), dtype=np.float32)
        _check(device_lib().ptss_read_triangle_bounds(self._ctx, out.ctypes.data_as(_f32p), out.size))
        return out

    def triangle_positions(self, count):
        out = np.empty(count, dtype=np.int32)
        _check(device_lib().ptss_read_triangle_positions(self._ctx, out.ctypes.data_as(C.POINTER(C.c_int)), out.size))
        return out

    def intersect(self, rays):
        return self._query(rays, any_hit=False)

    def occluded(self, rays):
        return self._query(rays, any_hit=True)

    def _query(self, rays, any_hit):
        L = device_lib()
        fn = L.ptss_occluded if any_hit else L.ptss_intersect
        if type(rays).__module__.split(".")[0] == "torch":
            import sys
            torch = sys.modules["torch"]
            if rays.dtype != torch.float32 or rays.dim() != 2 or rays.shape[1] != 8 or not rays.is_contiguous() or not rays.is_cuda:
                raise ValueError("rays: a contiguous (N, 8) float32 device tensor")
            n = rays.shape[0]
            out = (torch.empty(n, dtype=torch.int32, device=rays.device) if any_hit
                   else torch.empty((n, 12), dtype=torch.float32, device=rays.device))
            stream = torch.cuda.current_stream(rays.device).cuda_stream
            _check(fn(self._ctx, C.c_void_p(rays.data_ptr()), C.c_void_p(out.data_ptr()), n, C.c_void_p(stream)))
            return out
        a = np.asarray(rays)
        if a.dtype == RAY_DTYPE:
            a = np.ascontiguousarray(a).view(np.float32).reshape(-1, 8)
        a = np.ascontiguousarray(a, dtype=np.float32)
        if a.ndim != 2 or a.shape[1] != 8:
            raise ValueError("rays: (N, 8) float32 or (N,) RAY_DTYPE")
        n = a.shape[0]
        out = np.empty(n, dtype=np.uint32) if any_hit else np.empty(n, dtype=HIT_DTYPE)
        if n == 0:
            return out
        H = _hip_lib()
        _hip_check(H.hipSetDevice(self.cfg.device), "hipSetDevice")
        d_rays, d_out = C.c_void_p(), C.c_void_p()
        _hip_check(H.hipMalloc(C.byref(d_rays), a.nbytes), "hipMalloc")
        try:
            _hip_check(H.hipMalloc(C.byref(d_out), out.nbytes), "hipMalloc")
            _hip_check(H.hipMemcpy(d_rays, a.ctypes.data, a.nbytes, 1), "hipMemcpy")
            _check(fn(self._ctx, d_rays, d_out, n, None))
            self.synchronize()
            _hip_check(H.hipMemcpy(out.ctypes.data, d_out, out.nbytes, 2), "hipMemcpy")
        finally:
            H.hipFree(d_rays)
            if d_out:
                H.hipFree(d_out)
        return out

    def seed_path_rng(self, n, seed, first_sequence=0, skip=0, device=None):
        L = device_lib()
        n = int(n)
        if device is not None:
            import sys
            torch = sys.modules.get("torch")
            if torch is None:
                raise ValueError("device=...: import torch first")
            dev = torch.device("cuda", self.cfg.device) if device is True else torch.device(device)
            out = torch.empty((n, 6), dtype=torch.int32, device=dev)
            stream = torch.cuda.current_stream(dev).cuda_stream
            _check(L.ptss_seed_path_rng(self._ctx, C.c_void_p(out.data_ptr()) if n else None, n, seed, first_sequence, skip, C.c_void_p(stream)))
            return out
        out = np.empty(n, dtype=PATH_RNG_DTYPE)
        if n == 0:
            _check(L.ptss_seed_path_rng(self._ctx, None, 0, seed, first_sequence, skip, None))
            return out
        H = _hip_lib()
        _hip_check(H.hipSetDevice(self.cfg.device), "hipSetDevice")
        d = C.c_void_p()
        _hip_check(H.hipMalloc(C.byref(d), out.nbytes), "hipMalloc")
        try:
            _check(L.ptss_seed_path_rng(self._ctx, d, n, seed, first_sequence, skip, None))
            self.synchronize()
            _hip_check(H.hipMemcpy(out.ctypes.data, d, out.nbytes, 2), "hipMemcpy")
        finally:
            H.hipFree(d)
        return out

    def trace_paths(self, rays, rng, max_iterations):
        L = device_lib()
        if type(rays).__module__.split(".")[0] == "torch":
            import sys
            torch = sys.modules["torch"]
            if rays.dtype != torch.float32 or rays.dim() != 2 or rays.shape[1] != 8 or not rays.is_contiguous() or not rays.is_cuda:
                raise ValueError("rays: a contiguous (N, 8) float32 device tensor")
            n = rays.shape[0]
            if (type(rng).__module__.split(".")[0] != "torch" or rng.dtype != torch.int32 or tuple(rng.shape) != (n, 6) or not rng.is_contiguous() or
                    rng.device != rays.device):
                raise ValueError("rng: a contiguous (N, 6) int32 tensor on the rays' device")
            out = torch.empty((n, 4), dtype=torch.float32, device=rays.device)
            stream = torch.cuda.current_stream(rays.device).cuda_stream
            _check(L.ptss_trace_paths(self._ctx, C.c_void_p(rays.data_ptr()), C.c_void_p(rng.data_ptr()), C.c_void_p(out.data_ptr()), n,
                                      int(max_iterations), C.c_void_p(stream)))
            return out
        a = np.asarray(rays)
        if a.dtype == RAY_DTYPE:
            a = np.ascontiguousarray(a).view(np.float32).reshape(-1, 8)
        a = np.ascontiguousarray(a, dtype=np.float32)
        if a.ndim != 2 or a.shape[1] != 8:
            raise ValueError("rays: (N, 8) float32 or (N,) RAY_DTYPE")
        n = a.shape[0]
        s = np.asarray(rng)
        if s.dtype == PATH_RNG_DTYPE:
            s = np.ascontiguousarray(s).view(np.uint32).reshape(-1, 6)
        s = np.ascontiguousarray(s, dtype=np.uint32)
        if s.shape != (n, 6):
            raise ValueError("rng: (N,) PATH_RNG_DTYPE or (N, 6) uint32, one state per ray")
        out = np.empty(n, dtype=PATH_RESULT_DTYPE)
        after = np.empty(n, dtype=PATH_RNG_DTYPE)
        if n == 0:
            _check(L.ptss_trace_paths(self._ctx, None, None, None, 0, int(max_iterations), None))
            return out, after
        H = _hip_lib()
        _hip_check(H.hipSetDevice(self.cfg.device), "hipSetDevice")
        bufs = [C.c_void_p(), C.c_void_p(), C.c_void_p()]
        try:
            for b, nbytes in zip(bufs, (a.nbytes, s.nbytes, out.nbytes)):
                _hip_check(H.hipMalloc(C.byref(b), nbytes), "hipMalloc")
            _hip_check(H.hipMemcpy(bufs[0], a.ctypes.data, a.nbytes, 1), "hipMemcpy")
            _hip_check(H.hipMemcpy(bufs[1], s.ctypes.data, s.nbytes, 1), "hipMemcpy")
            _check(L.ptss_trace_paths(self._ctx, bufs[0], bufs[1], bufs[2], n, int(max_iterations), None))
            self.synchronize()
            _hip_check(H.hipMemcpy(out.ctypes.data, bufs[2], out.nbytes, 2), "hipMemcpy")
            _hip_check(H.hipMemcpy(after.ctypes.data, bufs[1], after.nbytes, 2), "hipMemcpy")
        finally:
            for b in bufs:
                if b:
                    H.hipFree(b)
        return out, after

    def path_launches(self):
        out = (C.c_ulonglong * 2)()
        _check(device_lib().ptss_path_launches(self._ctx, out))
        return int(out[0]), int(out[1])

    def _device_buffer(self, name, nbytes):
# ... 277 lines not shown
```

### include/ptss.h

```cpp
#ifndef PTSS_H
#define PTSS_H

#include "ptss_types.h"

#ifdef __cplusplus
extern "C" {
#endif

#define PTSS_OK 0
#define PTSS_EINVAL (-1)
#define PTSS_EHIP (-2)
#define PTSS_ENODEVICE (-3)
#define PTSS_ENOMEM (-4)
#define PTSS_ERANGE (-5)
#define PTSS_ETIMEOUT (-6)
#define PTSS_VERSION 300

typedef struct ptss_context ptss_context;

typedef struct ptss_render_config {
    unsigned int structSize;
    int width, height;
    unsigned long long seed;
    unsigned int maxIterations;
    int device;
    int tileRank, tileWorld, bandRows;
    int syncEachFrame;
    int floatAccumulator;
    int timeKernels;
    int samplesPerPass;
    int everySphereLoop;
    int frameLanes;
    int lanesFreeRun;
    int oneLaunchFrames;
} ptss_render_config;

int ptss_default_config(ptss_render_config* cfg);

int ptss_create(const ptss_scene_desc* scene, const ptss_render_config* cfg, ptss_context** out);

int ptss_destroy(ptss_context* ctx);

int ptss_generate_frame(ptss_context* ctx, ptss_uchar4* dev_pixels, int ticks);

int ptss_set_camera(ptss_context* ctx, const ptss_camera* camera);
int ptss_get_camera(const ptss_context* ctx, ptss_camera* out);
int ptss_request_reset(ptss_context* ctx);
int ptss_set_mode(ptss_context* ctx, int usePathTracer);
int ptss_set_max_iterations(ptss_context* ctx, unsigned int maxIterations);

int ptss_set_stream(ptss_context* ctx, void* hipStream);
int ptss_bind_accumulator(ptss_context* ctx, uint32_t* dev_uint3);
int ptss_accumulator_devptr(ptss_context* ctx, uint32_t** out);
int ptss_float_accumulator_devptr(ptss_context* ctx, float** out);
int ptss_alloc_pixels(ptss_context* ctx, ptss_uchar4** out_dev);
int ptss_free_pixels(ptss_context* ctx, ptss_uchar4* dev);
int ptss_local_pixels(const ptss_context* ctx, size_t* out);
int ptss_local_rows(const ptss_context* ctx, int* rows, int cap, int* count);

int ptss_read_accumulator(ptss_context* ctx, uint32_t* host_uint3, size_t count);
int ptss_read_float_accumulator(ptss_context* ctx, float* host_float3, size_t count);
int ptss_read_pixels(ptss_context* ctx, const ptss_uchar4* dev_pixels, ptss_uchar4* host, size_t count);
int ptss_read_rng_state(ptss_context* ctx, size_t local_pixel, uint32_t* out6);
int ptss_read_rng_state_lane(ptss_context* ctx, size_t local_pixel, unsigned int lane, uint32_t* out6);
int ptss_synchronize(ptss_context* ctx);

int ptss_last_pass_ms(ptss_context* ctx, float* out_ms);
int ptss_samples_since_reset(const ptss_context* ctx, int* out);
int ptss_live_counts(ptss_context* ctx, uint32_t* out, int cap, int* n);
int ptss_total_ray_bounces(ptss_context* ctx, unsigned long long* out);
int ptss_bounce_kernel_time(ptss_context* ctx, double* total_ms, unsigned long long* launches);

int ptss_one_launch_frames(const ptss_context* ctx, int* out);
int ptss_frame_lanes(const ptss_context* ctx, int* out);
int ptss_guard_timeouts(ptss_context* ctx, unsigned int* out);

int ptss_launched_kernels(const ptss_context* ctx, unsigned long long* out);

int ptss_guard_flags(const ptss_context* ctx, unsigned int* out);

int ptss_intersect(ptss_context* ctx, const ptss_ray_query* dev_rays, ptss_ray_hit* dev_hits, size_t n, void* hipStream);
int ptss_occluded(ptss_context* ctx, const ptss_ray_query* dev_rays, uint32_t* dev_occluded, size_t n, void* hipStream);

int ptss_render_features(ptss_context* ctx, ptss_pixel_feature* dev_features, void* hipStream);

int ptss_render_features_motion(ptss_context* ctx, const ptss_triangle* dev_triangles_prev, size_t first, size_t count,
                                ptss_pixel_feature* dev_features, ptss_pixel_motion* dev_motion, void* hipStream);

int ptss_render_features_specular(ptss_context* ctx, int maxSteps, ptss_pixel_feature* dev_features, uint32_t* dev_steps ,
                                  void* hipStream);
int ptss_specular_feature_launches(const ptss_context* ctx, unsigned long long* out2);

int ptss_seed_path_rng(ptss_context* ctx, ptss_path_rng* dev_rng, size_t n, unsigned long long seed, unsigned long long firstSequence,
                       unsigned int skip, void* hipStream);
int ptss_trace_paths(ptss_context* ctx, const ptss_ray_query* dev_rays, ptss_path_rng* dev_rng , ptss_path_result* dev_results,
                     size_t n, unsigned int maxIterations, void* hipStream);
int ptss_path_launches(const ptss_context* ctx, unsigned long long* out2);

int ptss_render_features_scaled(ptss_context* ctx, int factor, ptss_pixel_feature* dev_features_hi, void* hipStream);

int ptss_default_upsample_params(ptss_upsample_params* p);

int ptss_upsample(ptss_context* ctx, const ptss_uchar4* dev_lo, const ptss_pixel_feature* dev_features_lo,
                  const ptss_pixel_feature* dev_features_hi, const ptss_upsample_params* params, ptss_uchar4* dev_out_hi,
                  ptss_history_entry* dev_out_hi_float , void* hipStream);
int ptss_upsample_launches(const ptss_context* ctx, unsigned long long* out);

int ptss_default_denoise_params(ptss_denoise_params* p);

int ptss_denoise(ptss_context* ctx, const ptss_pixel_feature* dev_features, const ptss_denoise_params* params, ptss_uchar4* dev_out,
                 void* hipStream);

int ptss_read_denoise_plane(ptss_context* ctx, float* host_float3, size_t count, int* level);

int ptss_default_reproject_params(ptss_reproject_params* p);

int ptss_reproject(ptss_context* ctx, const ptss_pixel_feature* dev_features_now, const ptss_camera* prev_camera,
                   const ptss_pixel_feature* dev_features_prev, const ptss_history_entry* dev_history_prev,
                   const ptss_reproject_params* params, ptss_history_entry* dev_history_out, void* hipStream);

int ptss_reproject_motion(ptss_context* ctx, const ptss_pixel_feature* dev_features_now, const ptss_pixel_motion* dev_motion_now,
                          const ptss_camera* prev_camera, const ptss_pixel_feature* dev_features_prev,
                          const ptss_history_entry* dev_history_prev, const ptss_reproject_params* params,
                          ptss_history_entry* dev_history_out, void* hipStream);

int ptss_denoise_history(ptss_context* ctx, const ptss_history_entry* dev_history, const ptss_pixel_feature* dev_features,
                         const ptss_denoise_params* params, ptss_uchar4* dev_out, void* hipStream);

int ptss_triangle_leaves(const ptss_context* ctx, int* out);

int ptss_set_scene(ptss_context* ctx, const ptss_scene_desc* scene);

int ptss_update_triangles(ptss_context* ctx, const ptss_triangle* dev_triangles, size_t first, size_t count, void* hipStream);
int ptss_update_rejected(ptss_context* ctx, unsigned long long* out);

int ptss_resort_triangles(ptss_context* ctx, void* hipStream);
int ptss_resort_launches(const ptss_context* ctx, unsigned long long* out);

int ptss_reseed(ptss_context* ctx, unsigned long long seed);

int ptss_read_triangle_bounds(ptss_context* ctx, float* host, size_t count);
int ptss_read_triangle_positions(ptss_context* ctx, int* host, size_t count);

int ptss_debug_counters(ptss_context* ctx, unsigned long long* out8);

const char* ptss_error_string(int code);
const char* ptss_last_error_detail(void);
int ptss_version(void);

#ifdef __cplusplus
}
#endif
#endif
```

### include/ptss_host.h

```cpp
#ifndef PTSS_HOST_H
#define PTSS_HOST_H

#include "ptss_types.h"

#ifdef __cplusplus
extern "C" {
#endif

#define PTSS_HOST_OK 0
#define PTSS_HOST_EINVAL (-1)
#define PTSS_HOST_EIO (-2)

typedef struct ptss_scene ptss_scene;

int ptss_scene_create(const char* preset, ptss_scene** out);
void ptss_scene_destroy(ptss_scene* s);
int ptss_scene_describe(const ptss_scene* s, ptss_scene_desc* out);

int ptss_scene_add_obj(ptss_scene* s, const char* path, const float* mat4x4, int materialIdx, size_t* added);

int ptss_camera_default(ptss_camera* out);
int ptss_camera_move(ptss_camera* cam, unsigned char key, int* moved);
int ptss_camera_ray(const ptss_camera* cam, int width, int height, int x, int y, float jx, float jy, ptss_ray_query* out);

int ptss_write_tga(const char* filename, const ptss_uchar4* rgba, int width, int height);

int ptss_tile_rows(int height, int band_rows, int rank, int world, int* rows, int cap);

int ptss_probe_math(int op, const float* x, const float* y, float* out, size_t n);
int ptss_probe_guard(int op, const float* x, unsigned int* out, size_t n);
int ptss_probe_guard_constants(float* out9);
int ptss_probe_scene_guard_flags(const ptss_scene_desc* scene, unsigned int* out);
int ptss_probe_quantize(const float* x, unsigned int* out, size_t n);
int ptss_probe_quant_table(float* out257);
int ptss_probe_triangle_forms(const float* tri9, const float* o3, const float* d3, const float* limit, int primary, size_t n, int* cls,
                              float* general6, float* classed6);
int ptss_probe_wave_locate(int width, int rank, int world, int bandRows, unsigned int firstBegin, size_t n, int* wave3, int* lane3, int* fast);
int ptss_probe_mesh_bound(const float* tri9, size_t ntri, const float* o3, const float* d3, size_t n, float margin, int* out, float* bound12);
int ptss_probe_mesh_refit(const float* tri9, size_t ntri, float* bounds12);
int ptss_probe_kd_order(const ptss_triangle* triangles, size_t n, int* position);
int ptss_probe_kd_order_signed_zero(const ptss_triangle* triangles, size_t n, int* position);
int ptss_probe_pack_scene(const ptss_scene_desc* scene, int everySphereLoop, int image, int* numImages, int* inLds, void* layout,
                          size_t layoutBytes, float* blob, size_t blobCapacity, size_t* blobWords);
int ptss_probe_mesh_touch(const float* bound12, const float* o3, const float* d3, size_t n, float margin, int* out);
int ptss_probe_denoise(const uint32_t* accum, float inverseTicks, const ptss_pixel_feature* features, int width, int height,
                       const ptss_denoise_params* params, unsigned char* out_rgba, float* out_float);
int ptss_probe_denoise_history(const ptss_history_entry* history, const ptss_pixel_feature* features, int width, int height,
                               const ptss_denoise_params* params, unsigned char* out_rgba, float* out_float);
int ptss_probe_upsample(const unsigned char* lo_rgba, const ptss_pixel_feature* features_lo, int width, int height,
                        const ptss_pixel_feature* features_hi, const ptss_upsample_params* params, unsigned char* out_rgba, float* out_float4);
int ptss_probe_upsample_axis(int X, int factor, int* x0, int* k, float* fx);
int ptss_probe_reproject(const uint32_t* accum, float inverseTicks, int n, const ptss_camera* camera_now, const ptss_camera* camera_prev,
                         int width, int height, const ptss_pixel_feature* features_now, const ptss_pixel_feature* features_prev,
                         const ptss_history_entry* history_prev, const ptss_reproject_params* params, ptss_history_entry* out);
int ptss_probe_reproject_motion(const uint32_t* accum, float inverseTicks, int n, const ptss_camera* camera_now, const ptss_camera* camera_prev,
                                int width, int height, const ptss_pixel_feature* features_now, const ptss_pixel_motion* motion_now,
                                const ptss_pixel_feature* features_prev, const ptss_history_entry* history_prev,
                                const ptss_reproject_params* params, ptss_history_entry* out);
int ptss_probe_motion(const ptss_ray_query* rays, const ptss_ray_hit* hits, size_t n, const ptss_triangle* triangles_prev, size_t first,
                      size_t count, size_t numTriangles, ptss_pixel_motion* out);
int ptss_probe_specular_step(const ptss_ray_query* rays, const ptss_ray_hit* hits, size_t n, const ptss_material* materials, size_t numMaterials,
                             ptss_ray_query* next, int* follows);
int ptss_probe_specular_class(const ptss_material* material);
int ptss_probe_rng_init(unsigned long long seed, unsigned int subsequence, unsigned int* out6);
int ptss_probe_rng_draw(unsigned int* state6, unsigned int* raw, float* uni, size_t n);
int ptss_probe_rng_jump_table(unsigned int* out, size_t words);

#ifdef __cplusplus
}
#endif
#endif
```

Measured before the change: 18370 Mrays/s.

## Cull primary-ray candidates per pixel strip with a conservative frustum mask

Adds a kernel, run whenever the camera changes, that builds a conservative pyramid frustum for each 64-pixel strip in double precision. It culls spheres and triangles that lie entirely outside that frustum and stores one 64-bit keep mask per strip. The primary-bounce closest-hit path reads one mask per wave and skips sphere candidate groups and classed triangle tests that are masked off. The aim is to cut primary intersection work for scenes with few primitives, at the cost of an extra precompute kernel, a per-wave global load, and the risk of wrongly culling a primitive near a frustum edge.

```diff
diff --git a/cuda-path-tracer-ss_amd/csrc/pthit.h b/cuda-path-tracer-ss_amd/csrc/pthit.h
--- a/cuda-path-tracer-ss_amd/csrc/pthit.h
+++ b/cuda-path-tracer-ss_amd/csrc/pthit.h
@@ -5,7 +5,10 @@
 namespace {
 
 template <bool kPrimary, bool kAccel, bool kBounded, bool kMesh = false>
-__device__ __forceinline__ Hit closestHit(const float4* sc, const float4* cold, const SceneLayout& L, vec3 o, vec3 d, bool live, uint32_t* ws) {
+__device__ __forceinline__ Hit closestHit(const float4* sc, const float4* cold, const SceneLayout& L, vec3 o, vec3 d, bool live, uint32_t* ws,
+                                          unsigned long long strip = ~0ull) {
+    constexpr bool kStrips = kPrimary && !kAccel && kBounded && !kMesh;
+    const uint32_t stripSpheres = kStrips ? (uint32_t)strip : ~0u, stripTriangles = kStrips ? (uint32_t)(strip >> 32) : ~0u;
     Hit h;
     h.distance = ptm::inf();
     h.kind = 0;
@@ -14,8 +17,8 @@
     if constexpr (kAccel) closestSpheresRegrouped<kPrimary>(sc, cold, L, o, d, live, h, ws);
     for (int base = 0; base < (kAccel ? 0 : L.numSpheres); base += 32) {
         const int cnt = (L.numSpheres - base < 32) ? (L.numSpheres - base) : 32;
-        uint32_t mask = sphereCandidates<kPrimary, kBounded>(sc, (kPrimary ? L.offPrimSphere : L.offSphere) + base, cnt, o, d);
-        mask &= live ? lowBits(cnt) : 0u;
+        uint32_t mask = sphereCandidates<kPrimary, kBounded, kStrips>(sc, (kPrimary ? L.offPrimSphere : L.offSphere) + base, cnt, o, d, stripSpheres);
+        mask &= live ? (lowBits(cnt) & stripSpheres) : 0u;
         PTSS_DIAG_CANDIDATES(mask, live, 0);
         while (mask != 0) {
             const int j = __builtin_ctz(mask);
@@ -49,8 +52,9 @@
         if (classedQueryOk(o, d)) {
             TriBest best{h.distance, kNoTriangle, 0.0f, 0.0f};
             uint32_t triAt = vectorRow(sc, L.offTri), primAt = vectorRow(sc, L.offPrimTri);
-#define PTSS_CLOSEST_BODY(c1, c2, t) \
-    triangleClassed<kPrimary, c1, c2, true>(rowAt(sc, triAt), rowAt(sc, primAt), 0u, o, d, liveMask, best);
+#define PTSS_CLOSEST_BODY(c1, c2, t)                                                                   \
+    if (!kStrips || ((stripTriangles >> ((uint32_t)(t) & 31u)) & 1u) != 0u)  \
+        triangleClassed<kPrimary, c1, c2, true>(rowAt(sc, triAt), rowAt(sc, primAt), 0u, o, d, liveMask, best);
             PTSS_FOR_TRIANGLES_BY_CLASS(L, PTSS_CLOSEST_BODY, (triAt += 3 * kRowBytes, primAt += 2 * kRowBytes));
 #undef PTSS_CLOSEST_BODY
             if (waveAny(best.key != kNoTriangle)) {
diff --git a/cuda-path-tracer-ss_amd/csrc/ptprim.h b/cuda-path-tracer-ss_amd/csrc/ptprim.h
--- a/cuda-path-tracer-ss_amd/csrc/ptprim.h
+++ b/cuda-path-tracer-ss_amd/csrc/ptprim.h
@@ -256,12 +256,18 @@
         shiftInMayHit(rev, b * b, 4 * pv.w);
     }
 }
-template <bool kPrimary, bool kBounded>
-__device__ __forceinline__ uint32_t sphereCandidates(const float4* image, int firstRow, int cnt, vec3 o, vec3 d) {
+template <bool kPrimary, bool kBounded, bool kStrips = false>
+__device__ __forceinline__ uint32_t sphereCandidates(const float4* image, int firstRow, int cnt, vec3 o, vec3 d, uint32_t wanted = ~0u) {
     const int trips = (cnt + 3) >> 2;
     uint32_t rev = 0;
     uint32_t at = vectorRow(image, firstRow);
     for (int g = 0; g < trips; ++g, at += 4 * kRowBytes) {
+        if constexpr (kStrips) {
+            if (((wanted >> (4 * g)) & 15u) == 0u) {
+                rev <<= 4;
+                continue;
+            }
+        }
         const float4* p = rowAt(image, at);
         const float4 r0 = p[0], r1 = p[1], r2 = p[2], r3 = p[3];
         if constexpr (kPrimary) {
diff --git a/cuda-path-tracer-ss_amd/csrc/ptss_api.hip b/cuda-path-tracer-ss_amd/csrc/ptss_api.hip
--- a/cuda-path-tracer-ss_amd/csrc/ptss_api.hip
+++ b/cuda-path-tracer-ss_amd/csrc/ptss_api.hip
@@ -14,6 +14,7 @@
 #include "ptreproject.h"
 #include "ptspecular.h"
 #include "ptpack.h"
+#include "ptstrip.h"
 
 using namespace ptv;
 using ptpack::cameraInRange;
@@ -97,6 +98,9 @@
     uint32_t capacity = 0, numPixels = 0;
     uint32_t samples = 1;
     bool cameraDirty = true;
+    unsigned long long* dStrips = nullptr;
+    bool stripsOn = false;
+    bool stripsRead = false;
     float defaultColor[3] = {0, 0, 0};
     ptss_camera camera{};
     int lastResetTick = 0;
@@ -360,7 +364,7 @@
 
 ptss::EyeParams eyeParams(const ptss_context* c) {
     return {c->camera, -2 * ptm::tan(c->camera.fieldOfView * 0.5f), (float)c->tile.height / (float)c->tile.width, 1.0f / c->tile.width,
-            1.0f / c->tile.height};
+            1.0f / c->tile.height, nullptr};
 }
 
 void harvestHints(ptss_context* c) {
@@ -615,6 +619,7 @@
         if (c->stagedTwice)
             for (int q = 0; q < 2; ++q) CREATE_TRY(hipEventCreateWithFlags(&c->evDisplay[q], hipEventDisableTiming));
     }
+    CREATE_TRY(hipMalloc(&c->dStrips, (size_t)(c->capacity / ptloc::kStrip) * sizeof(unsigned long long)));
     CREATE_TRY(hipEventCreate(&c->evStart));
     CREATE_TRY(hipEventCreate(&c->evStop));
     CREATE_TRY(hipEventCreate(&c->evEpoch));
@@ -647,6 +652,7 @@
     (void)hipFree(c->dAccumOwned);
     (void)hipFree(c->dFsum);
     (void)hipFree(c->dStaged);
+    (void)hipFree(c->dStrips);
     for (float4* plane : c->dDenoise) (void)hipFree(plane);
     ptss::releaseResortScratch(c->resortScratch);
     (void)hipFree(c->dPathJumpTable);
@@ -682,16 +688,20 @@
     if (c->cfg.syncEachFrame) HIP_TRY(hipEventRecord(c->evStart, st));
 
     const int numIterations = c->usePathTracer ? (int)c->maxIterations : 1;
-    const ptss::EyeParams eye = eyeParams(c);
+    ptss::EyeParams eye = eyeParams(c);
+    const bool bounded = c->image().layout.sphereBounded != 0 && cameraInRange(c->camera);
     if (c->cameraDirty) {
         forkNeeded = true;
         HIP_TRY(ptss::launchPrimaryPrep(st, c->image().dBlob, c->image().layout, c->camera.position));
+        c->stripsOn = ptstrip::eligible(c->image().layout, bounded);
+        if (c->stripsOn) HIP_TRY(ptss::launchStripMasks(st, c->dStrips, c->capacity, c->numPixels, c->image().dBlob, c->image().layout, c->tile, eye));
         c->cameraDirty = false;
     }
+    if (c->stripsOn && !(c->image().oneLaunch && K == 1)) eye.strips = c->dStrips;
+    c->stripsRead = eye.strips != nullptr;
     harvestHints(c);
     RC_TRY(forkLanes(c, forkNeeded));
     if (c->cfg.timeKernels) drainKernelEvents(c, false);
-    const bool bounded = c->image().layout.sphereBounded != 0 && cameraInRange(c->camera);
     RC_TRY(c->image().oneLaunch && K == 1 ? traceOneLaunch(c, fbs[0], numIterations, bounded, eye) : traceBounces(c, fbs, numIterations, bounded, eye));
     RC_TRY(flushAndJoin(c, fbs, numIterations));
     if (c->samples > 1) {
@@ -715,6 +725,23 @@
     c->camera = *camera;
     c->cameraDirty = true;
     c->resetTicksThisFrame = true;
+    return PTSS_OK;
+}
+
+int ptss_read_strip_words(ptss_context* c, unsigned long long* host_words, size_t capacity, size_t* count, int* enabled) {
+    if (!c || !host_words || !count || !enabled) return fail(PTSS_EINVAL, "null argument");
+    const size_t n = c->capacity / ptloc::kStrip;
+    *count = n;
+    if (capacity < n) return fail(PTSS_EINVAL, "host_words holds fewer words than the context has strips");
+    const bool on = c->stripsRead && !c->cameraDirty;
+    *enabled = on ? 1 : 0;
+    if (!on) {
+        for (size_t i = 0; i < n; ++i) host_words[i] = ptstrip::kAll;
+        return PTSS_OK;
+    }
+    HIP_TRY(hipSetDevice(c->cfg.device));
+    HIP_TRY(hipStreamSynchronize(c->stream));
+    HIP_TRY(hipMemcpy(host_words, c->dStrips, n * sizeof(unsigned long long), hipMemcpyDeviceToHost));
     return PTSS_OK;
 }
 
diff --git a/cuda-path-tracer-ss_amd/csrc/ptss_device.h b/cuda-path-tracer-ss_amd/csrc/ptss_device.h
--- a/cuda-path-tracer-ss_amd/csrc/ptss_device.h
+++ b/cuda-path-tracer-ss_amd/csrc/ptss_device.h
@@ -59,6 +59,7 @@
     float s;
     float aspect;
     float invW, invH;
+    const unsigned long long* strips;
 };
 
 constexpr int kMaxLanes = 4;
@@ -105,6 +106,8 @@
 hipError_t launchDisplay(hipStream_t st, const FrameBuffers& fb);
 hipError_t launchClear(hipStream_t st, const FrameBuffers& fb);
 hipError_t launchPrimaryPrep(hipStream_t st, float4* sceneBlob, const SceneLayout& layout, ptss_vec3 origin);
+hipError_t launchStripMasks(hipStream_t st, unsigned long long* masks, uint32_t plane, uint32_t numPixels, const float4* sceneBlob,
+                            const SceneLayout& layout, TileMap tile, EyeParams eye);
 hipError_t launchBounce(hipStream_t st, const FrameBuffers& fb, const float4* sceneBlob, SceneLayout layout, int bounce,
                         bool isLast, bool sceneInLds, bool bounded, int gridBlocks, TileMap tile, EyeParams eye, unsigned long long* launched);
 hipError_t launchFrame(hipStream_t st, const FrameBuffers& fb, const float4* sceneBlob, SceneLayout layout, int numBounces, bool bounded, int gridBlocks,
diff --git a/cuda-path-tracer-ss_amd/csrc/ptss_kernels.hip b/cuda-path-tracer-ss_amd/csrc/ptss_kernels.hip
--- a/cuda-path-tracer-ss_amd/csrc/ptss_kernels.hip
+++ b/cuda-path-tracer-ss_amd/csrc/ptss_kernels.hip
@@ -3,6 +3,7 @@
 #include "ptspecular.h"
 #include "pthit.h"
 #include "ptshade.h"
+#include "ptstrip.h"
 
 #include <array>
 #include <utility>
@@ -88,6 +89,15 @@
         blob[L.offPrimTri + 2 * i] = float4{s.x, s.y, s.z, dot(e2, r)};
         blob[L.offPrimTri + 2 * i + 1] = float4{r.x, r.y, r.z, 0.0f};
     }
+}
+
+__global__ void stripMaskKernel(unsigned long long* __restrict__ masks, uint32_t numStrips, uint32_t numPixels, const float4* __restrict__ blob,
+                                SceneLayout L, TileMap tile, EyeParams eye) {
+    const uint32_t i = blockIdx.x * blockDim.x + threadIdx.x;
+    if (i >= numStrips) return;
+    const ptstrip::View view{eye.camera, eye.s, eye.aspect, eye.invW, eye.invH};
+    const ptstrip::Tile t{tile.width, tile.rank, tile.world, tile.bandRows};
+    masks[i] = ptstrip::stripMask(view, t, numPixels, i * ptloc::kStrip, reinterpret_cast<const float*>(blob), L);
 }
 
 struct TileEnv {
@@ -131,6 +141,11 @@
         ray.o = ray.d = ray.L0 = ray.T = v3(0, 0, 0);
         ray.pix = 0;
         ray.active = false;
+        unsigned long long strip = ptstrip::kAll;
+        if constexpr (kFirst && !kAccel && kBounded && !kMesh) {
+            const uint32_t waveFirst = __builtin_amdgcn_readfirstlane(firstPixel - lane);
+            if (eye.strips != nullptr) strip = eye.strips[waveFirst >> 6];
+        }
         if constexpr (kFirst) {
             if (valid) {
                 const uint32_t pixel = firstPixel;
@@ -157,7 +172,7 @@
         h.kind = 2; h.idx = (int)(pixOf(ray.pix) % (uint32_t)L.numTriangles); h.distance = 1.0f + ray.d.x;
         h.w0 = 0.3f; h.w1 = 0.3f; h.w2 = 0.4f;
 #else
-        const Hit h = closestHit<kFirst, kAccel, kBounded, kMesh>(sc, sceneBlob, L, ray.o, ray.d, valid, reinterpret_cast<uint32_t*>(wq));
+        const Hit h = closestHit<kFirst, kAccel, kBounded, kMesh>(sc, sceneBlob, L, ray.o, ray.d, valid, reinterpret_cast<uint32_t*>(wq), strip);
 #endif
         const bool hit = valid && h.kind != 0;
         if constexpr (!kFirst) {
@@ -849,6 +864,14 @@
     return hipGetLastError();
 }
 
+hipError_t launchStripMasks(hipStream_t st, unsigned long long* masks, uint32_t plane, uint32_t numPixels, const float4* sceneBlob,
+                            const SceneLayout& layout, TileMap tile, EyeParams eye) {
+    const uint32_t numStrips = plane / ptloc::kStrip;
+    if (numStrips == 0) return hipSuccess;
+    hipLaunchKernelGGL(stripMaskKernel, dim3(blocksFor(numStrips, 64)), dim3(64), 0, st, masks, numStrips, numPixels, sceneBlob, layout, tile, eye);
+    return hipGetLastError();
+}
+
 #if PTSS_DIAG
 hipError_t readDiagCounters(unsigned long long* out8) { return hipMemcpyFromSymbol(out8, HIP_SYMBOL(g_diag), 64); }
 #endif
diff --git a/cuda-path-tracer-ss_amd/csrc/ptstrip.h b/cuda-path-tracer-ss_amd/csrc/ptstrip.h
--- /dev/null
+++ b/cuda-path-tracer-ss_amd/csrc/ptstrip.h
@@ -0,0 +1,173 @@
+#pragma once
+#include "ptlocate.h"
+#include "ptscene.h"
+
+namespace ptstrip {
+
+constexpr unsigned long long kAll = ~0ull;
+constexpr int kMaxPerKind = 32;
+constexpr double kPixelMargin = 1.0;
+constexpr double kTheta = 1e-4;
+constexpr double kSphereRel = 1e-5;
+constexpr double kInsideRel = 2e-3;
+constexpr double kGraze = 1e-3;
+constexpr double kPlaneRel = 1e-4;
+constexpr double kWeightEps = 16.0 / 16777216.0;
+constexpr double kCoordLimit = 1048576.0;
+
+struct D3 {
+    double x, y, z;
+};
+PTM_HD D3 d3(double x, double y, double z) { return D3{x, y, z}; }
+PTM_HD D3 operator+(D3 a, D3 b) { return D3{a.x + b.x, a.y + b.y, a.z + b.z}; }
+PTM_HD D3 operator-(D3 a, D3 b) { return D3{a.x - b.x, a.y - b.y, a.z - b.z}; }
+PTM_HD D3 operator*(D3 a, double s) { return D3{a.x * s, a.y * s, a.z * s}; }
+PTM_HD double dot(D3 a, D3 b) { return a.x * b.x + a.y * b.y + a.z * b.z; }
+PTM_HD D3 cross(D3 a, D3 b) { return D3{a.y * b.z - a.z * b.y, a.z * b.x - a.x * b.z, a.x * b.y - a.y * b.x}; }
+PTM_HD double length(D3 a) { return __builtin_sqrt(dot(a, a)); }
+PTM_HD double absd(double x) { return __builtin_fabs(x); }
+PTM_HD bool within(double x, double limit) { return absd(x) <= limit; }
+PTM_HD bool within(D3 a, double limit) { return within(a.x, limit) && within(a.y, limit) && within(a.z, limit); }
+
+struct View {
+    ptss_camera camera;
+    float s, aspect, invW, invH;
+};
+struct Tile {
+    int width, rank, world, bandRows;
+};
+
+PTM_HD bool viewInDomain(const View& v) {
+    const ptss_quat q = v.camera.rotation;
+    const double qq = (double)q.x * q.x + (double)q.y * q.y + (double)q.z * q.z + (double)q.w * q.w;
+    const double s = v.s, a = v.aspect;
+    return within(d3(v.camera.position.x, v.camera.position.y, v.camera.position.z), kCoordLimit) && qq >= 1.0 - 1e-3 && qq <= 1.0 + 1e-3 &&
+           absd((double)v.camera.zNear) >= 0x1p-30 && absd((double)v.camera.zNear) <= 0x1p30 && absd(s) >= 0x1p-20 && a > 0.0 && absd(s) * (a > 1.0 ? a : 1.0) <= 16.0 &&
+           v.invW > 0.0f && v.invW <= 1.0f && v.invH > 0.0f && v.invH <= 1.0f;
+}
+
+PTM_HD D3 rotated(ptss_quat q, D3 v) {
+    const D3 u = d3(q.x, q.y, q.z);
+    const D3 uv = cross(u, v);
+    const D3 uuv = cross(u, uv);
+    return (v + uv * (2.0 * (double)q.w)) + uuv * 2.0;
+}
+
+struct Pyramid {
+    D3 n[5];
+    D3 corner[4];
+    bool ok;
+};
+PTM_HD Pyramid pyramidOf(const View& v, int x0, int x1, int y0, int y1) {
+    Pyramid p;
+    p.ok = false;
+    const double s = v.s, sy = (double)v.s * (double)v.aspect;
+    const double ua = (((double)x0 - kPixelMargin) * (double)v.invW - 0.5) * s, ub = (((double)x1 + 1.0 + kPixelMargin) * (double)v.invW - 0.5) * s;
+    const double va = (((double)y0 - kPixelMargin) * (double)v.invH - 0.5) * sy, vb = (((double)y1 + 1.0 + kPixelMargin) * (double)v.invH - 0.5) * sy;
+    const ptss_quat q = v.camera.rotation;
+    const double z = v.camera.zNear < 0.0f ? -1.0 : 1.0;
+    const D3 w[4] = {rotated(q, d3(ua, va, 1.0) * z), rotated(q, d3(ub, va, 1.0) * z), rotated(q, d3(ub, vb, 1.0) * z), rotated(q, d3(ua, vb, 1.0) * z)};
+    const D3 centre = rotated(q, d3(0.5 * (ua + ub), 0.5 * (va + vb), 1.0) * z);
+    const double centreLen = length(centre);
+    if (!(centreLen > 0.0)) return p;
+    bool ok = true;
+    for (int k = 0; k < 5; ++k) {
+        D3 n = k < 4 ? cross(w[k], w[(k + 1) & 3]) : cross(rotated(q, d3(1.0, 0.0, 0.0)), rotated(q, d3(0.0, 1.0, 0.0)));
+        const double len = length(n);
+        if (!(len > 0.0) || !within(len, 1e300)) return p;
+        n = n * (1.0 / len);
+        const double side = dot(n, centre) / centreLen;
+        if (side < 0.0) n = n * -1.0;
+        ok = ok && absd(side) > 1e-9;
+        p.n[k] = n;
+    }
+    for (int k = 0; k < 4; ++k) {
+        const double len = length(w[k]);
+        if (!(len > 0.0) || !within(len, 1e300)) return p;
+        p.corner[k] = w[k] * (1.0 / len);
+    }
+    p.ok = ok;
+    return p;
+}
+
+PTM_HD bool sphereCulled(const Pyramid& p, D3 o, const float* row) {
+    const D3 c = d3(row[0], row[1], row[2]);
+    const double r2 = row[3];
+    if (!within(c, kCoordLimit) || !(r2 > 0.0) || !(r2 <= kCoordLimit * kCoordLimit)) return false;
+    const D3 v = c - o;
+    const double vv = dot(v, v);
+    if (!(vv > r2 * (1.0 + kInsideRel))) return false;
+    const double reff = __builtin_sqrt(r2 + kSphereRel * vv);
+    const double slack = reff + kTheta * (__builtin_sqrt(vv) + reff);
+    for (int k = 0; k < 5; ++k)
+        if (dot(p.n[k], v) < -slack) return true;
+    return false;
+}
+
+PTM_HD bool triangleCulled(const Pyramid& p, D3 o, const float* rows) {
+    const D3 v0 = d3(rows[0], rows[1], rows[2]), e1 = d3(rows[4], rows[5], rows[6]), e2 = d3(rows[8], rows[9], rows[10]);
+    if (!within(v0, kCoordLimit) || !within(e1, 2.0 * kCoordLimit) || !within(e2, 2.0 * kCoordLimit)) return false;
+    const D3 N = cross(e1, e2);
+    const double l1 = length(e1), l2 = length(e2), L2 = l1 * l2, lenN = length(N);
+    if (!(L2 > 0.0)) return false;
+    const D3 vert[3] = {v0, v0 + e1, v0 + e2};
+    const D3 s0 = vert[0] - o, s1 = vert[1] - o, s2 = vert[2] - o;
+    double smax = length(s0);
+    const double len1 = length(s1), len2 = length(s2);
+    smax = len1 > smax ? len1 : smax;
+    smax = len2 > smax ? len2 : smax;
+    if (!(absd(dot(s0, N)) >= kPlaneRel * smax * L2)) return false;
+    double lo = 0.0;
+    int positive = 0, negative = 0;
+    for (int k = 0; k < 4; ++k) {
+        const double a = dot(p.corner[k], N);
+        positive += a > 0.0 ? 1 : 0;
+        negative += a < 0.0 ? 1 : 0;
+        const double m = absd(a);
+        lo = (k == 0 || m < lo) ? m : lo;
+    }
+    if (positive != 4 && negative != 4) return false;
+    const double detMin = lo - kTheta * lenN;
+    if (!(detMin >= kGraze * L2)) return false;
+    const double beta = kWeightEps * smax * (l1 + l2) / detMin + 1e-6;
+    if (!within(beta, 1e6)) return false;
+    const D3 g = (vert[0] + vert[1] + vert[2]) * (1.0 / 3.0);
+    D3 big[3];
+    double far[3];
+    for (int i = 0; i < 3; ++i) {
+        big[i] = (g + (vert[i] - g) * (1.0 + 3.0 * beta)) - o;
+        far[i] = kTheta * length(big[i]);
+    }
+    for (int k = 0; k < 5; ++k)
+        if (dot(p.n[k], big[0]) < -far[0] && dot(p.n[k], big[1]) < -far[1] && dot(p.n[k], big[2]) < -far[2]) return true;
+    return false;
+}
+
+PTM_HD unsigned long long rectMask(const View& v, const float* blob, const ptss::SceneLayout& L, int x0, int x1, int y) {
+    const Pyramid p = pyramidOf(v, x0, x1, y, y);
+    if (!p.ok) return kAll;
+    const D3 o = d3(v.camera.position.x, v.camera.position.y, v.camera.position.z);
+    unsigned long long m = 0ull;
+    for (int j = 0; j < L.numSpheres; ++j)
+        if (!sphereCulled(p, o, blob + 4 * (size_t)(L.offSphere + j))) m |= 1ull << j;
+    for (int t = 0; t < L.numTriangles; ++t)
+        if (!triangleCulled(p, o, blob + 4 * (size_t)(L.offTri + 3 * t))) m |= 1ull << (32 + t);
+    return m;
+}
+
+inline bool eligible(const ptss::SceneLayout& L, bool bounded) {
+    return bounded && !L.accelSpheres && L.triClassed && L.numSpheres <= kMaxPerKind && L.numTriangles <= kMaxPerKind;
+}
+
+PTM_HD unsigned long long stripMask(const View& v, const Tile& t, uint32_t numPixels, uint32_t first, const float* blob, const ptss::SceneLayout& L) {
+    if (first >= numPixels || L.numSpheres > kMaxPerKind || L.numTriangles > kMaxPerKind || !viewInDomain(v)) return kAll;
+    const uint32_t last = (first + (ptloc::kStrip - 1) < numPixels) ? first + (ptloc::kStrip - 1) : numPixels - 1;
+    const uint32_t rowFirst = first / (uint32_t)t.width, rowLast = last / (uint32_t)t.width;
+    if (rowLast - rowFirst > 1u) return kAll;
+    const ptloc::Coord a = ptloc::locate(t.width, t.rank, t.world, t.bandRows, first);
+    const ptloc::Coord b = ptloc::locate(t.width, t.rank, t.world, t.bandRows, last);
+    if (rowLast == rowFirst) return rectMask(v, blob, L, a.x, b.x, a.gy);
+    return rectMask(v, blob, L, a.x, t.width - 1, a.gy) | rectMask(v, blob, L, 0, b.x, b.gy);
+}
+
+}
diff --git a/cuda-path-tracer-ss_amd/host/host_capi.cpp b/cuda-path-tracer-ss_amd/host/host_capi.cpp
--- a/cuda-path-tracer-ss_amd/host/host_capi.cpp
+++ b/cuda-path-tracer-ss_amd/host/host_capi.cpp
@@ -17,6 +17,7 @@
 #include "ptmesh.h"
 #include "ptorder.h"
 #include "ptpack.h"
+#include "ptstrip.h"
 #include "pttri.h"
 #include "xorwow.h"
 
@@ -205,6 +206,43 @@
             b[0] = ref.x; b[1] = ref.gy; b[2] = (int)ref.globalIndex;
         }
     }
+    return PTSS_HOST_OK;
+}
+
+int ptss_probe_strip_masks(const ptss_scene_desc* scene, const ptss_camera* camera, int width, int height, int bandRows, int rank, int world,
+                           unsigned long long* masks, size_t capacity, size_t* numStrips, int* enabled, int* triPos) {
+    if (!scene || !camera || !masks || !numStrips || !enabled || width <= 0 || height <= 0 || bandRows <= 0 || world <= 0 || rank < 0 || rank >= world ||
+        ptpack::validateScene(*scene))
+        return PTSS_HOST_EINVAL;
+    int rows = 0;
+    for (int y = 0; y < height; ++y)
+        if ((y / bandRows) % world == rank) ++rows;
+    const uint32_t numPixels = (uint32_t)width * (uint32_t)rows;
+    const uint32_t plane = numPixels == 0 ? (uint32_t)ptss::kBlock : ((numPixels + ptss::kBlock - 1) / ptss::kBlock) * ptss::kBlock;
+    const size_t n = plane / ptloc::kStrip;
+    *numStrips = n;
+    if (capacity < n) return PTSS_HOST_EINVAL;
+    std::vector<ptpack::PackedImage> images;
+    try {
+        images = ptpack::packImages(*scene, false);
+    } catch (const std::bad_alloc&) {
+        return PTSS_HOST_EINVAL;
+    }
+    const bool inRange = ptpack::cameraInRange(*camera);
+    const ptpack::PackedImage& im = images[(images.size() > 1 && !inRange) ? 1 : 0];
+    const bool on = ptstrip::eligible(im.layout, im.layout.sphereBounded != 0 && inRange);
+    *enabled = on ? 1 : 0;
+    if (triPos && im.layout.numTriangles > 0) {
+        if (im.layout.triClassed || ptss::meshImage(im.layout))
+            std::memcpy(triPos, &im.blob[(size_t)im.layout.offTriPos], sizeof(int) * (size_t)im.layout.numTriangles);
+        else
+            for (int t = 0; t < im.layout.numTriangles; ++t) triPos[t] = t;
+    }
+    const ptstrip::View view{*camera, -2 * ptm::tan(camera->fieldOfView * 0.5f), (float)height / (float)width, 1.0f / width, 1.0f / height};
+    const ptstrip::Tile tile{width, rank, world, bandRows};
+    for (size_t i = 0; i < n; ++i)
+        masks[i] = on ? ptstrip::stripMask(view, tile, numPixels, (uint32_t)(i * ptloc::kStrip), reinterpret_cast<const float*>(im.blob.data()), im.layout)
+                      : ptstrip::kAll;
     return PTSS_HOST_OK;
 }
 
diff --git a/cuda-path-tracer-ss_amd/ptss.py b/cuda-path-tracer-ss_amd/ptss.py
--- a/cuda-path-tracer-ss_amd/ptss.py
+++ b/cuda-path-tracer-ss_amd/ptss.py
@@ -153,6 +153,8 @@
         L.ptss_probe_motion.argtypes = [C.c_void_p, C.c_void_p, C.c_size_t, C.c_void_p, C.c_size_t, C.c_size_t, C.c_size_t, C.c_void_p]
         L.ptss_probe_specular_step.argtypes = [C.c_void_p, C.c_void_p, C.c_size_t, C.c_void_p, C.c_size_t, C.c_void_p, C.POINTER(C.c_int)]
         L.ptss_probe_specular_class.argtypes = [C.c_void_p]
+        L.ptss_probe_strip_masks.argtypes = [C.POINTER(SceneDesc), C.POINTER(Camera), C.c_int, C.c_int, C.c_int, C.c_int, C.c_int, C.c_void_p,
+                                             C.c_size_t, C.POINTER(C.c_size_t), C.POINTER(C.c_int), C.c_void_p]
         _host = L
     return _host
 
@@ -239,6 +241,7 @@
         L.ptss_resort_triangles.argtypes = [vp, vp]
         L.ptss_resort_launches.argtypes = [vp, C.POINTER(C.c_ulonglong)]
         L.ptss_reseed.argtypes = [vp, C.c_ulonglong]
+        L.ptss_read_strip_words.argtypes = [vp, C.c_void_p, C.c_size_t, C.POINTER(C.c_size_t), C.POINTER(C.c_int)]
         L.ptss_read_triangle_bounds.argtypes = [vp, _f32p, C.c_size_t]
         L.ptss_read_triangle_positions.argtypes = [vp, C.POINTER(C.c_int), C.c_size_t]
         L.ptss_error_string.argtypes = [C.c_int]
@@ -635,6 +638,20 @@
                 raise PtssError("ptss_camera_ray failed")
             out[y * width + x] = buf
     return out
+
+
+def probe_strip_masks(scene, cam, width, height, band_rows=8, rank=0, world=1):
+    desc = scene.desc if hasattr(scene, "desc") else scene
+    rows = len(tile_rows(height, band_rows, rank, world))
+    cap = max((width * rows + 255) // 256, 1) * 4
+    masks = np.zeros(cap, dtype=np.uint64)
+    tri_pos = np.zeros(max(int(desc.numTriangles), 1), dtype=np.int32)
+    n, on = C.c_size_t(), C.c_int()
+    rc = host_lib().ptss_probe_strip_masks(C.byref(desc), C.byref(cam), width, height, band_rows, rank, world, masks.ctypes.data_as(C.c_void_p), cap,
+                                           C.byref(n), C.byref(on), tri_pos.ctypes.data_as(C.c_void_p))
+    if rc != 0:
+        raise PtssError(f"ptss_probe_strip_masks: {rc}")
+    return masks[:n.value], bool(on.value), tri_pos[:int(desc.numTriangles)]
 
 
 def tile_rows(height, band_rows, rank, world):
@@ -862,6 +879,13 @@
         v = C.c_ulonglong()
         _check(device_lib().ptss_resort_launches(self._ctx, C.byref(v)))
         return v.value
+
+    def strip_words(self):
+        cap = max((self.local_pixels + 255) // 256, 1) * 4
+        words = np.zeros(cap, dtype=np.uint64)
+        n, on = C.c_size_t(), C.c_int()
+        _check(device_lib().ptss_read_strip_words(self._ctx, words.ctypes.data_as(C.c_void_p), cap, C.byref(n), C.byref(on)))
+        return words[:n.value], bool(on.value)
 
     def reseed(self, seed):
         _check(device_lib().ptss_reseed(self._ctx, seed))
diff --git a/include/ptss.h b/include/ptss.h
--- a/include/ptss.h
+++ b/include/ptss.h
@@ -77,6 +77,8 @@
 
 int ptss_launched_kernels(const ptss_context* ctx, unsigned long long* out);
 
+int ptss_read_strip_words(ptss_context* ctx, unsigned long long* host_words, size_t capacity, size_t* count, int* enabled);
+
 int ptss_guard_flags(const ptss_context* ctx, unsigned int* out);
 
 int ptss_intersect(ptss_context* ctx, const ptss_ray_query* dev_rays, ptss_ray_hit* dev_hits, size_t n, void* hipStream);
diff --git a/include/ptss_host.h b/include/ptss_host.h
--- a/include/ptss_host.h
+++ b/include/ptss_host.h
@@ -36,6 +36,8 @@
 int ptss_probe_triangle_forms(const float* tri9, const float* o3, const float* d3, const float* limit, int primary, size_t n, int* cls,
                               float* general6, float* classed6);
 int ptss_probe_wave_locate(int width, int rank, int world, int bandRows, unsigned int firstBegin, size_t n, int* wave3, int* lane3, int* fast);
+int ptss_probe_strip_masks(const ptss_scene_desc* scene, const ptss_camera* camera, int width, int height, int bandRows, int rank, int world,
+                           unsigned long long* masks, size_t capacity, size_t* numStrips, int* enabled, int* triPos);
 int ptss_probe_mesh_bound(const float* tri9, size_t ntri, const float* o3, const float* d3, size_t n, float margin, int* out, float* bound12);
 int ptss_probe_mesh_refit(const float* tri9, size_t ntri, float* bounds12);
 int ptss_probe_kd_order(const ptss_triangle* triangles, size_t n, int* position);
```

Result: faster. 18690 Mrays/s (median of 6 runs) (+1.8%).
